# Owen1B/KAIR

Measured on AMD Instinct MI355X. Metric: train patches/sec + PSNR, SwinIR x4 48-px LQ, at 1/2/4/8 MI355X, higher is better.
Workload: dtype fp32x3

## Files before the change

include/kair_hip.h:

```cpp
#ifndef KAIR_HIP_H
#define KAIR_HIP_H

#ifdef __cplusplus
extern "C" {
#endif

#define KAIR_OK 0
#define KAIR_ERR_ARG (-1)
#define KAIR_ERR_HIP (-2)

typedef enum { KAIR_F32 = 0, KAIR_BF16 = 1, KAIR_F16 = 3 } kair_dtype;
#define KAIR_COMPUTE_X3 2
#define KAIR_X3_WEXP 12

typedef enum {
  KAIR_LD_ROWS = 0,
  KAIR_LD_IM2COL3 = 1,
  KAIR_LD_QKVBLK = 2,
  KAIR_LD_S2D = 3
} kair_load_mode;

typedef struct {
  const void* ptr;
  int dtype;
// ... 47 lines not shown
} kair_epilogue;

int kair_gemm_nt(const kair_operand* A, const kair_operand* B, const kair_epilogue* E,
                 long M, int N, int K, int compute, void* stream);

int kair_conv3x3_halo_geometry(int H, int W, int C, long M, int N);

int kair_wgrad_splits(long M, int N, int K);
int kair_gemm_tn(const kair_operand* A, const kair_operand* B, float* ws, int splits,
                 long M, int N, int K, int compute, void* stream);

typedef struct {
  int kind;
  int N, K;
  int nG, nGr, nGp;
  int kG, kGr, kGp;
  int n_perm;
} kair_wmap;

int kair_pack_weight(const float* src, void* dst, int dst_dtype, const kair_wmap* map, void* stream);
typedef struct kair_pack_job {
  const float* src;
  void* dst;
  int dst_dtype;
  int reserved;
  kair_wmap map;
  long total;
} kair_pack_job;
long kair_pack_table_bytes(int njobs);
long kair_pack_table_build(kair_pack_job* jobs, int njobs, void* table_dev);
int kair_pack_weights(const void* table_dev, int njobs, long nblocks, void* stream);
int kair_wgrad_finalize(const float* partial, int splits, const kair_wmap* map, float* grad_ref,
                        float* bias_grad, int ones_col, int accumulate, void* stream);
typedef struct {
  kair_operand A, B;
  int N, K;
  kair_wmap map;
  float* grad;
  float* bias_grad;
  int ones_col;
} kair_wgrad_job;
long kair_wgrad_grouped_ws(const kair_wgrad_job* jobs, int njobs, long M);
int kair_wgrad_grouped(const kair_wgrad_job* jobs, int njobs, long M, float* ws, void* stream);
int kair_wgrad_grouped_ex(const kair_wgrad_job* jobs, int njobs, long M, float* ws, int max_ctas, void* stream);
int kair_colsum(const kair_operand* G, long M, int Np, const kair_wmap* map, float* bias_grad,
                float* ws, int accumulate, void* stream);

int kair_layernorm_fwd(const float* x, long ldx, void* y, int y_dtype, long ldy, const float* gamma,
                       const float* beta, float* mean, float* rstd, long M, int C, float eps,
                       int win_H, int win_W, int win_ws, int win_shift, int one_col, void* stream);
int kair_layernorm_fwd_x3(const float* x, long ldx, void* y_hi, void* y_lo, long ldy, const float* gamma,
                          const float* beta, float* mean, float* rstd, long M, int C, float eps,
                          int win_H, int win_W, int win_ws, int win_shift, int one_col, int x3_exp, void* stream);
typedef struct {
  void* out;
  int dtype;
  long ld;
  const float* rowscale;
  int rows_per_scale;
  int win_H, win_W, win_ws, win_shift;
  void* out_lo;
  int x3_exp;
} kair_copy_desc;
int kair_row_copy(const float* src, long ld_src, long M, int C, const kair_copy_desc* copy, void* stream);

int kair_layernorm_bwd(const float* x, long ldx, const void* dy, int dy_dtype, long ldy,
                       const float* gamma, const float* mean, const float* rstd, float* dx_acc,
                       long ld_dx, int dx_accumulate, float* dgamma, float* dbeta, int dparam_accumulate,
                       float* ws, long M, int C, int win_H, int win_W, int win_ws, int win_shift,
                       const kair_copy_desc* copy, void* stream);

long kair_layernorm_bwd_blocks(long M);
typedef struct {
  const float* part; long nb; int C;
  float* dgamma; float* dbeta; int accumulate;
} kair_ln_param_job;
int kair_ln_param_reduce_grouped(const kair_ln_param_job* jobs, int njobs, void* stream);

int kair_window_attn_fwd(const void* qkv, int dtype, const float* table, void* O, long ldo, float* lse,
                         long nWin, int nh, int hd, float scale, int H, int W, int shift, int ones_col,
                         const float* mask, int mask_nw, void* stream);
long kair_window_attn_bwd_ws(long nWin, int nh);
int kair_window_attn_bwd(const void* qkv, const void* O, long ldo, const void* dO, long lddo, int dtype,
                         const float* table, const float* lse, void* dqkv, float* dtable, int dtable_accumulate,
                         float* ws, long nWin, int nh, int hd, float scale, int H, int W, int shift,
                         const float* mask, int mask_nw, void* stream);
int kair_window_attn_bwd_ex(const void* qkv, const void* O, long ldo, const void* dO, long lddo, int dtype,
                            const float* table, const float* lse, void* dqkv, int dqkv_rows, float* dtable,
                            int dtable_accumulate, float* ws, long nWin, int nh, int hd, float scale, int H, int W,
                            int shift, const float* mask, int mask_nw, int head_pad, void* stream);
int kair_window_attn_fwd_ex(const void* qkv, int dtype, const float* table, void* O, long ldo, float* lse,
                            long nWin, int nh, int hd, float scale, int H, int W, int shift, int ones_col,
                            const float* mask, int mask_nw, int head_pad, void* stream);
int kair_window_attn_fwd_w(const void* qkv, int dtype, const float* table, void* O, long ldo, float* lse,
                           long nWin, int nh, int hd, float scale, int H, int W, int shift, int ones_col,
                           const float* mask, int mask_nw, int head_pad, int ws, void* stream);
int kair_window_attn_bwd_w(const void* qkv, const void* O, long ldo, const void* dO, long lddo, int dtype,
                           const float* table, const float* lse, void* dqkv, int dqkv_rows, float* dtable,
                           int dtable_accumulate, float* ws, long nWin, int nh, int hd, float scale, int H, int W,
                           int shift, const float* mask, int mask_nw, int head_pad, int win_ws, void* stream);
long kair_window_attn_bwd_ws_w(long nWin, int nh, int win_ws);

int kair_window_attn_fwd_x3(const void* qkv, const void* qkv_lo, const float* table, void* O, void* O_lo, long ldo,
                            float* lse, long nWin, int nh, int hd, float scale, int H, int W, int shift, int ones_col,
                            int e_in, int e_out, void* stream);
int kair_window_attn_bwd_x3(const void* qkv, const void* qkv_lo, const void* O, const void* O_lo, long ldo,
                            const void* dO, const void* dO_lo, long lddo, const float* table, const float* lse,
                            void* dqkv, void* dqkv_lo, float* dtable, int dtable_accumulate, float* ws, long nWin,
                            int nh, int hd, float scale, int H, int W, int shift, int e_act, int e_grad, void* stream);
int kair_window_attn_fwd_x3_w(const void* qkv, const void* qkv_lo, const float* table, void* O, void* O_lo, long ldo,
                              float* lse, long nWin, int nh, int hd, float scale, int H, int W, int shift, int ones_col,
                              int e_in, int e_out, int ws, void* stream);
int kair_window_attn_bwd_x3_w(const void* qkv, const void* qkv_lo, const void* O, const void* O_lo, long ldo,
                              const void* dO, const void* dO_lo, long lddo, const float* table, const float* lse,
                              void* dqkv, void* dqkv_lo, float* dtable, int dtable_accumulate, float* ws, long nWin,
                              int nh, int hd, float scale, int H, int W, int shift, int e_act, int e_grad, int win_ws,
                              void* stream);

long kair_window_attn_bwd_groups(long nWin, int nh, int dtype);
typedef struct {
  const float* ws; long nWin; int nh; int dtype;
  float* dtable; int accumulate;
  int win_ws;
} kair_attn_dtable_job;
int kair_attn_dtable_grouped(const kair_attn_dtable_job* jobs, int njobs, void* stream);

int kair_swin_attn_fwd(const float* x, long ldx, const float* gamma, const float* beta, float eps, int C,
                       void* ln, long ldln, float* mean, float* rstd, const void* wqkv, const float* bqkv,
                       void* qkv, const float* table, float scale, void* O, long ldo, int o_ones_col,
                       float* lse, const void* wproj, const float* bproj, const float* rowscale,
                       int rows_per_scale, float* out, long ldout, long nWin, int nh, int H, int W, int shift,
                       int w_split, void* stream);
int kair_swin_mlp_fwd(const float* x, long ldx, const float* gamma, const float* beta, float eps, int C,
                      void* ln, long ldln, float* mean, float* rstd, const void* w1, const float* b1, void* u,
                      void* h, long ldh, int hd, const void* w2, const float* b2, const float* rowscale,
                      int rows_per_scale, float* out, long ldout, long M, int Cp, int Hp, int w_split,
                      void* stream);

long kair_swin_mlp_bwd_ws(void);
int kair_swin_mlp_bwd(const void* dc, long lddc, const void* gd, long ldg, const void* w2t, const void* w1t,
                      void* du, long lddu, const float* x, long ldx, const float* gamma, const float* mean,
                      const float* rstd, int C, float* D, long ldD, void* dco, long lddo, const float* rowscale,
                      int rows_per_scale, int H, int W, int shift, float* dgamma, float* dbeta, int dparam_acc,
                      float* ws, long M, int Cp, int Hp, void* stream);

int kair_conv3x3_wr_tile(int split, int B, int H, int W, int C, int N);
int kair_conv3x3_wr(const void* x, int x_dtype, long ldx, int split, int flip, const void* w, int n_blocks,
                    const float* bias, const float* resid, long ldr, void* out, int out_dtype, long ldo, void* acopy,
                    long ldac, int acones, int B, int H, int W, int C, int N, void* stream);
int kair_conv3x3_wr_ex(const void* x, int x_dtype, long ldx, int split, int flip, const void* w, int n_blocks,
                       const float* bias, const float* resid, long ldr, void* out, int out_dtype, long ldo, void* out_lo,
                       int ps_r, int act, float slope, const void* gate, long ldg, void* acopy, long ldac, int acones,
                       int B, int H, int W, int C, int N, void* stream);

int kair_conv3x3_narrow_fwd(const void* x, long ldx, int lo_off, const void* w, const float* bias, int NR,
                            const float* mean, float img_range, const float* resid, float* out, int B, int H, int W,
                            void* stream);
long kair_conv3x3_narrow_dgrad_ws(void);
int kair_conv3x3_narrow_dgrad(const void* dE, long lde, const float* w, int NR, void* ws, void* out, int out_dtype,
                              long ldo, int ps_r, int B, int H, int W, void* stream);
long kair_conv3x3_narrow_wgrad_ws(int NR);
int kair_conv3x3_narrow_wgrad(const void* dE, long lde, const void* x, long ldx, int NR, float* ws, float* grad_w,
                              float* grad_b, int accumulate, int B, int H, int W, void* stream);

long kair_conv3x3_narrow_x3_ws(void);
int kair_conv3x3_narrow_fwd_x3(const float* x, long ldx, int ex, const float* w, const float* bias, int NR, void* ws,
                               const float* mean, float img_range, const float* resid, float* out, int B, int H, int W,
                               void* stream);
int kair_conv3x3_narrow_dgrad_x3(const float* dE, long lde, int eg, const float* w, int NR, void* ws, float* out, long ldo,
                                 int ps_r, int B, int H, int W, void* stream);
int kair_conv3x3_narrow_wgrad_x3(const float* dE, long lde, int eg, const float* x, long ldx, int ex, int NR, float* ws,
                                 float* grad_w, float* grad_b, int accumulate, int B, int H, int W, void* stream);

int kair_image_to_nhwc(const float* img, void* out, int dtype, int ldc, const float* mean, float img_range,
                       int B, int C, int H, int W, void* stream);
int kair_image_to_nhwc_hilo(const float* img, void* out, int ldc, const float* mean, float img_range,
                            int B, int C, int H, int W, void* stream);
int kair_l1_loss(const float* E, const float* H, float* loss_out, void* dE, int dtype, int ldc, int ps_r, float weight,
                 int B, int C, int Hh, int Ww, float* ws, void* stream);
int kair_charbonnier_loss(const float* E, const float* H, float* loss_out, void* dE, int dtype, int ldc, int ps_r,
                          float weight, float eps, int B, int C, int Hh, int Ww, float* ws, void* stream);
int kair_axpy(float* y, const float* x, float a, long n, void* stream);
long kair_bn_ws(int C);
int kair_bn_fwd(const float* z, long ldz, void* out, int out_dtype, long ldo, long M, int C, const float* gamma,
                const float* beta, float* running_mean, float* running_var, float momentum, float eps, int training,
                float* mean, float* rstd, int act, float slope, float* ws, void* stream);
int kair_bn_bwd(const float* z, long ldz, const void* a, int a_dtype, long lda, const float* da, long ldda, void* dz,
                int dz_dtype, long lddz, long M, int C, const float* gamma, const float* mean, const float* rstd,
                int act, float slope, float* dgamma, float* dbeta, int accumulate, float* ws, void* stream);

int kair_axpby(float* y, const float* x, float a, float b, long n, void* stream);
int kair_axpby_rows(float* y, long ldy, const float* x, long ldx, long M, int C, float a, float b, void* stream);
int kair_act_grad_cast(const float* G, long ldg, const void* X, int x_dtype, long ldx, void* out, int out_dtype,
                       long ldo, long M, int C, int kind, float slope, float scale, void* stream);
int kair_sumpool2x(const float* src, long lds, float* dst, long ldd, int B, int H, int W, int C, int accumulate,
                   void* stream);
int kair_adam_ema(float* p, const float* g, float* m, float* v, float* ema, long n, const float* lr_t,
                  float beta1, float beta2, float eps, float weight_decay, float ema_decay, void* stream);
int kair_adam_ema_ex(float* p, const float* g, float* m, float* v, float* ema, long n, const float* lr_t,
                     float beta1, float beta2, float eps, float weight_decay, float ema_decay, const unsigned* skip,
                     void* stream);
int kair_range_check(const float* g, const float* p, long n, const float* loss, float p_limit, unsigned* flag,
                     void* stream);
long kair_gemm_nt_x3_lnbwd_parts(long M, int N);
int kair_gemm_nt_x3_lnbwd(const kair_operand* A, const kair_operand* B, long M, int N, int K, int win_H, int win_W,
                          int win_ws, int win_shift, const float* x, long ldx, const float* gamma, const float* mean,
                          const float* rstd, int C, float* D, long ldd, float* part, const kair_copy_desc* copy,
                          void* stream);

int kair_ktime_begin(int n);
int kair_ktime_count(void);
int kair_ktime_end(void);
int kair_ktime_read(int i, float* ms, const char** name);

int kair_gate_hold(int timeout_ms, void* stream);
int kair_gate_release(void);
int kair_gate_status(void);

#define KAIR_USR_SRC_NCHW 0
#define KAIR_USR_SRC_PSF 1
#define KAIR_USR_SRC_ZUP 2
#define KAIR_USR_SRC_NHWC 3
#define KAIR_USR_COL_FB 0
#define KAIR_USR_COL_FBFY 1
#define KAIR_USR_COL_DATA_FWD 2
#define KAIR_USR_COL_DATA_BWD 3
#define KAIR_USR_CHAN_CHUNKS 64
int kair_usr_fft_rows(const float* src, int src_mode, int C, long ld, int kh, int kw, int sf, void* T,
                      int planes, int H, int W, void* stream);
int kair_usr_fft_cols(int mode, const void* T, void* T_out, const void* FB, const void* FBFy, void* FR,
                      float* invW, const float* alpha, int alpha_stride, float* part, int planes, int C,
                      int H, int W, int sf, void* stream);
int kair_usr_ifft_rows(const void* T, void* dst, int nhwc, int dst_dtype, int C, long ld, float scale,
                       int planes, int H, int W, void* stream);
int kair_usr_seg_sum(const float* ws, int seglen, int nseg, float scale, float* out, int ostride,
                     int accumulate, void* stream);
int kair_usr_chan_sum(const float* x, long ld, int c, long HW, int B, float* ws, float* out, int ostride,
                      int accumulate, void* stream);
enum { KAIR_USR_PAD_REPLICATE = 0, KAIR_USR_PAD_ZERO = 1, KAIR_USR_PAD_FOLD = 2, KAIR_USR_CROP_NCHW = 3 };
int kair_usr_pad(const void* src, void* dst, int dtype, int mode, int ldc, int nb, int H, int W, int Hp, int Wp,
                 void* stream);
int kair_usr_upsample_nearest(const float* L, float* out, int planes, int h, int w, int sf, void* stream);
int kair_usr_pack_input(const float* x, const float* beta, int beta_stride, void* out, int dtype, int ld,
                        int B, int C, long HW, void* stream);
int kair_hypanet_fwd(const float* sigma, float sf, const float* W1, const float* b1, const float* W2,
                     const float* b2, const float* W3, const float* b3, int hc, int no, int B, float* ab,
                     void* stream);
int kair_hypanet_bwd(const float* sigma, float sf, const float* W1, const float* b1, const float* W2,
                     const float* b2, const float* W3, const float* b3, int hc, int no, int B, const float* gab,
                     float* gW1, float* gb1, float* gW2, float* gb2, float* gW3, float* gb3, int accumulate,
                     void* stream);

int kair_rowgemm_store(const void* A, long lda, long M, int K, const void* W, int N, void* out, long ldo,
                       void* stream);
int kair_rowgemm_gate(const void* A, long lda, long M, int K, const void* W, int N, const void* gate, long ldg,
                      void* out, long ldo, void* stream);
long kair_rowgemm_ln_blocks(long M, int K);
int kair_rowgemm_lnbwd(const void* A, long lda, long M, int K, const void* W, const float* x, long ldx,
                       const float* gamma, const float* mean, const float* rstd, int C, float* D, long ldD,
                       int win_H, int win_W, int win_ws, int win_shift, const kair_copy_desc* copy, float* part,
                       void* stream);

int kair_synth_sr(const float* pool, int C, int Hs, int Ws, const int* params, int B, int PS, int sf,
                  const float* wh, const int* ih, const float* ww, const int* iw, int P, float* outH,
                  float* outL, void* stream);
int kair_synth_dn(const float* pool, int C, int Hs, int Ws, const int* params, int B, int PS, float sigma,
                  unsigned long long seed, unsigned long long step, float* outH, float* outL, void* stream);

const char* kair_last_error(void);
int kair_device_arch(char* buf, int len);

int kair_debug_attn_stamps(unsigned long long* host, int n);
int kair_debug_fused_stamps(unsigned long long* host, int n);
int kair_debug_x3_stamps(unsigned long long* host, int n);

#ifdef __cplusplus
}
#endif
#endif
```

kair_amd/_hip.py:

```python
import ctypes
import os

import torch

LIB_PATH = os.path.join(os.path.dirname(os.path.abspath(__file__)), "lib",
                        {"debug": "libkair_hip_dbg.so", "base": "libkair_hip_base.so"}.get(os.environ.get("KAIR_LIB"),
                                                                                          "libkair_hip.so"))

F32, BF16, F16 = 0, 1, 3
X3 = 2
X3_WEXP = 12
LD_ROWS, LD_IM2COL3, LD_QKVBLK, LD_S2D = 0, 1, 2, 3
USR_SRC_NCHW, USR_SRC_PSF, USR_SRC_ZUP, USR_SRC_NHWC = 0, 1, 2, 3
USR_COL_FB, USR_COL_FBFY, USR_COL_DATA_FWD, USR_COL_DATA_BWD = 0, 1, 2, 3
USR_CHAN_CHUNKS = 64
USR_PAD_REPLICATE, USR_PAD_ZERO, USR_PAD_FOLD, USR_CROP_NCHW = 0, 1, 2, 3
OUT_ROWS, OUT_QKVBLK, OUT_PSHUF, OUT_PUNSHUF, OUT_NCHW, OUT_PSHUF_NCHW = 0, 1, 2, 3, 4, 5
OUT_PSHUF_SPM, OUT_PUNSHUF_SPM = 6, 7
ACT_NONE, ACT_GELU, ACT_LEAKY, ACT_RELU = 0, 1, 2, 3

c_long, c_int, c_float, c_vp = ctypes.c_long, ctypes.c_int, ctypes.c_float, ctypes.c_void_p


class Operand(ctypes.Structure):
    _fields_ = [("ptr", c_vp), ("dtype", c_int), ("mode", c_int), ("ld", c_long),
                ("win_H", c_int), ("win_W", c_int), ("win_ws", c_int), ("win_shift", c_int),
                ("im_H", c_int), ("im_W", c_int), ("im_C", c_int), ("im_flip", c_int),
                ("qkv_nh", c_int), ("qkv_hdp", c_int), ("qkv_tok", c_int),
                ("rowscale", c_vp), ("rows_per_scale", c_int), ("ones_col", c_int), ("ones_in_data", c_int),
                ("im_up", c_int), ("w_split", c_int), ("a_split", c_int), ("lo_ptr", c_vp), ("x3_exp", c_int)]


class CopyDesc(ctypes.Structure):
    _fields_ = [("out", c_vp), ("dtype", c_int), ("ld", c_long), ("rowscale", c_vp), ("rows_per_scale", c_int),
                ("win_H", c_int), ("win_W", c_int), ("win_ws", c_int), ("win_shift", c_int), ("out_lo", c_vp),
                ("x3_exp", c_int)]


def copy_desc(out, ld=None, rowscale=None, rows_per_scale=1, win=None, x3_exp=0):
    d = CopyDesc()
    d._keep = (out, rowscale)
    if out.dtype == torch.float16:
        d.out, d.out_lo, d.dtype, d.x3_exp = ptr(out[0]), ptr(out[1]), F16, int(x3_exp)
    else:
        d.out, d.dtype = ptr(out), dtype_code(out)
    d.ld = ld if ld is not None else out.shape[-1]
    d.rowscale, d.rows_per_scale = ptr(rowscale), rows_per_scale
    if win:
        d.win_H, d.win_W, d.win_ws, d.win_shift = win
    return d


class Epilogue(ctypes.Structure):
    _fields_ = [("out", c_vp), ("out_dtype", c_int), ("out_mode", c_int), ("ldo", c_long),
                ("win_H", c_int), ("win_W", c_int), ("win_ws", c_int), ("win_shift", c_int),
                ("bias", c_vp), ("act", c_int), ("slope", c_float),
                ("out_pre", c_vp), ("pre_dtype", c_int), ("ldp", c_long),
                ("resid", c_vp), ("ldr", c_long),
                ("rowscale", c_vp), ("rows_per_scale", c_int),
                ("gate", c_vp), ("gate_dtype", c_int), ("ldg", c_long), ("gate_kind", c_int),
                ("ps_r", c_int), ("ps_H", c_int), ("ps_W", c_int),
                ("qkv_nh", c_int), ("qkv_hdp", c_int), ("qkv_tok", c_int),
                ("img_mean", c_vp), ("img_range", c_float), ("img_C", c_int), ("img_H", c_int), ("img_W", c_int),
                ("out_ones_col_p1", c_int), ("resid2", c_vp), ("ldr2", c_long), ("pre_kind", c_int),
                ("a_copy", c_vp), ("ld_acopy", c_long), ("acopy_ones_col_p1", c_int), ("out_lo", c_vp),
                ("x3_out_exp", c_int)]


class WMap(ctypes.Structure):
    _fields_ = [("kind", c_int), ("N", c_int), ("K", c_int), ("nG", c_int), ("nGr", c_int), ("nGp", c_int),
                ("kG", c_int), ("kGr", c_int), ("kGp", c_int), ("n_perm", c_int)]


class WgradJob(ctypes.Structure):
    _fields_ = [("A", Operand), ("B", Operand), ("N", c_int), ("K", c_int), ("map", WMap), ("grad", c_vp),
                ("bias_grad", c_vp), ("ones_col", c_int)]


class LnParamJob(ctypes.Structure):
    _fields_ = [("part", c_vp), ("nb", c_long), ("C", c_int), ("dgamma", c_vp), ("dbeta", c_vp), ("accumulate", c_int)]


class DtabJob(ctypes.Structure):
    _fields_ = [("ws", c_vp), ("nWin", c_long), ("nh", c_int), ("dtype", c_int), ("dtable", c_vp), ("accumulate", c_int),
                ("win_ws", c_int)]


class PackJob(ctypes.Structure):
    _fields_ = [("src", c_vp), ("dst", c_vp), ("dst_dtype", c_int), ("reserved", c_int), ("map", WMap),
                ("total", c_long)]


_SIGS = {
    "kair_gemm_nt": [ctypes.POINTER(Operand), ctypes.POINTER(Operand), ctypes.POINTER(Epilogue), c_long, c_int, c_int,
                     c_int, c_vp],
    "kair_wgrad_splits": [c_long, c_int, c_int],
    "kair_conv3x3_halo_geometry": [c_int, c_int, c_int, c_long, c_int],
    "kair_gemm_tn": [ctypes.POINTER(Operand), ctypes.POINTER(Operand), c_vp, c_int, c_long, c_int, c_int, c_int, c_vp],
    "kair_wgrad_grouped_ws": [ctypes.POINTER(WgradJob), c_int, c_long],
    "kair_wgrad_grouped": [ctypes.POINTER(WgradJob), c_int, c_long, c_vp, c_vp],
    "kair_wgrad_grouped_ex": [ctypes.POINTER(WgradJob), c_int, c_long, c_vp, c_int, c_vp],
    "kair_layernorm_bwd_blocks": [c_long],
    "kair_ln_param_reduce_grouped": [ctypes.POINTER(LnParamJob), c_int, c_vp],
    "kair_window_attn_bwd_groups": [c_long, c_int, c_int],
    "kair_attn_dtable_grouped": [ctypes.POINTER(DtabJob), c_int, c_vp],
    "kair_pack_weight": [c_vp, c_vp, c_int, ctypes.POINTER(WMap), c_vp],
    "kair_pack_table_bytes": [c_int],
    "kair_pack_table_build": [ctypes.POINTER(PackJob), c_int, c_vp],
    "kair_pack_weights": [c_vp, c_int, c_long, c_vp],
    "kair_wgrad_finalize": [c_vp, c_int, ctypes.POINTER(WMap), c_vp, c_vp, c_int, c_int, c_vp],
    "kair_colsum": [ctypes.POINTER(Operand), c_long, c_int, ctypes.POINTER(WMap), c_vp, c_vp, c_int, c_vp],
    "kair_layernorm_fwd": [c_vp, c_long, c_vp, c_int, c_long, c_vp, c_vp, c_vp, c_vp, c_long, c_int, c_float, c_int,
                           c_int, c_int, c_int, c_int, c_vp],
    "kair_layernorm_fwd_x3": [c_vp, c_long, c_vp, c_vp, c_long, c_vp, c_vp, c_vp, c_vp, c_long, c_int, c_float, c_int,
                              c_int, c_int, c_int, c_int, c_int, c_vp],
    "kair_layernorm_bwd": [c_vp, c_long, c_vp, c_int, c_long, c_vp, c_vp, c_vp, c_vp, c_long, c_int, c_vp, c_vp, c_int,
                           c_vp, c_long, c_int, c_int, c_int, c_int, c_int, ctypes.POINTER(CopyDesc), c_vp],
    "kair_row_copy": [c_vp, c_long, c_long, c_int, ctypes.POINTER(CopyDesc), c_vp],
    "kair_gemm_nt_x3_lnbwd": [ctypes.POINTER(Operand), ctypes.POINTER(Operand), c_long, c_int, c_int, c_int, c_int, c_int,
                              c_int, c_vp, c_long, c_vp, c_vp, c_vp, c_int, c_vp, c_long, c_vp, ctypes.POINTER(CopyDesc),
                              c_vp],
    "kair_gemm_nt_x3_lnbwd_parts": [c_long, c_int],
    "kair_window_attn_fwd": [c_vp, c_int, c_vp, c_vp, c_long, c_vp, c_long, c_int, c_int, c_float, c_int, c_int, c_int,
                             c_int, c_vp, c_int, c_vp],
    "kair_window_attn_bwd_ws": [c_long, c_int],
    "kair_window_attn_bwd_ws_w": [c_long, c_int, c_int],
    "kair_window_attn_fwd_w": [c_vp, c_int, c_vp, c_vp, c_long, c_vp, c_long, c_int, c_int, c_float, c_int, c_int, c_int,
                               c_int, c_vp, c_int, c_int, c_int, c_vp],
    "kair_window_attn_bwd_w": [c_vp, c_vp, c_long, c_vp, c_long, c_int, c_vp, c_vp, c_vp, c_int, c_vp, c_int, c_vp, c_long,
                               c_int, c_int, c_float, c_int, c_int, c_int, c_vp, c_int, c_int, c_int, c_vp],
    "kair_window_attn_fwd_x3_w": [c_vp, c_vp, c_vp, c_vp, c_vp, c_long, c_vp, c_long, c_int, c_int, c_float, c_int, c_int,
                                  c_int, c_int, c_int, c_int, c_int, c_vp],
    "kair_window_attn_bwd_x3_w": [c_vp, c_vp, c_vp, c_vp, c_long, c_vp, c_vp, c_long, c_vp, c_vp, c_vp, c_vp, c_vp, c_int,
                                  c_vp, c_long, c_int, c_int, c_float, c_int, c_int, c_int, c_int, c_int, c_int, c_vp],
    "kair_window_attn_bwd": [c_vp, c_vp, c_long, c_vp, c_long, c_int, c_vp, c_vp, c_vp, c_vp, c_int, c_vp, c_long, c_int,
                             c_int, c_float, c_int, c_int, c_int, c_vp, c_int, c_vp],
    "kair_window_attn_bwd_ex": [c_vp, c_vp, c_long, c_vp, c_long, c_int, c_vp, c_vp, c_vp, c_int, c_vp, c_int, c_vp, c_long,
                                c_int, c_int, c_float, c_int, c_int, c_int, c_vp, c_int, c_int, c_vp],
    "kair_window_attn_fwd_ex": [c_vp, c_int, c_vp, c_vp, c_long, c_vp, c_long, c_int, c_int, c_float, c_int, c_int, c_int,
                                c_int, c_vp, c_int, c_int, c_vp],
    "kair_image_to_nhwc": [c_vp, c_vp, c_int, c_int, c_vp, c_float, c_int, c_int, c_int, c_int, c_vp],
    "kair_image_to_nhwc_hilo": [c_vp, c_vp, c_int, c_vp, c_float, c_int, c_int, c_int, c_int, c_vp],
    "kair_conv3x3_narrow_fwd": [c_vp, c_long, c_int, c_vp, c_vp, c_int, c_vp, c_float, c_vp, c_vp, c_int, c_int, c_int,
                                c_vp],
    "kair_conv3x3_wr_tile": [c_int, c_int, c_int, c_int, c_int, c_int],
    "kair_conv3x3_wr": [c_vp, c_int, c_long, c_int, c_int, c_vp, c_int, c_vp, c_vp, c_long, c_vp, c_int, c_long, c_vp,
                        c_long, c_int, c_int, c_int, c_int, c_int, c_int, c_vp],
    "kair_conv3x3_wr_ex": [c_vp, c_int, c_long, c_int, c_int, c_vp, c_int, c_vp, c_vp, c_long, c_vp, c_int, c_long, c_vp,
                           c_int, c_int, c_float, c_vp, c_long, c_vp, c_long, c_int, c_int, c_int, c_int, c_int, c_int,
                           c_vp],
    "kair_conv3x3_narrow_dgrad_ws": [],
    "kair_conv3x3_narrow_dgrad": [c_vp, c_long, c_vp, c_int, c_vp, c_vp, c_int, c_long, c_int, c_int, c_int, c_int, c_vp],
    "kair_conv3x3_narrow_wgrad_ws": [c_int],
    "kair_conv3x3_narrow_wgrad": [c_vp, c_long, c_vp, c_long, c_int, c_vp, c_vp, c_vp, c_int, c_int, c_int, c_int, c_vp],
    "kair_conv3x3_narrow_x3_ws": [],
    "kair_conv3x3_narrow_fwd_x3": [c_vp, c_long, c_int, c_vp, c_vp, c_int, c_vp, c_vp, c_float, c_vp, c_vp, c_int, c_int,
                                   c_int, c_vp],
    "kair_conv3x3_narrow_dgrad_x3": [c_vp, c_long, c_int, c_vp, c_int, c_vp, c_vp, c_long, c_int, c_int, c_int, c_int,
                                     c_vp],
    "kair_conv3x3_narrow_wgrad_x3": [c_vp, c_long, c_int, c_vp, c_long, c_int, c_int, c_vp, c_vp, c_vp, c_int, c_int,
                                     c_int, c_int, c_vp],
    "kair_l1_loss": [c_vp, c_vp, c_vp, c_vp, c_int, c_int, c_int, c_float, c_int, c_int, c_int, c_int, c_vp, c_vp],
    "kair_charbonnier_loss": [c_vp, c_vp, c_vp, c_vp, c_int, c_int, c_int, c_float, c_float, c_int, c_int, c_int, c_int,
                              c_vp, c_vp],
    "kair_axpy": [c_vp, c_vp, c_float, c_long, c_vp],
    "kair_axpby": [c_vp, c_vp, c_float, c_float, c_long, c_vp],
    "kair_bn_ws": [c_int],
    "kair_bn_fwd": [c_vp, c_long, c_vp, c_int, c_long, c_long, c_int, c_vp, c_vp, c_vp, c_vp, c_float, c_float, c_int,
                    c_vp, c_vp, c_int, c_float, c_vp, c_vp],
    "kair_bn_bwd": [c_vp, c_long, c_vp, c_int, c_long, c_vp, c_long, c_vp, c_int, c_long, c_long, c_int, c_vp, c_vp, c_vp,
                    c_int, c_float, c_vp, c_vp, c_int, c_vp, c_vp],
    "kair_axpby_rows": [c_vp, c_long, c_vp, c_long, c_long, c_int, c_float, c_float, c_vp],
    "kair_act_grad_cast": [c_vp, c_long, c_vp, c_int, c_long, c_vp, c_int, c_long, c_long, c_int, c_int, c_float, c_float,
                           c_vp],
    "kair_sumpool2x": [c_vp, c_long, c_vp, c_long, c_int, c_int, c_int, c_int, c_int, c_vp],
    "kair_adam_ema": [c_vp, c_vp, c_vp, c_vp, c_vp, c_long, c_vp, c_float, c_float, c_float, c_float, c_float, c_vp],
    "kair_adam_ema_ex": [c_vp, c_vp, c_vp, c_vp, c_vp, c_long, c_vp, c_float, c_float, c_float, c_float, c_float, c_vp,
                         c_vp],
    "kair_range_check": [c_vp, c_vp, c_long, c_vp, c_float, c_vp, c_vp],
    "kair_gate_hold": [c_int, c_vp],
    "kair_gate_release": [],
    "kair_gate_status": [],
    "kair_ktime_begin": [c_int],
    "kair_ktime_count": [],
    "kair_ktime_end": [],
    "kair_ktime_read": [c_int, ctypes.POINTER(ctypes.c_float), ctypes.POINTER(ctypes.c_char_p)],
    "kair_usr_fft_rows": [c_vp, c_int, c_int, c_long, c_int, c_int, c_int, c_vp, c_int, c_int, c_int, c_vp],
    "kair_usr_fft_cols": [c_int, c_vp, c_vp, c_vp, c_vp, c_vp, c_vp, c_vp, c_int, c_vp, c_int, c_int, c_int, c_int, c_int,
                          c_vp],
    "kair_usr_ifft_rows": [c_vp, c_vp, c_int, c_int, c_int, c_long, c_float, c_int, c_int, c_int, c_vp],
    "kair_usr_seg_sum": [c_vp, c_int, c_int, c_float, c_vp, c_int, c_int, c_vp],
    "kair_usr_chan_sum": [c_vp, c_long, c_int, c_long, c_int, c_vp, c_vp, c_int, c_int, c_vp],
    "kair_usr_upsample_nearest": [c_vp, c_vp, c_int, c_int, c_int, c_int, c_vp],
    "kair_usr_pack_input": [c_vp, c_vp, c_int, c_vp, c_int, c_int, c_int, c_int, c_long, c_vp],
    "kair_usr_pad": [c_vp, c_vp, c_int, c_int, c_int, c_int, c_int, c_int, c_int, c_int, c_vp],
    "kair_hypanet_fwd": [c_vp, c_float] + [c_vp] * 6 + [c_int, c_int, c_int, c_vp, c_vp],
    "kair_hypanet_bwd": [c_vp, c_float] + [c_vp] * 6 + [c_int, c_int, c_int, c_vp] + [c_vp] * 6 + [c_int, c_vp],
    "kair_synth_sr": [c_vp, c_int, c_int, c_int, c_vp, c_int, c_int, c_int, c_vp, c_vp, c_vp, c_vp, c_int, c_vp, c_vp,
                      c_vp],
    "kair_synth_dn": [c_vp, c_int, c_int, c_int, c_vp, c_int, c_int, c_float, ctypes.c_ulonglong, ctypes.c_ulonglong,
                      c_vp, c_vp, c_vp],
    "kair_swin_attn_fwd": [c_vp, c_long, c_vp, c_vp, c_float, c_int, c_vp, c_long, c_vp, c_vp, c_vp, c_vp, c_vp, c_vp,
                           c_float, c_vp, c_long, c_int, c_vp, c_vp, c_vp, c_vp, c_int, c_vp, c_long, c_long, c_int,
                           c_int, c_int, c_int, c_int, c_vp],
    "kair_swin_mlp_fwd": [c_vp, c_long, c_vp, c_vp, c_float, c_int, c_vp, c_long, c_vp, c_vp, c_vp, c_vp, c_vp, c_vp,
                          c_long, c_int, c_vp, c_vp, c_vp, c_int, c_vp, c_long, c_long, c_int, c_int, c_int, c_vp],
    "kair_debug_attn_stamps": [c_vp, c_int],
    "kair_debug_fused_stamps": [c_vp, c_int],
    "kair_debug_x3_stamps": [c_vp, c_int],
    "kair_swin_mlp_bwd_ws": [],
    "kair_swin_mlp_bwd": [c_vp, c_long, c_vp, c_long, c_vp, c_vp, c_vp, c_long, c_vp, c_long, c_vp, c_vp, c_vp, c_int,
                          c_vp, c_long, c_vp, c_long, c_vp, c_int, c_int, c_int, c_int, c_vp, c_vp, c_int, c_vp, c_long,
                          c_int, c_int, c_vp],
    "kair_rowgemm_store": [c_vp, c_long, c_long, c_int, c_vp, c_int, c_vp, c_long, c_vp],
    "kair_rowgemm_gate": [c_vp, c_long, c_long, c_int, c_vp, c_int, c_vp, c_long, c_vp, c_long, c_vp],
    "kair_rowgemm_ln_blocks": [c_long, c_int],
    "kair_rowgemm_lnbwd": [c_vp, c_long, c_long, c_int, c_vp, c_vp, c_long, c_vp, c_vp, c_vp, c_int, c_vp, c_long,
                           c_int, c_int, c_int, c_int, ctypes.POINTER(CopyDesc), c_vp, c_vp],
    "kair_window_attn_fwd_x3": [c_vp, c_vp, c_vp, c_vp, c_vp, c_long, c_vp, c_long, c_int, c_int, c_float, c_int, c_int,
                                c_int, c_int, c_int, c_int, c_vp],
    "kair_window_attn_bwd_x3": [c_vp, c_vp, c_vp, c_vp, c_long, c_vp, c_vp, c_long, c_vp, c_vp, c_vp, c_vp, c_vp, c_int,
                                c_vp, c_long, c_int, c_int, c_float, c_int, c_int, c_int, c_int, c_int, c_vp],
    "kair_last_error": [],
    "kair_device_arch": [ctypes.c_char_p, c_int],
}
_RESTYPE = {"kair_gemm_nt_x3_lnbwd_parts": c_long, "kair_layernorm_bwd_blocks": c_long, "kair_rowgemm_ln_blocks": c_long, "kair_window_attn_bwd_groups": c_long, "kair_wgrad_grouped_ws": c_long, "kair_swin_mlp_bwd_ws": c_long, "kair_bn_ws": c_long, "kair_last_error": ctypes.c_char_p, "kair_window_attn_bwd_ws": c_long, "kair_window_attn_bwd_ws_w": c_long, "kair_pack_table_bytes": c_long,
            "kair_pack_table_build": c_long, "kair_conv3x3_narrow_wgrad_ws": c_long,
            "kair_conv3x3_narrow_dgrad_ws": c_long, "kair_conv3x3_narrow_x3_ws": c_long}

_lib = None


def lib():
    global _lib
    if _lib is None:
        if not os.path.exists(LIB_PATH):
            raise RuntimeError(f"kair_amd: HIP kernel library not built ({LIB_PATH}); run `python -m kair_amd.build`")
        L = ctypes.CDLL(LIB_PATH)
        for name, args in _SIGS.items():
            if (name.startswith("kair_debug_") or os.environ.get("KAIR_LIB") == "base") and not hasattr(L, name):
                continue
            fn = getattr(L, name)
            fn.argtypes = args
            fn.restype = _RESTYPE.get(name, c_int)
        _lib = L
    return _lib


def exported_symbols():
    return list(_SIGS)


def check(rc, what=""):
    if rc != 0:
        msg = lib().kair_last_error().decode(errors="replace")
        raise RuntimeError(f"kair_hip {what} failed ({rc}): {msg}")


def ptr(t):
    if t is None:
        return None
    return t.data_ptr()


def stream_ptr():
    return torch.cuda.current_stream().cuda_stream


def dtype_code(t):
    if t.dtype == torch.float32:
        return F32
    if t.dtype == torch.bfloat16:
        return BF16
    if t.dtype == torch.float16:
        return F16
    raise TypeError(f"unsupported dtype {t.dtype}")


def require_device(*ts):
    for t in ts:
        if t is not None and not t.is_cuda:
            raise RuntimeError("kair_amd runs on the HIP device only (got a CPU tensor); there is no CPU fallback")


def rows(t, ld=None, win=None, rowscale=None, rows_per_scale=1, ones_col=-1, ones_in_data=False, w_split=False):
    o = Operand()
    o._keep = (t, rowscale)
    o.ptr = ptr(t)
    o.dtype = dtype_code(t)
    o.mode = LD_ROWS
    o.ld = ld if ld is not None else t.shape[-1]
    if win:
        o.win_H, o.win_W, o.win_ws, o.win_shift = win
    o.rowscale = ptr(rowscale)
    o.rows_per_scale = rows_per_scale
    o.ones_col = ones_col
    o.ones_in_data = int(ones_in_data)
    o.w_split = int(w_split)
    return o


def asplit(op, lo=None, pair=False):
    op.a_split = 2 if pair else 1
# ... 162 lines not shown
        arr = (PackJob * n)()
        for i, (src, dst, m) in enumerate(jobs):
            arr[i].src, arr[i].dst, arr[i].dst_dtype, arr[i].map = ptr(src), ptr(dst), dtype_code(dst), m
        self._keep = [(s, d) for s, d, _ in jobs]
        self.n = n
        self.table = torch.empty(lib().kair_pack_table_bytes(n), dtype=torch.uint8, device=jobs[0][1].device)
        nb = lib().kair_pack_table_build(arr, n, ptr(self.table))
        if nb <= 0:
            check(int(nb) or -1, "pack_table_build")
        self.nblocks = nb

    def run(self):
        check(lib().kair_pack_weights(ptr(self.table), self.n, self.nblocks, stream_ptr()), "pack_weights")


def wgrad_finalize(partial, splits, m, grad, bias_grad=None, ones_col=-1, accumulate=False):
    check(lib().kair_wgrad_finalize(ptr(partial), splits, ctypes.byref(m), ptr(grad), ptr(bias_grad), ones_col,
                                    int(accumulate), stream_ptr()), "wgrad_finalize")


def colsum(G, M, Np, m, bias_grad, ws, accumulate=False):
    check(lib().kair_colsum(ctypes.byref(G), M, Np, ctypes.byref(m), ptr(bias_grad), ptr(ws), int(accumulate),
                            stream_ptr()), "colsum")


def layernorm_fwd(x, ldx, y, ldy, gamma, beta, mean, rstd, M, C, eps=1e-5, win=(0, 0, 0, 0), one_col=-1):
    check(lib().kair_layernorm_fwd(ptr(x), ldx, ptr(y), dtype_code(y), ldy, ptr(gamma), ptr(beta), ptr(mean), ptr(rstd),
                                   M, C, eps, *win, one_col, stream_ptr()), "layernorm_fwd")


def layernorm_fwd_x3(x, ldx, y, ldy, gamma, beta, mean, rstd, M, C, eps=1e-5, win=(0, 0, 0, 0), one_col=-1, x3_exp=0):
    check(lib().kair_layernorm_fwd_x3(ptr(x), ldx, ptr(y[0]), ptr(y[1]), ldy, ptr(gamma), ptr(beta), ptr(mean), ptr(rstd),
                                      M, C, eps, *win, one_col, int(x3_exp), stream_ptr()), "layernorm_fwd_x3")


def layernorm_bwd(x, ldx, dy, ldy, gamma, mean, rstd, dx, ld_dx, dx_acc, dgamma, dbeta, dparam_acc, ws, M, C,
                  win=(0, 0, 0, 0), copy=None):
    check(lib().kair_layernorm_bwd(ptr(x), ldx, ptr(dy), dtype_code(dy), ldy, ptr(gamma), ptr(mean), ptr(rstd), ptr(dx),
                                   ld_dx, int(dx_acc), ptr(dgamma), ptr(dbeta), int(dparam_acc), ptr(ws), M, C, *win,
                                   ctypes.byref(copy) if copy is not None else None, stream_ptr()), "layernorm_bwd")


def gemm_nt_lnbwd(A, B, M, N, K, x, ldx, gamma, mean, rstd, C, D, ldd, part, win=(0, 0, 0, 0), copy=None):
    check(lib().kair_gemm_nt_x3_lnbwd(ctypes.byref(A), ctypes.byref(B), M, N, K, *win, ptr(x), ldx, ptr(gamma), ptr(mean),
                                      ptr(rstd), C, ptr(D), ldd, ptr(part),
                                      ctypes.byref(copy) if copy is not None else None, stream_ptr()), "gemm_nt_x3_lnbwd")


def gemm_nt_lnbwd_parts(M, N):
    return lib().kair_gemm_nt_x3_lnbwd_parts(M, N)


def row_copy(src, ld_src, M, C, copy):
    check(lib().kair_row_copy(ptr(src), ld_src, M, C, ctypes.byref(copy), stream_ptr()), "row_copy")


def window_attn_fwd(qkv, table, O, ldo, lse, nWin, nh, hd, scale, H, W, shift, ones_col=-1, mask=None, head_pad=32, ws=8):
    mnw = mask.shape[0] if mask is not None else 0
    check(lib().kair_window_attn_fwd_w(ptr(qkv), dtype_code(qkv), ptr(table), ptr(O), ldo, ptr(lse), nWin, nh, hd, scale,
                                       H, W, shift, ones_col, ptr(mask), mnw, head_pad, ws, stream_ptr()), "window_attn_fwd")


GROUP_MAX = 32


def layernorm_bwd_blocks(M):
    return lib().kair_layernorm_bwd_blocks(M)


def ln_param_reduce_grouped(jobs):
    arr = (LnParamJob * len(jobs))()
    for i, job in enumerate(jobs):
        part, M, C, dg, db, acc = job[:6]
        nb = job[6] if len(job) > 6 else layernorm_bwd_blocks(M)
        arr[i].part, arr[i].nb, arr[i].C = ptr(part), nb, C
        arr[i].dgamma, arr[i].dbeta, arr[i].accumulate = ptr(dg), ptr(db), int(acc)
    check(lib().kair_ln_param_reduce_grouped(arr, len(jobs), stream_ptr()), "ln_param_reduce_grouped")


def attn_dtable_grouped(jobs):
    arr = (DtabJob * len(jobs))()
    for i, job in enumerate(jobs):
        ws, nWin, nh, dt, dtable, acc = job[:6]
        arr[i].ws, arr[i].nWin, arr[i].nh, arr[i].dtype = ptr(ws), nWin, nh, dt
        arr[i].dtable, arr[i].accumulate = ptr(dtable), int(acc)
        arr[i].win_ws = job[6] if len(job) > 6 else 0
    check(lib().kair_attn_dtable_grouped(arr, len(jobs), stream_ptr()), "attn_dtable_grouped")


def window_attn_bwd_ws(nWin, nh, ws=8):
    if ws not in (7, 8):
        raise ValueError(f"window_attn_bwd_ws: window size {ws} (7 or 8)")
    return lib().kair_window_attn_bwd_ws_w(nWin, nh, ws)


def window_attn_bwd(qkv, O, ldo, dO, lddo, table, lse, dqkv, dtable, dtable_acc, ws, nWin, nh, hd, scale, H, W, shift,
                    mask=None, dqkv_rows=False, head_pad=32, win_ws=8):
    mnw = mask.shape[0] if mask is not None else 0
    check(lib().kair_window_attn_bwd_w(ptr(qkv), ptr(O), ldo, ptr(dO), lddo, dtype_code(qkv), ptr(table), ptr(lse),
                                       ptr(dqkv), int(dqkv_rows), ptr(dtable), int(dtable_acc), ptr(ws), nWin, nh, hd,
                                       scale, H, W, shift, ptr(mask), mnw, head_pad, win_ws, stream_ptr()), "window_attn_bwd")


def _planes(t):
    return (ptr(t), None) if t.dtype == torch.float32 else (ptr(t[0]), ptr(t[1]))


def window_attn_fwd_x3(qkv, table, O, ldo, lse, nWin, nh, hd, scale, H, W, shift, ones_col=-1, e_in=0, e_out=0, ws=8):
    o, ol = _planes(O)
    check(lib().kair_window_attn_fwd_x3_w(ptr(qkv[0]), ptr(qkv[1]), ptr(table), o, ol, ldo, ptr(lse), nWin,
                                          nh, hd, scale, H, W, shift, ones_col, e_in, e_out, ws, stream_ptr()),
          "window_attn_fwd_x3")


def window_attn_bwd_x3(qkv, O, ldo, dO, lddo, table, lse, dqkv, dtable, dtable_acc, ws, nWin, nh, hd, scale, H, W, shift,
                       e_act=0, e_grad=0, win_ws=8):
    o, ol = _planes(O)
    dq, dql = _planes(dqkv)
    check(lib().kair_window_attn_bwd_x3_w(ptr(qkv[0]), ptr(qkv[1]), o, ol, ldo, ptr(dO[0]), ptr(dO[1]), lddo,
                                          ptr(table), ptr(lse), dq, dql, ptr(dtable), int(dtable_acc),
                                          ptr(ws), nWin, nh, hd, scale, H, W, shift, e_act, e_grad, win_ws, stream_ptr()),
          "window_attn_bwd_x3")


def with_lo(op, lo):
    op.lo_ptr = ptr(lo)
    op._keep = (op._keep, lo)
    return op


def conv3x3_narrow_fwd(x, ldx, lo_off, w, bias, NR, mean, img_range, resid, out, B, H, W):
    check(lib().kair_conv3x3_narrow_fwd(ptr(x), ldx, lo_off, ptr(w), ptr(bias), NR, ptr(mean), img_range, ptr(resid),
                                        ptr(out), B, H, W, stream_ptr()), "conv3x3_narrow_fwd")


def conv3x3_wr_tile(split, B, H, W, C, N):
    return lib().kair_conv3x3_wr_tile(int(bool(split)), B, H, W, C, N)


def conv3x3_wr(x, ldx, flip, w, bias, resid, out, B, H, W, C, N, ldr=None, ldo=None, acopy=None, ldac=None, acones=-1,
               n_blocks=None, split=None, out_lo=None, ps_r=0, act=ACT_NONE, slope=0.0, gate=None, ldg=None):
    if split is None:
        split = x.dtype == torch.float32
    if n_blocks is None:
        n_blocks = 16 if N > 192 else 12 if N > 64 else 4
    check(lib().kair_conv3x3_wr_ex(ptr(x), dtype_code(x), ldx, int(bool(split)), int(flip), ptr(w), n_blocks, ptr(bias),
                                   ptr(resid), ldr if ldr is not None else (resid.shape[-1] if resid is not None else 0),
                                   ptr(out), dtype_code(out), ldo if ldo is not None else out.shape[-1], ptr(out_lo), ps_r,
                                   act, slope, ptr(gate), ldg if ldg is not None else (gate.shape[-1] if gate is not None else 0),
                                   ptr(acopy), ldac if ldac is not None else (acopy.shape[-1] if acopy is not None else 0),
                                   acones, B, H, W, C, N, stream_ptr()), "conv3x3_wr")


def conv3x3_narrow_dgrad_ws():
    return lib().kair_conv3x3_narrow_dgrad_ws()


def conv3x3_narrow_dgrad(dE, lde, w, NR, ws, out, ldo, ps_r, B, H, W):
    check(lib().kair_conv3x3_narrow_dgrad(ptr(dE), lde, ptr(w), NR, ptr(ws), ptr(out), dtype_code(out), ldo, ps_r, B, H, W,
                                          stream_ptr()), "conv3x3_narrow_dgrad")


def conv3x3_narrow_wgrad_ws(NR):
    return lib().kair_conv3x3_narrow_wgrad_ws(NR)


def conv3x3_narrow_wgrad(dE, lde, x, ldx, NR, ws, grad_w, grad_b, B, H, W, accumulate=False):
    check(lib().kair_conv3x3_narrow_wgrad(ptr(dE), lde, ptr(x), ldx, NR, ptr(ws), ptr(grad_w), ptr(grad_b),
                                          int(accumulate), B, H, W, stream_ptr()), "conv3x3_narrow_wgrad")


def conv3x3_narrow_x3_ws():
    return lib().kair_conv3x3_narrow_x3_ws()


def conv3x3_narrow_fwd_x3(x, ldx, ex, w, bias, NR, ws, mean, img_range, resid, out, B, H, W):
    check(lib().kair_conv3x3_narrow_fwd_x3(ptr(x), ldx, ex, ptr(w), ptr(bias), NR, ptr(ws), ptr(mean), img_range, ptr(resid),
                                           ptr(out), B, H, W, stream_ptr()), "conv3x3_narrow_fwd_x3")


def conv3x3_narrow_dgrad_x3(dE, lde, eg, w, NR, ws, out, ldo, ps_r, B, H, W):
    check(lib().kair_conv3x3_narrow_dgrad_x3(ptr(dE), lde, eg, ptr(w), NR, ptr(ws), ptr(out), ldo, ps_r, B, H, W,
                                             stream_ptr()), "conv3x3_narrow_dgrad_x3")


def conv3x3_narrow_wgrad_x3(dE, lde, eg, x, ldx, ex, NR, ws, grad_w, grad_b, B, H, W, accumulate=False):
    check(lib().kair_conv3x3_narrow_wgrad_x3(ptr(dE), lde, eg, ptr(x), ldx, ex, NR, ptr(ws), ptr(grad_w), ptr(grad_b),
                                             int(accumulate), B, H, W, stream_ptr()), "conv3x3_narrow_wgrad_x3")


def image_to_nhwc_hilo(img, out, ldc, mean, img_range, B, C, H, W):
    check(lib().kair_image_to_nhwc_hilo(ptr(img), ptr(out), ldc, ptr(mean), img_range, B, C, H, W, stream_ptr()),
          "image_to_nhwc_hilo")


def image_to_nhwc(img, out, ldc, mean, img_range, B, C, H, W):
    check(lib().kair_image_to_nhwc(ptr(img), ptr(out), dtype_code(out), ldc, ptr(mean), img_range, B, C, H, W,
                                   stream_ptr()), "image_to_nhwc")


def l1_loss(E, H, loss_out, dE, ldc, weight, B, C, Hh, Ww, ws, ps_r=1, charb_eps=None):
    if charb_eps is not None:
        check(lib().kair_charbonnier_loss(ptr(E), ptr(H), ptr(loss_out), ptr(dE), dtype_code(dE), ldc, ps_r, weight,
                                          float(charb_eps), B, C, Hh, Ww, ptr(ws), stream_ptr()), "charbonnier_loss")
        return
    check(lib().kair_l1_loss(ptr(E), ptr(H), ptr(loss_out), ptr(dE), dtype_code(dE), ldc, ps_r, weight, B, C, Hh, Ww,
                             ptr(ws), stream_ptr()), "l1_loss")


def axpy(y, x, a, n=None):
    check(lib().kair_axpy(ptr(y), ptr(x), a, n if n is not None else y.numel(), stream_ptr()), "axpy")


def adam_ema(p, g, m, v, ema, n, lr_t, beta1, beta2, eps, wd, decay, skip=None):
    if skip is not None:
        check(lib().kair_adam_ema_ex(ptr(p), ptr(g), ptr(m), ptr(v), ptr(ema), n, ptr(lr_t), beta1, beta2, eps, wd, decay,
                                     ptr(skip), stream_ptr()), "adam_ema_ex")
        return
    check(lib().kair_adam_ema(ptr(p), ptr(g), ptr(m), ptr(v), ptr(ema), n, ptr(lr_t), beta1, beta2, eps, wd, decay,
                              stream_ptr()), "adam_ema")


def ktime_begin(n=4096):
    check(lib().kair_ktime_begin(n), "ktime_begin")


def ktime_count():
    return lib().kair_ktime_count()


def ktime_end():
    return lib().kair_ktime_end()


def gate_hold(timeout_ms=5000):
    check(lib().kair_gate_hold(timeout_ms, stream_ptr()), "gate_hold")


def gate_release():
    check(lib().kair_gate_release(), "gate_release")


def gate_status():
    return lib().kair_gate_status()


def ktime_read(i):
    ms, name = ctypes.c_float(), ctypes.c_char_p()
    check(lib().kair_ktime_read(i, ctypes.byref(ms), ctypes.byref(name)), "ktime_read")
    return ms.value, (name.value or b"").decode(errors="replace")


def range_check(g, p, loss, p_limit, flag):
    check(lib().kair_range_check(ptr(g), ptr(p), g.numel(), ptr(loss), float(p_limit), ptr(flag), stream_ptr()),
          "range_check")


def axpby(y, x, a, b, n=None):
    check(lib().kair_axpby(ptr(y), ptr(x), a, b, n if n is not None else y.numel(), stream_ptr()), "axpby")


def act_grad_cast(G, ldg, X, ldx, out, ldo, M, C, kind, slope=0.0, scale=1.0):
    check(lib().kair_act_grad_cast(ptr(G), ldg, ptr(X), dtype_code(X) if X is not None else F32, ldx, ptr(out),
                                   dtype_code(out), ldo, M, C, kind, slope, scale, stream_ptr()), "act_grad_cast")


def sumpool2x(src, lds, dst, ldd, B, H, W, C, accumulate=False):
    check(lib().kair_sumpool2x(ptr(src), lds, ptr(dst), ldd, B, H, W, C, int(accumulate), stream_ptr()), "sumpool2x")


def axpby_rows(y, ldy, x, ldx, M, C, a, b):
    check(lib().kair_axpby_rows(ptr(y), ldy, ptr(x), ldx, M, C, a, b, stream_ptr()), "axpby_rows")


def usr_fft_rows(src, mode, C, ld, kh, kw, sf, T, planes, Hh, Ww):
    check(lib().kair_usr_fft_rows(ptr(src), mode, C, ld, kh, kw, sf, ptr(T), planes, Hh, Ww, stream_ptr()), "usr_fft_rows")


def usr_fft_cols(mode, T, Tout, FB, FBFy, FR, invW, alpha, alpha_stride, part, planes, C, Hh, Ww, sf):
    check(lib().kair_usr_fft_cols(mode, ptr(T), ptr(Tout), ptr(FB), ptr(FBFy), ptr(FR), ptr(invW), ptr(alpha),
                                  alpha_stride, ptr(part), planes, C, Hh, Ww, sf, stream_ptr()), "usr_fft_cols")


def usr_ifft_rows(T, dst, nhwc, C, ld, scale, planes, Hh, Ww):
    check(lib().kair_usr_ifft_rows(ptr(T), ptr(dst), int(nhwc), dtype_code(dst), C, ld, scale, planes, Hh, Ww,
                                   stream_ptr()), "usr_ifft_rows")


def usr_seg_sum(ws, seglen, nseg, scale, out, ostride, accumulate=False):
    check(lib().kair_usr_seg_sum(ptr(ws), seglen, nseg, scale, ptr(out), ostride, int(accumulate), stream_ptr()),
          "usr_seg_sum")


def usr_chan_sum(x, ld, c, HW, B, ws, out, ostride, accumulate=False):
    check(lib().kair_usr_chan_sum(ptr(x), ld, c, HW, B, ptr(ws), ptr(out), ostride, int(accumulate), stream_ptr()),
          "usr_chan_sum")


def usr_upsample_nearest(L, out, planes, h, w, sf):
    check(lib().kair_usr_upsample_nearest(ptr(L), ptr(out), planes, h, w, sf, stream_ptr()), "usr_upsample_nearest")


def usr_pad(src, dst, mode, ldc, nb, H, W, Hp, Wp):
    if src.dtype != dst.dtype:
        raise ValueError("usr_pad: src and dst dtypes differ")
    check(lib().kair_usr_pad(ptr(src), ptr(dst), dtype_code(dst), mode, ldc, nb, H, W, Hp, Wp, stream_ptr()), "usr_pad")
# ... 130 lines not shown
```

kair_amd/csrc/conv_wr.hip:

```cpp
#include "common.h"

namespace {

constexpr int WR_WAVES = 4;
constexpr int WR_NT = 64 * WR_WAVES;
template <int RN, bool SPLIT> struct WrPD {
  static constexpr int PD = RN != 1 ? 3 : SPLIT ? 6 : 9, UNR = RN == 1 && !SPLIT ? 18 : 6;
};

struct ConvWrArgs {
  const void* x; long ldx;
  const bf16* w;
  const float* bias;
  const float* resid; long ldr;
  void* out; int odt; long ldo;
  bf16* acopy; long ldac; int acones;
  bf16* out_lo;
  int ps_r;
  int act; float slope;
  const bf16* gate; long ldg;
  int psH, psW;
  int B, H, W, C, N, flip;
  long tilesM;
  FDiv fc8, fhwd;
};

template <bool SPLIT> struct WrGeom {
  static constexpr int HALO = SPLIT ? 40000 : 80000;
};

template <typename TX, bool SPLIT, int BM, bool RESID, int RN, int EM>
__global__ __launch_bounds__(WR_NT, 1) void conv3x3_wr_kernel(const ConvWrArgs a) {
  constexpr bool PAIR = SPLIT && sizeof(TX) == 2;
  constexpr int RM = BM / 16;
  constexpr int HALO = WrGeom<SPLIT>::HALO;
  constexpr int NB = SPLIT ? 2 : 1;
  __shared__ __attribute__((aligned(16))) bf16 sH[SPLIT ? 2 * HALO : HALO];
  bf16* const sLo = sH + (SPLIT ? HALO : 0);
  const int tid = threadIdx.x, lane = tid & 63, wave = __builtin_amdgcn_readfirstlane(tid >> 6);
  const int fr = lane & 15, fq = lane >> 4;
  const int H = a.H, W = a.W, C = a.C;
  constexpr int CGP = BM == 192 ? 2 : 1;
  static_assert(CGP == 1 || (!SPLIT && !RESID), "channel-half passes: plain image, no residual");
  const int CH = C / CGP;
  const int XW = W < BM ? W : BM, RPT = BM / XW, HWD = XW + 2, HR = RPT + 2, PS = CH + 8;
  const int c8n = CH / 8, halo_pieces = HR * HWD * c8n;
  const int cps = C / 32, cpsP = CH / 32, KSP = 9 * cpsP, KS = 9 * cps;
  int pass = 0;
  auto wstep = [&](int sl) { const int tap = sl / cpsP; return tap * cps + pass * cpsP + (sl - tap * cpsP); };
  int hb[RM];
#pragma unroll
  for (int i = 0; i < RM; ++i) {
    const int p = i * 16 + fr;
    const int ry = p / XW, rx = p - (p / XW) * XW;
    hb[i] = ((ry + 1) * HWD + rx + 1) * PS + fq * 8;
  }
  const bf16* wb = a.w + ((long)(RN * wave) * KS * NB) * 512 + lane * 8;
  auto wfrag = [&](int rn, int s, int half) {
    return *(const bf16x8*)(wb + (((long)rn * KS + s) * NB + half) * 512);
  };
  float4 bias4[RN];
#pragma unroll
  for (int rn = 0; rn < RN; ++rn) {
    const int n = 16 * RN * wave + 16 * rn + 4 * fq;
    bias4[rn] = a.bias && n < a.N ? *(const float4*)(a.bias + n) : make_float4(0.f, 0.f, 0.f, 0.f);
  }

  constexpr int PD = WrPD<RN, SPLIT>::PD, UNR = WrPD<RN, SPLIT>::UNR;
  bf16x8 rb[PD][RN][NB];
  auto issue_w = [&](int slot, int s) {
#pragma unroll
    for (int rn = 0; rn < RN; ++rn)
#pragma unroll
      for (int h = 0; h < NB; ++h) rb[slot][rn][h] = wfrag(rn, s, h);
  };
  bf16x8 ra[2][RM][NB];
  auto read_a = [&](int buf, int s) {
    const int tap = s / cpsP, c0 = (s - tap * cpsP) * 32;
    int dy = tap / 3 - 1, dx = tap - (tap / 3) * 3 - 1;
    if (a.flip) { dy = -dy; dx = -dx; }
    const int off = (dy * HWD + dx) * PS + c0;
#pragma unroll
    for (int i = 0; i < RM; ++i) {
      ra[buf][i][0] = *(const bf16x8*)(sH + hb[i] + off);
      if constexpr (SPLIT) ra[buf][i][1] = *(const bf16x8*)(sLo + hb[i] + off);
    }
  };

  const long tiles = a.tilesM;
  for (long t = blockIdx.x; t < tiles; t += gridDim.x) {
    const long p0 = t * BM;
    const int b = (int)(p0 / ((long)H * W));
    const int rem = (int)(p0 - (long)b * H * W);
    const int y0 = rem / W, x0 = rem - (rem / W) * W;
    f32x4 acc[RM][RN];
#pragma unroll
    for (int i = 0; i < RM; ++i)
#pragma unroll
      for (int rn = 0; rn < RN; ++rn) acc[i][rn] = f32x4{0.f, 0.f, 0.f, 0.f};
    float4 ex[RESID ? RM : 1][RN];
    auto load_resid = [&]() {
      if constexpr (RESID) {
#pragma unroll
        for (int i = 0; i < RM; ++i)
#pragma unroll
          for (int rn = 0; rn < RN; ++rn) {
            const long m = p0 + i * 16 + fr;
            const int n = 16 * RN * wave + 16 * rn + 4 * fq;
            ex[i][rn] = *(const float4*)(a.resid + m * a.ldr + (n < a.N ? n : 0));
          }
      }
    };
    for (pass = 0; pass < CGP; ++pass) {
#pragma unroll
    for (int u = 0; u < PD; ++u) issue_w(u, wstep(u));
    __syncthreads();
    {
      constexpr int HP = PAIR ? 5 : SPLIT ? 10 : (sizeof(TX) == 4 ? 12 : 16);
      const int per = (halo_pieces + WR_NT - 1) / WR_NT;
      for (int h0 = 0; h0 < per; h0 += HP) {
        uint4 v0[HP], v1[HP];
        bool okv[HP];
#pragma unroll
        for (int i = 0; i < HP; ++i) {
          const int idx = tid + WR_NT * (h0 + i);
          const int pix = fdiv(idx, a.fc8), c8 = idx - pix * c8n;
          const int hr = fdiv(pix, a.fhwd), hc = pix - hr * HWD;
          const int y = y0 - 1 + hr, x = x0 - 1 + hc;
          okv[i] = idx < halo_pieces && y >= 0 && y < H && x >= 0 && x < W;
          const long src = okv[i] ? ((long)(b * H + y) * W + x) * a.ldx + pass * CH + c8 * 8 : 0;
          if constexpr (sizeof(TX) == 4) {
            v0[i] = *(const uint4*)((const float*)a.x + src);
            v1[i] = *(const uint4*)((const float*)a.x + src + 4);
          } else {
            v0[i] = *(const uint4*)((const bf16*)a.x + src);
            if constexpr (PAIR) v1[i] = *(const uint4*)((const bf16*)a.x + src + C);
          }
        }
#pragma unroll
        for (int i = 0; i < HP; ++i) {
          const int idx = tid + WR_NT * (h0 + i);
          if (idx >= halo_pieces) continue;
          const int pix = fdiv(idx, a.fc8), c8 = idx - pix * c8n;
          uint4 qh, ql = make_uint4(0, 0, 0, 0);
          if constexpr (sizeof(TX) == 4) {
            const float4 u = __builtin_bit_cast(float4, v0[i]), v = __builtin_bit_cast(float4, v1[i]);
            const float f[8] = {u.x, u.y, u.z, u.w, v.x, v.y, v.z, v.w};
            bf16x8 hh, ll;
#pragma unroll
            for (int e = 0; e < 8; ++e) {
              hh[e] = (bf16)f[e];
              if constexpr (SPLIT) ll[e] = (bf16)(f[e] - (float)hh[e]);
            }
            qh = __builtin_bit_cast(uint4, hh);
            if constexpr (SPLIT) ql = __builtin_bit_cast(uint4, ll);
          } else {
            qh = v0[i];
            if constexpr (PAIR) ql = v1[i];
          }
          if (!okv[i]) qh = ql = make_uint4(0, 0, 0, 0);
          *(uint4*)(sH + pix * PS + c8 * 8) = qh;
          if constexpr (SPLIT) *(uint4*)(sLo + pix * PS + c8 * 8) = ql;
          if (a.acopy) {
            const int hr = fdiv(pix, a.fhwd), hc = pix - hr * HWD;
            if (hr >= 1 && hr <= RPT && hc >= 1 && hc <= XW) {
              uint4 qc = qh;
              const int oc = a.acones - c8 * 8;
              if ((unsigned)oc < 8u) {
                bf16x8 v8 = __builtin_bit_cast(bf16x8, qc);
                v8[oc] = (bf16)1.f;
                qc = __builtin_bit_cast(uint4, v8);
              }
              const long px = (long)(b * H + y0 + hr - 1) * W + x0 + hc - 1;
              *(uint4*)(a.acopy + px * a.ldac + c8 * 8) = qc;
            }
          }
        }
      }
    }
    __syncthreads();

    read_a(0, 0);
    auto step = [&](int u, int s, bool tail) {
      const int ab = u & 1, ws = u % PD;
      read_a(ab ^ 1, s + 1 < KSP ? s + 1 : KSP - 1);
      if (RESID && tail && u == UNR - 3) load_resid();
#pragma unroll
      for (int i = 0; i < RM; ++i)
#pragma unroll
        for (int rn = 0; rn < RN; ++rn) {
          acc[i][rn] = __builtin_amdgcn_mfma_f32_16x16x32_bf16(rb[ws][rn][0], ra[ab][i][0], acc[i][rn], 0, 0, 0);
          if constexpr (SPLIT) {
            acc[i][rn] = __builtin_amdgcn_mfma_f32_16x16x32_bf16(rb[ws][rn][1], ra[ab][i][0], acc[i][rn], 0, 0, 0);
            acc[i][rn] = __builtin_amdgcn_mfma_f32_16x16x32_bf16(rb[ws][rn][0], ra[ab][i][1], acc[i][rn], 0, 0, 0);
          }
        }
      issue_w(ws, wstep(s + PD < KSP ? s + PD : KSP - 1));
    };
    for (int s0 = 0; s0 < KSP - UNR; s0 += UNR) {
#pragma unroll
      for (int u = 0; u < UNR; ++u) step(u, s0 + u, false);
    }
#pragma unroll
    for (int u = 0; u < UNR; ++u) step(u, KSP - UNR + u, CGP == 1 || pass == CGP - 1);
    }
#pragma unroll
    for (int i = 0; i < RM; ++i)
#pragma unroll
      for (int rn = 0; rn < RN; ++rn) {
        const long m = p0 + i * 16 + fr;
        const int n = 16 * RN * wave + 16 * rn + 4 * fq;
        if (n >= a.N) continue;
        const float4 bb = bias4[rn];
        float v[4] = {acc[i][rn][0] + bb.x, acc[i][rn][1] + bb.y, acc[i][rn][2] + bb.z, acc[i][rn][3] + bb.w};
        if constexpr (RESID) {
          v[0] += ex[i][rn].x; v[1] += ex[i][rn].y; v[2] += ex[i][rn].z; v[3] += ex[i][rn].w;
        }
        if (a.act == KAIR_ACT_LEAKY) {
#pragma unroll
          for (int q = 0; q < 4; ++q) v[q] = v[q] > 0.f ? v[q] : v[q] * a.slope;
        }
        if (a.gate) {
          const bf16x4 gv = *(const bf16x4*)(a.gate + m * a.ldg + n);
#pragma unroll
          for (int q = 0; q < 4; ++q) v[q] *= (float)gv[q] > 0.f ? 1.f : a.slope;
        }
        long o = m * a.ldo + n;
        if constexpr (EM == 1) {
          const int r = a.ps_r, nf = a.N / (r * r);
          const int bi = (int)(m / ((long)H * W)), pp = (int)(m - (long)bi * H * W), yy = pp / W, xx = pp - yy * W;
          const int sp = n / nf, cc = n - sp * nf, ii = sp / r, jj = sp - ii * r;
          o = (((long)bi * H * r + (long)yy * r + ii) * ((long)W * r) + (long)xx * r + jj) * a.ldo + cc;
        } else if constexpr (EM == 2) {
          const int r = a.ps_r;
          const int bi = (int)(m / ((long)H * W)), pp = (int)(m - (long)bi * H * W), yy = pp / W, xx = pp - yy * W;
          const int yl = yy / r, xl = xx / r;
          o = (((long)bi * a.psH + yl) * a.psW + xl) * a.ldo + ((yy - yl * r) * r + (xx - xl * r)) * a.N + n;
        }
        if (a.odt == KAIR_BF16) {
          const bf16x4 hv = {(bf16)v[0], (bf16)v[1], (bf16)v[2], (bf16)v[3]};
          *(bf16x4*)((bf16*)a.out + o) = hv;
          if (a.out_lo)
            *(bf16x4*)(a.out_lo + o) = bf16x4{(bf16)(v[0] - (float)hv[0]), (bf16)(v[1] - (float)hv[1]),
                                              (bf16)(v[2] - (float)hv[2]), (bf16)(v[3] - (float)hv[3])};
        } else {
          *(float4*)((float*)a.out + o) = make_float4(v[0], v[1], v[2], v[3]);
        }
      }
  }
}

int wr_num_cus() {
  static int n = 0;
  if (n == 0) {
    int dev = 0;
    if (hipGetDevice(&dev) != hipSuccess || hipDeviceGetAttribute(&n, hipDeviceAttributeMultiprocessorCount, dev) != hipSuccess ||
        n <= 0)
      n = 256;
  }
  return n;
}

bool wr_geometry(int BM, int halo, long M, int H, int W, int C) {
  if (W <= 0 || H <= 0 || M <= 0) return false;
  if (W <= BM) {
    if (BM % W != 0 || H % (BM / W) != 0) return false;
  } else if (W % BM != 0) {
    return false;
  }
  const int XW = W < BM ? W : BM, RPT = BM / XW;
  return (long)(RPT + 2) * (XW + 2) * (C + 8) <= halo && M % BM == 0 && M % ((long)H * W) == 0;
}

}

extern "C" int kair_conv3x3_wr_tile(int split, int B, int H, int W, int C, int N) {
  const long M = (long)B * H * W;
  if (C <= 0 || C > 256 || C % 64 != 0 || N <= 0 || N > 256 || N % 4 != 0) return 0;
  if (split && C > 192) return 0;
  if (!split && N > 192) return 0;
  static const int cand_split[] = {96, 48}, cand_plain[] = {144, 96, 48}, cand_256[] = {192, 96, 48};
  const int* cand = split ? cand_split : C == 256 ? cand_256 : cand_plain;
  const int nc = split ? 2 : 3;
  const long want = 3L * wr_num_cus() / 4;
  int best = 0;
  for (int i = 0; i < nc; ++i) {
    const int bm = cand[i];
    if (!(split ? wr_geometry(bm, WrGeom<true>::HALO, M, H, W, C)
                : wr_geometry(bm, WrGeom<false>::HALO, M, H, W, bm == 192 ? C / 2 : C)))
      continue;
    if (bm == 192 && (N > 64 || W < 96)) continue;
    best = bm;
    if (M / bm >= want) return bm;
  }
  return best;
}

#define KAIR_WR(TXV, SPV, BMV, RV, RNV, EMV) \
  KAIR_LAUNCH((conv3x3_wr_kernel<TXV, SPV, BMV, RV, RNV, EMV>), dim3(grid), dim3(WR_NT), 0, s, a)

extern "C" int kair_conv3x3_wr_ex(const void* x, int x_dtype, long ldx, int split, int flip, const void* w, int n_blocks,
                                  const float* bias, const float* resid, long ldr, void* out, int out_dtype, long ldo,
                                  void* out_lo, int ps_r, int act, float slope, const void* gate, long ldg, void* acopy,
                                  long ldac, int acones, int B, int H, int W, int C, int N, void* stream) {
  KAIR_CHECK_ARG(x && w && out && B > 0, "conv3x3_wr: null operand");
  KAIR_CHECK_ARG(x_dtype == KAIR_F32 || x_dtype == KAIR_BF16, "conv3x3_wr: image dtype");
  KAIR_CHECK_ARG(out_dtype == KAIR_F32 || out_dtype == KAIR_BF16, "conv3x3_wr: output dtype");
  const bool pair = split && x_dtype == KAIR_BF16;
  int BM = kair_conv3x3_wr_tile(split, B, H, W, C, N);
  KAIR_CHECK_ARG(BM > 0, "conv3x3_wr: unsupported geometry (B %d, H %d, W %d, C %d, N %d)", B, H, W, C, N);
  if (BM == 144 && resid) {
    const long Mg = (long)B * H * W;
    BM = wr_geometry(96, WrGeom<false>::HALO, Mg, H, W, C) ? 96 : wr_geometry(48, WrGeom<false>::HALO, Mg, H, W, C) ? 48 : 0;
    KAIR_CHECK_ARG(BM > 0, "conv3x3_wr: no tile for a plain conv with a residual at this geometry");
  }
  const int RN = N > 192 ? 4 : N > 64 ? 3 : 1;
  KAIR_CHECK_ARG(n_blocks == 4 * RN, "conv3x3_wr: the packed weight needs %d output rows (%d blocks of 16), got %d blocks",
                 64 * RN, 4 * RN, n_blocks);
  KAIR_CHECK_ARG(ldx >= (pair ? 2 * C : C) && ldx % (x_dtype == KAIR_F32 ? 4 : 8) == 0 && ((uintptr_t)x & 15) == 0 &&
                     ((uintptr_t)w & 15) == 0,
                 "conv3x3_wr: image rows 16-byte aligned, ldx >= C (2 C for a [hi | lo] pair)");
  const int pr = ps_r < 0 ? -ps_r : ps_r;
  KAIR_CHECK_ARG(ps_r <= 0 || (N % (pr * pr) == 0 && (N / (pr * pr)) % 4 == 0 && !resid),
                 "conv3x3_wr: PixelShuffle output needs N %% r^2 == 0, N / r^2 %% 4 == 0 and no residual");
  KAIR_CHECK_ARG(ps_r >= 0 || (H % pr == 0 && W % pr == 0 && !resid && ldo >= (long)N * pr * pr),
                 "conv3x3_wr: PixelUnshuffle output needs H, W multiples of r, ldo >= N r^2, no residual");
  KAIR_CHECK_ARG(ldo >= (ps_r > 0 ? N / (pr * pr) : N) && ldo % 4 == 0 && ((uintptr_t)out & 15) == 0, "conv3x3_wr: output rows");
  KAIR_CHECK_ARG(!gate || (ps_r == 0 && !resid && ldg >= N && ldg % 4 == 0 && ((uintptr_t)gate & 7) == 0),
                 "conv3x3_wr: a gate needs a row output, no residual, 8-byte aligned bf16 rows");
  KAIR_CHECK_ARG(!out_lo || (out_dtype == KAIR_BF16 && ((uintptr_t)out_lo & 7) == 0), "conv3x3_wr: out_lo needs a bf16 output");
  KAIR_CHECK_ARG(!resid || (ldr >= N && ldr % 4 == 0 && ((uintptr_t)resid & 15) == 0), "conv3x3_wr: residual rows");
  KAIR_CHECK_ARG(!bias || ((uintptr_t)bias & 15) == 0, "conv3x3_wr: bias alignment");
  KAIR_CHECK_ARG(!acopy || (!pair && ldac >= C && ldac % 8 == 0 && ((uintptr_t)acopy & 15) == 0), "conv3x3_wr: a_copy rows");
  const long M = (long)B * H * W;
  KAIR_CHECK_ARG(M * (ldx > ldo ? ldx : ldo) * (ps_r ? ps_r * ps_r : 1) < (1L << 31), "conv3x3_wr: operands past 2^31 elements");
  ConvWrArgs a;
  a.x = x; a.ldx = ldx; a.w = (const bf16*)w; a.bias = bias; a.resid = resid; a.ldr = ldr;
  a.out = out; a.odt = out_dtype; a.ldo = ldo; a.acopy = (bf16*)acopy; a.ldac = ldac; a.acones = acopy ? acones : -1;
  a.out_lo = (bf16*)out_lo; a.ps_r = pr;
  a.gate = (const bf16*)gate; a.ldg = ldg;
  a.psH = pr ? H / pr : 0; a.psW = pr ? W / pr : 0;
  KAIR_CHECK_ARG(act == KAIR_ACT_NONE || (act == KAIR_ACT_LEAKY && !resid && !gate),
                 "conv3x3_wr: act none, or LeakyReLU without residual / gate");
  a.act = act; a.slope = slope;
  a.B = B; a.H = H; a.W = W; a.C = C; a.N = N; a.flip = flip;
  a.tilesM = M / BM;
  a.fc8 = make_fdiv(C / (BM == 192 ? 2 : 1) / 8);
  a.fhwd = make_fdiv((W < BM ? W : BM) + 2);
  const int ncu = wr_num_cus();
  const int grid = (int)(a.tilesM < ncu ? a.tilesM : ncu);
  hipStream_t s = (hipStream_t)stream;
  const bool rs = resid != nullptr;
#define KAIR_WR3(TXV, SPV, RV, RNV, EMV)                                                   \
  do {                                                                                     \
    if (BM == 48) KAIR_WR(TXV, SPV, 48, RV, RNV, EMV);                                     \
    else if (BM == 96) KAIR_WR(TXV, SPV, 96, RV, RNV, EMV);                                \
    else if constexpr (!SPV && !RV) KAIR_WR(TXV, SPV, 144, RV, RNV, EMV);                  \
  } while (0)
  if (pair) {
    KAIR_CHECK_ARG(RN == 4 && ps_r > 0 && !rs, "conv3x3_wr: the pair form is built for N in (192, 256] with a PixelShuffle store");
    KAIR_WR3(bf16, true, false, 4, 1);
  } else if (RN == 1 && !split) {
    KAIR_CHECK_ARG(x_dtype == KAIR_BF16 && ps_r <= 0 && !rs, "conv3x3_wr: the plain N <= 64 form takes a bf16 image");
    if (BM == 192) {
      KAIR_CHECK_ARG(!acopy, "conv3x3_wr: no a_copy with the two-pass tile");
      if (ps_r < 0) KAIR_WR(bf16, false, 192, false, 1, 2); else KAIR_WR(bf16, false, 192, false, 1, 0);
    } else if (ps_r < 0) KAIR_WR3(bf16, false, false, 1, 2); else KAIR_WR3(bf16, false, false, 1, 0);
  } else if (RN == 1) {
    KAIR_CHECK_ARG(split && x_dtype == KAIR_F32 && ps_r == 0, "conv3x3_wr: the N <= 64 form takes an fp32 image, split, rows");
    if (rs) KAIR_WR3(float, true, true, 1, 0); else KAIR_WR3(float, true, false, 1, 0);
  } else {
    KAIR_CHECK_ARG(RN == 3 && ps_r == 0, "conv3x3_wr: N <= 192 row outputs for this form");
    if (split) {
      if (rs) KAIR_WR3(float, true, true, 3, 0); else KAIR_WR3(float, true, false, 3, 0);
    } else if (x_dtype == KAIR_F32) {
      if (rs) KAIR_WR3(float, false, true, 3, 0); else KAIR_WR3(float, false, false, 3, 0);
    } else {
      if (rs) KAIR_WR3(bf16, false, true, 3, 0); else KAIR_WR3(bf16, false, false, 3, 0);
    }
  }
#undef KAIR_WR3
#undef KAIR_WR
  KAIR_CHECK_LAUNCH();
  return 0;
}

extern "C" int kair_conv3x3_wr(const void* x, int x_dtype, long ldx, int split, int flip, const void* w, int n_blocks,
                               const float* bias, const float* resid, long ldr, void* out, int out_dtype, long ldo, void* acopy,
                               long ldac, int acones, int B, int H, int W, int C, int N, void* stream) {
  return kair_conv3x3_wr_ex(x, x_dtype, ldx, split, flip, w, n_blocks, bias, resid, ldr, out, out_dtype, ldo, nullptr, 0,
                            KAIR_ACT_NONE, 0.f, nullptr, 0, acopy, ldac, acones, B, H, W, C, N, stream);
}
```

kair_amd/csrc/elementwise.hip:

```cpp
#include <stdlib.h>
#include <string.h>

#include <vector>

#include "common.h"

namespace {

KAIR_DEV int unpad(int ip, int G, int Gr, int Gp) {
  const int g = ip / Gp, i = ip - g * Gp;
  return (g < G && i < Gr) ? g * Gr + i : -1;
}

KAIR_DEV int nperm_fwd(const kair_wmap& mp, int n) {
  if (mp.n_perm <= 1 || n < 0) return n;
  const int nf = mp.N / mp.n_perm;
  return (n % nf) * mp.n_perm + n / nf;
}
KAIR_DEV int nperm_inv(const kair_wmap& mp, int co) {
  if (mp.n_perm <= 1) return co;
  const int nf = mp.N / mp.n_perm;
  return (co % mp.n_perm) * nf + co / mp.n_perm;
}

// ... 52 lines not shown
  } else if (mp.kind == 1) {
    const int np = (int)(t / (9 * Kp));
    const int kk = (int)(t - (long)np * 9 * Kp);
    const int tap = kk / Kp, cip = kk - tap * Kp;
    const int n = nperm_fwd(mp, unpad(np, mp.nG, mp.nGr, mp.nGp)), ci = unpad(cip, mp.kG, mp.kGr, mp.kGp);
    if (n >= 0 && ci >= 0) v = src[((long)n * mp.K + ci % mp.K) * 9 + tap];
  } else if (mp.kind == 2) {
    const int cip = (int)(t / (9 * Np));
    const int kk = (int)(t - (long)cip * 9 * Np);
    const int tap = kk / Np, cop = kk - tap * Np;
    const int n = nperm_fwd(mp, unpad(cop, mp.nG, mp.nGr, mp.nGp)), ci = unpad(cip, mp.kG, mp.kGr, mp.kGp);
    if (n >= 0 && ci >= 0) v = src[((long)n * mp.K + ci) * 9 + tap];
  } else if (mp.kind == 7) {
    const int np = (int)(t / (4 * Kp));
    const int kk = (int)(t - (long)np * 4 * Kp);
    const int tap = kk / Kp, kp = kk - tap * Kp;
    const int n = nperm_fwd(mp, unpad(np, mp.nG, mp.nGr, mp.nGp)), k = unpad(kp, mp.kG, mp.kGr, mp.kGp);
    if (n >= 0 && k >= 0) v = src[((long)n * mp.K + k) * 4 + tap];
  } else if (mp.kind == 9) {
    const int Kc = 9 * Kp, KS = 2 * ((Kc + 63) / 64) * 64;
    const int np = (int)(t / KS);
    const int kk = (int)(t - (long)np * KS);
    const int half = (kk >> 6) & 1, k = ((kk >> 7) << 6) + (kk & 63);
    if (k < Kc) {
      const int tap = k / Kp, cip = k - tap * Kp;
      const int n = nperm_fwd(mp, unpad(np, mp.nG, mp.nGr, mp.nGp)), ci = unpad(cip, mp.kG, mp.kGr, mp.kGp);
      if (n >= 0 && ci >= 0) v = src[((long)n * mp.K + ci % mp.K) * 9 + tap];
    }
    if (dt == KAIR_F16) {
      const float w = ldexpf(v, KAIR_X3_WEXP);
      const f16 hf = (f16)w;
      ((f16*)dst)[t] = half ? (f16)(w - (float)hf) : hf;
      return;
    }
    const bf16 hi = (bf16)v;
    ((bf16*)dst)[t] = half ? (bf16)(v - (float)hi) : hi;
    return;
  } else if (mp.kind == 10) {
    const int KB = Kp / 16;
    const int j = (int)(t & 7), ln = (int)((t >> 3) & 63);
    const long blk = t >> 9;
    const int kb = (int)(blk % KB), nb = (int)(blk / KB);
    const int np = nb * 32 + (ln & 31), kp = kb * 16 + 8 * (ln >> 5) + j;
    const int n = nperm_fwd(mp, unpad(np, mp.nG, mp.nGr, mp.nGp)), k = unpad(kp, mp.kG, mp.kGr, mp.kGp);
    if (n >= 0 && k >= 0) v = src[(long)n * mp.K + k];
  } else if (mp.kind == 13) {
    const int KB = Np / 16;
    const int j = (int)(t & 7), ln = (int)((t >> 3) & 63);
    const long blk = t >> 9;
    const int kb = (int)(blk % KB), ob = (int)(blk / KB);
    const int kp = ob * 32 + (ln & 31), np = kb * 16 + 8 * (ln >> 5) + j;
    const int n = nperm_fwd(mp, unpad(np, mp.nG, mp.nGr, mp.nGp)), k = unpad(kp, mp.kG, mp.kGr, mp.kGp);
    if (n >= 0 && k >= 0) v = src[(long)n * mp.K + k];
  } else if (mp.kind == 14) {
    const int KB = Kp / 32;
    const int j = (int)(t & 7), ln = (int)((t >> 3) & 63);
    const long blk = t >> 9;
    const int kb = (int)(blk % KB), nb = (int)(blk / KB);
    const int np = nb * 16 + (ln & 15), kp = kb * 32 + 8 * (ln >> 4) + j;
    const int n = nperm_fwd(mp, unpad(np, mp.nG, mp.nGr, mp.nGp)), k = unpad(kp, mp.kG, mp.kGr, mp.kGp);
    if (n >= 0 && k >= 0) v = src[(long)n * mp.K + k];
  } else if (mp.kind == 12) {
    const int KB = Kp / 16;
    const int j = (int)(t & 7), ln = (int)((t >> 3) & 63), half = (int)((t >> 9) & 1);
    const long blk = t >> 10;
    const int kb = (int)(blk % KB), nb = (int)(blk / KB);
    const int np = nb * 32 + (ln & 31), kp = kb * 16 + 8 * (ln >> 5) + j;
    const int n = nperm_fwd(mp, unpad(np, mp.nG, mp.nGr, mp.nGp)), k = unpad(kp, mp.kG, mp.kGr, mp.kGp);
    if (n >= 0 && k >= 0) v = src[(long)n * mp.K + k];
    const bf16 hi = (bf16)v;
    ((bf16*)dst)[t] = half ? (bf16)(v - (float)hi) : hi;
    return;
  } else if (mp.kind == 15) {
    const int KB = 9 * Kp / 32;
    const int j = (int)(t & 7), ln = (int)((t >> 3) & 63), half = (int)((t >> 9) & 1);
    const long blk = t >> 10;
    const int kb = (int)(blk % KB), nb = (int)(blk / KB);
    const int np = nb * 16 + (ln & 15), kk = kb * 32 + 8 * (ln >> 4) + j;
    const int tap = kk / Kp, cip = kk - tap * Kp;
    const int n = nperm_fwd(mp, unpad(np, mp.nG, mp.nGr, mp.nGp)), ci = unpad(cip, mp.kG, mp.kGr, mp.kGp);
    if (n >= 0 && ci >= 0) v = src[((long)n * mp.K + ci % mp.K) * 9 + tap];
    const bf16 hi = (bf16)v;
    ((bf16*)dst)[t] = half ? (bf16)(v - (float)hi) : hi;
    return;
  } else if (mp.kind == 16) {
    const int KB = 9 * Np / 32;
    const int j = (int)(t & 7), ln = (int)((t >> 3) & 63);
    const long blk = t >> 9;
    const int kb = (int)(blk % KB), cb = (int)(blk / KB);
    const int cip = cb * 16 + (ln & 15), kk = kb * 32 + 8 * (ln >> 4) + j;
    const int tap = kk / Np, cop = kk - tap * Np;
    const int n = nperm_fwd(mp, unpad(cop, mp.nG, mp.nGr, mp.nGp)), ci = unpad(cip, mp.kG, mp.kGr, mp.kGp);
    if (n >= 0 && ci >= 0) v = src[((long)n * mp.K + ci) * 9 + tap];
  } else if (mp.kind == 8) {
    const int row = (int)(t / Np), np = (int)(t - (long)row * Np);
    const int kp = row >> 2, tap = row & 3;
    const int n = nperm_fwd(mp, unpad(np, mp.nG, mp.nGr, mp.nGp)), k = unpad(kp, mp.kG, mp.kGr, mp.kGp);
    if (n >= 0 && k >= 0) v = src[((long)n * mp.K + k) * 4 + tap];
  } else {
    const int n = nperm_fwd(mp, unpad((int)t, mp.nG, mp.nGr, mp.nGp));
    if (n >= 0) v = src[n];
  }
  if (dt == KAIR_BF16) ((bf16*)dst)[t] = (bf16)v;
  else ((float*)dst)[t] = v;
}

__global__ void pack_kernel(const float* __restrict__ src, void* __restrict__ dst, int dt, kair_wmap mp, long total) {
  const long t = (long)blockIdx.x * blockDim.x + threadIdx.x;
  if (t < total) pack_element(src, dst, dt, mp, t);
}

__host__ __device__ inline bool pack_vec(const kair_wmap& mp, int dt) {
  if (dt != KAIR_BF16) return false;
  if (mp.kind == 0 || mp.kind == 10 || mp.kind == 14) return mp.kGp % 8 == 0 && (mp.kG * mp.kGp) % 8 == 0;
  if (mp.kind == 13) return mp.nGp % 8 == 0 && (mp.nG * mp.nGp) % 8 == 0;
  return false;
}

KAIR_DEV void pack_chunk(const float* __restrict__ src, bf16* __restrict__ dst, const kair_wmap& mp, long u) {
  const int Np = mp.nG * mp.nGp, Kp = mp.kG * mp.kGp;
  float v[8];
  long t0;
  if (mp.kind == 13) {
    const int kp = (int)(u % Kp), np0 = (int)(u / Kp) * 8;
    const int k = unpad(kp, mp.kG, mp.kGr, mp.kGp);
#pragma unroll
    for (int j = 0; j < 8; ++j) {
      const int n = nperm_fwd(mp, unpad(np0 + j, mp.nG, mp.nGr, mp.nGp));
      v[j] = (n >= 0 && k >= 0) ? src[(long)n * mp.K + k] : 0.f;
    }
    t0 = (((long)(kp >> 5) * (Np / 16) + (np0 >> 4)) * 64 + (kp & 31) + 32 * ((np0 & 15) >> 3)) * 8;
  } else {
    const int kc = Kp / 8;
    const int np = (int)(u / kc), kp0 = (int)(u % kc) * 8;
    const int n = nperm_fwd(mp, unpad(np, mp.nG, mp.nGr, mp.nGp));
#pragma unroll
    for (int j = 0; j < 8; ++j) {
      const int k = unpad(kp0 + j, mp.kG, mp.kGr, mp.kGp);
      v[j] = (n >= 0 && k >= 0) ? src[(long)n * mp.K + k] : 0.f;
    }
    if (mp.kind == 0) t0 = (long)np * Kp + kp0;
    else if (mp.kind == 10) t0 = (((long)(np >> 5) * (Kp / 16) + (kp0 >> 4)) * 64 + (np & 31) + 32 * ((kp0 & 15) >> 3)) * 8;
    else t0 = (((long)(np >> 4) * (Kp / 32) + (kp0 >> 5)) * 64 + (np & 15) + 16 * ((kp0 & 31) >> 3)) * 8;
  }
  bf16x8 o;
#pragma unroll
  for (int j = 0; j < 8; ++j) o[j] = (bf16)v[j];
  *(bf16x8*)(dst + t0) = o;
}

__host__ __device__ inline bool pack_pair_vec(const kair_wmap& mp, int dt) {
  if (dt != KAIR_F16 && dt != KAIR_BF16) return false;
  const int Np = mp.nG * mp.nGp, Kp = mp.kG * mp.kGp;
  if (mp.kind == 9 || mp.kind == 17 || mp.kind == 20) return Kp % 8 == 0;
  if (mp.kind == 18 || mp.kind == 19 || mp.kind == 21) return Np % 8 == 0;
  return false;
}

KAIR_DEV void pack_pair_chunk(const float* __restrict__ src, void* __restrict__ dst, int dt, const kair_wmap& mp, int u) {
  const int Np = mp.nG * mp.nGp, Kp = mp.kG * mp.kGp;
  const bool rows_n = mp.kind == 9 || mp.kind == 17 || mp.kind == 20;
  const int rowlen = mp.kind == 9 ? 9 * Kp : mp.kind == 17 ? Kp : mp.kind == 18 ? 9 * Np : mp.kind == 20 ? 4 * Kp : Np;
  const int rl64 = (rowlen + 63) / 64 * 64, cpr = rl64 / 8;
  const int row = u / cpr, k0 = (u - row * cpr) * 8;
  float v[8];
#pragma unroll
  for (int j = 0; j < 8; ++j) v[j] = 0.f;
  if (k0 < rowlen) {
    const int rr = rows_n ? nperm_fwd(mp, unpad(row, mp.nG, mp.nGr, mp.nGp))
                          : unpad(mp.kind == 21 ? row >> 2 : row, mp.kG, mp.kGr, mp.kGp);
    const int seg = (mp.kind == 9 || mp.kind == 20) ? Kp : (mp.kind == 18) ? Np : rowlen;
    const int tap = mp.kind == 21 ? (row & 3) : k0 / seg, c0 = mp.kind == 21 ? k0 : k0 - (k0 / seg) * seg;
#pragma unroll
    for (int j = 0; j < 8; ++j) {
      const int c = c0 + j;
      int n, k;
      if (rows_n) { n = rr; k = unpad(c, mp.kG, mp.kGr, mp.kGp); }
      else { n = nperm_fwd(mp, unpad(c, mp.nG, mp.nGr, mp.nGp)); k = rr; }
      if (n < 0 || k < 0) continue;
      if (mp.kind == 9) v[j] = src[((long)n * mp.K + k % mp.K) * 9 + tap];
      else if (mp.kind == 18) v[j] = src[((long)n * mp.K + k) * 9 + tap];
      else if (mp.kind == 20 || mp.kind == 21) v[j] = src[((long)n * mp.K + k) * 4 + tap];
      else v[j] = src[(long)n * mp.K + k];
    }
  }
  const long o = (long)row * 2 * rl64 + ((k0 >> 6) << 7) + (k0 & 63);
  if (dt == KAIR_F16) {
    f16x8 hi, lo;
#pragma unroll
    for (int j = 0; j < 8; ++j) {
      const float w = ldexpf(v[j], KAIR_X3_WEXP);
      hi[j] = (f16)w;
      lo[j] = (f16)(w - (float)hi[j]);
    }
    *(f16x8*)((f16*)dst + o) = hi;
    *(f16x8*)((f16*)dst + o + 64) = lo;
  } else {
    bf16x8 hi, lo;
#pragma unroll
    for (int j = 0; j < 8; ++j) {
      hi[j] = (bf16)v[j];
      lo[j] = (bf16)(v[j] - (float)hi[j]);
    }
    *(bf16x8*)((bf16*)dst + o) = hi;
    *(bf16x8*)((bf16*)dst + o + 64) = lo;
  }
}

__global__ __launch_bounds__(256) void pack_pair_kernel(const float* __restrict__ src, void* __restrict__ dst, int dt,
                                                        kair_wmap mp, long chunks) {
  const long u = (long)blockIdx.x * blockDim.x + threadIdx.x;
  if (u < chunks) pack_pair_chunk(src, dst, dt, mp, (int)u);
}

__global__ __launch_bounds__(256) void pack_batched_kernel(const kair_pack_job* __restrict__ jobs, int njobs,
                                                           const long* __restrict__ first) {
  const long bid = blockIdx.x;
  int lo = 0, hi = njobs - 1;
  while (lo < hi) {
    const int mid = (lo + hi + 1) >> 1;
    if (first[mid] <= bid) lo = mid;
    else hi = mid - 1;
  }
  const kair_pack_job& j = jobs[lo];
  const long t = (bid - first[lo]) * 256 + threadIdx.x;
  if (pack_vec(j.map, j.dst_dtype)) {
    if (t < j.total / 8) pack_chunk(j.src, (bf16*)j.dst, j.map, t);
  } else if (pack_pair_vec(j.map, j.dst_dtype)) {
    if (t < j.total / 16) pack_pair_chunk(j.src, j.dst, j.dst_dtype, j.map, (int)t);
  } else if (t < j.total) {
    pack_element(j.src, j.dst, j.dst_dtype, j.map, t);
  }
}

__global__ __launch_bounds__(1024) void wgrad_finalize_kernel(const float* __restrict__ part, int splits, kair_wmap mp,
                                                              float* grad, float* bias_grad, int ones_col, int acc,
                                                              long nw, long Kt, long plane, int taps) {
  const long t = (long)blockIdx.x * 64 + (threadIdx.x & 63);
  const long nb = bias_grad ? mp.N : 0;
  const bool valid = t < nw + nb;
  long off = 0;
  if (valid) {
    if (t < nw) {
      if (mp.kind == 0) {
        const int n = (int)(t / mp.K), k = (int)(t - (long)n * mp.K);
        const int np = (n / mp.nGr) * mp.nGp + n % mp.nGr, kp = (k / mp.kGr) * mp.kGp + k % mp.kGr;
        off = (long)np * Kt + kp;
      } else {
        const int co = (int)(t / ((long)mp.K * taps));
        const int rem = (int)(t - (long)co * mp.K * taps);
        const int ci = rem / taps, tap = rem - (rem / taps) * taps;
        const int cq = nperm_inv(mp, co);
        const int np = (cq / mp.nGr) * mp.nGp + cq % mp.nGr;
        const int cip = (ci / mp.kGr) * mp.kGp + ci % mp.kGr;
        const int Cip = mp.kG * mp.kGp;
        off = (long)np * Kt + (long)tap * Cip + cip;
      }
    } else {
      const int n = nperm_inv(mp, (int)(t - nw));
      const int np = (n / mp.nGr) * mp.nGp + n % mp.nGr;
      off = (long)np * Kt + ones_col;
    }
  }
  const float s = split_sum16(part, splits, plane, off, valid);
  if (valid && threadIdx.x < 64) {
    float* o = t < nw ? grad + t : bias_grad + (t - nw);
    *o = acc ? *o + s : s;
  }
}

KAIR_DEV void finalize4_body(const float* __restrict__ part, int splits, const kair_wmap& mp, float* grad,
                             float* bias_grad, int ones_col, int acc, long Kt, long plane, int taps, long blk) {
  __shared__ float4 red[4][64];
  const int q = threadIdx.x & 63, ph = threadIdx.x >> 6;
  const long e4 = blk * 64 + q;
  const bool valid = e4 * 4 < plane;
  float4 s = make_float4(0.f, 0.f, 0.f, 0.f);
  if (valid) {
    const float4* p = (const float4*)part + e4;
    const long st = plane / 4;
    for (int sp = ph; sp < splits; sp += 32) {
      float4 v[8];
#pragma unroll
      for (int u = 0; u < 8; ++u) {
        const int spu = sp + 4 * u < splits ? sp + 4 * u : splits - 1;
        v[u] = p[(long)spu * st];
      }
#pragma unroll
      for (int u = 0; u < 8; ++u)
        if (sp + 4 * u < splits) { s.x += v[u].x; s.y += v[u].y; s.z += v[u].z; s.w += v[u].w; }
    }
  }
  red[ph][q] = s;
  __syncthreads();
  if (ph != 0 || !valid) return;
  const float4 a = red[0][q], b = red[1][q], c = red[2][q], d = red[3][q];
  const float t4[4] = {((a.x + b.x) + c.x) + d.x, ((a.y + b.y) + c.y) + d.y, ((a.z + b.z) + c.z) + d.z,
                       ((a.w + b.w) + c.w) + d.w};
  const int Cip = mp.kG * mp.kGp;
#pragma unroll
  for (int j = 0; j < 4; ++j) {
    const long pe = e4 * 4 + j;
    const int np = (int)(pe / Kt);
    const int kk = (int)(pe - (long)np * Kt);
    const int n = nperm_fwd(mp, unpad(np, mp.nG, mp.nGr, mp.nGp));
    if (n < 0) continue;
    float* o = nullptr;
    if (bias_grad && kk == ones_col) {
      o = bias_grad + n;
    } else {
      const int tap = taps == 1 ? 0 : kk / Cip;
      const int k = unpad(taps == 1 ? kk : kk - tap * Cip, mp.kG, mp.kGr, mp.kGp);
      if (k < 0) continue;
      o = grad + ((long)n * mp.K + k) * taps + tap;
    }
    *o = acc ? *o + t4[j] : t4[j];
  }
}

__global__ __launch_bounds__(256) void wgrad_finalize4_kernel(const float* __restrict__ part, int splits, kair_wmap mp,
                                                              float* grad, float* bias_grad, int ones_col, int acc,
                                                              long Kt, long plane, int taps) {
  finalize4_body(part, splits, mp, grad, bias_grad, ones_col, acc, Kt, plane, taps, blockIdx.x);
}

__global__ __launch_bounds__(256) void wgrad_finalize_grouped_kernel(const FinGroup g) {
  const long b = blockIdx.x;
  int ji = 0;
  for (int i = 1; i < g.njobs; ++i)
    if (g.j[i].blk0 <= b) ji = i;
  ji = __builtin_amdgcn_readfirstlane(ji);
  const FinJob& jb = g.j[ji];
  finalize4_body(jb.part, g.splits, jb.mp, jb.grad, jb.bias, jb.ones_col, 0, jb.Kt, jb.plane, 1, b - jb.blk0);
}

template <typename T>
__global__ void row_copy_kernel(const float* __restrict__ src, long lds, T* __restrict__ dst, long ldd,
                                const float* __restrict__ scale, int rps, WinMap wm, long M, int C4) {
  const long i = (long)blockIdx.x * blockDim.x + threadIdx.x;
  if (i >= M * C4) return;
  const long t = i / C4;
  const int c = (int)(i - t * C4) * 4;
  const float4 v = *(const float4*)(src + t * lds + c);
  const float sc = scale ? scale[t / rps] : 1.f;
  T* o = dst + token_to_win(t, wm) * ldd + c;
  if constexpr (sizeof(T) == 2) {
    bf16x4 q = {(bf16)(sc * v.x), (bf16)(sc * v.y), (bf16)(sc * v.z), (bf16)(sc * v.w)};
    *(bf16x4*)o = q;
  } else {
    *(float4*)o = make_float4(sc * v.x, sc * v.y, sc * v.z, sc * v.w);
  }
}

__global__ void row_copy_pair_kernel(const float* __restrict__ src, long lds, f16* __restrict__ hi, f16* __restrict__ lo,
                                     long ldd, const float* __restrict__ scale, int rps, WinMap wm, long M, int C4, float es) {
  const long i = (long)blockIdx.x * blockDim.x + threadIdx.x;
  if (i >= M * C4) return;
  const long t = i / C4;
// ... 213 lines not shown
      const long i = ((long)b * C + c) * HW + pp;
      const float d = E[i] - H[i];
      if constexpr (CH) {
        const float q = sqrtf(d * d + eps);
        s += q;
        g4[c] = q > 0.f ? gscale * d / q : 0.f;
      } else {
        s += fabsf(d);
        g4[c] = d > 0.f ? gscale : (d < 0.f ? -gscale : 0.f);
      }
    }
    *(float4*)(dE + (long)pix * 4) = make_float4(g4[0], g4[1], g4[2], g4[3]);
  }
  red[threadIdx.x] = s;
  __syncthreads();
  for (int o = 128; o > 0; o >>= 1) {
    if (threadIdx.x < o) red[threadIdx.x] += red[threadIdx.x + o];
    __syncthreads();
  }
  if (threadIdx.x == 0) ws[blockIdx.x] = red[0];
}

__global__ void l1_final(const float* __restrict__ ws, int nb, float scale, float* out) {
  __shared__ float red[256];
  float s = 0.f;
  for (int i = threadIdx.x; i < nb; i += 256) s += ws[i];
  red[threadIdx.x] = s;
  __syncthreads();
  for (int o = 128; o > 0; o >>= 1) {
    if (threadIdx.x < o) red[threadIdx.x] += red[threadIdx.x + o];
    __syncthreads();
  }
  if (threadIdx.x == 0) out[0] = red[0] * scale;
}

__global__ void range_check_kernel(const float* __restrict__ g, const float* __restrict__ p, long n,
                                   const float* __restrict__ loss, float p_limit, unsigned* __restrict__ flag) {
  unsigned bits = 0;
  const long n4 = n / 4;
  for (long i = (long)blockIdx.x * blockDim.x + threadIdx.x; i < n4; i += (long)gridDim.x * blockDim.x) {
    const float4 gv = ((const float4*)g)[i];
    const float4 pv = ((const float4*)p)[i];
    const float gs = (gv.x - gv.x) + (gv.y - gv.y) + (gv.z - gv.z) + (gv.w - gv.w);
    if (gs != 0.f) bits |= 1u;
    const float pm = fmaxf(fmaxf(fabsf(pv.x), fabsf(pv.y)), fmaxf(fabsf(pv.z), fabsf(pv.w)));
    if (!(pm < p_limit)) bits |= 4u;
  }
  for (long i = n4 * 4 + (long)blockIdx.x * blockDim.x + threadIdx.x; i < n; i += (long)gridDim.x * blockDim.x) {
    if (g[i] - g[i] != 0.f) bits |= 1u;
    if (!(fabsf(p[i]) < p_limit)) bits |= 4u;
  }
  if (blockIdx.x == 0 && threadIdx.x == 0 && loss && loss[0] - loss[0] != 0.f) bits |= 2u;
  __shared__ unsigned red;
  if (threadIdx.x == 0) red = 0;
  __syncthreads();
  if (bits) atomicOr(&red, bits);
  __syncthreads();
  if (threadIdx.x == 0 && red) atomicOr(flag, red);
}

__global__ void adam_ema_kernel(float* __restrict__ p, const float* __restrict__ g, float* __restrict__ m,
                                float* __restrict__ v, float* __restrict__ ema, long n, const float* __restrict__ lr_t,
                                float b1, float b2, float eps, float wd, float decay, const unsigned* __restrict__ skip) {
  if (skip && *skip) return;
  const float step = lr_t[0], bc2s = lr_t[1];
  for (long i = (long)blockIdx.x * blockDim.x + threadIdx.x; i < n; i += (long)gridDim.x * blockDim.x) {
    float gi = g[i];
    float pi = p[i];
    if (wd != 0.f) gi = gi + wd * pi;
    float mi = m[i];
    mi = mi + (1.f - b1) * (gi - mi);
    float vi = v[i] * b2;
    vi = vi + (1.f - b2) * (gi * gi);
    const float denom = sqrtf(vi) / bc2s + eps;
    pi = pi + (-step) * (mi / denom);
    m[i] = mi;
    v[i] = vi;
    p[i] = pi;
    if (ema) ema[i] = ema[i] * decay + (1.f - decay) * pi;
  }
}

__global__ void axpy_kernel(float* __restrict__ y, const float* __restrict__ x, float a, long n) {
  const long n4 = n / 4;
  for (long i = (long)blockIdx.x * blockDim.x + threadIdx.x; i < n4; i += (long)gridDim.x * blockDim.x) {
    float4 yv = ((float4*)y)[i];
    const float4 xv = ((const float4*)x)[i];
    yv.x += a * xv.x; yv.y += a * xv.y; yv.z += a * xv.z; yv.w += a * xv.w;
    ((float4*)y)[i] = yv;
  }
  for (long i = n4 * 4 + (long)blockIdx.x * blockDim.x + threadIdx.x; i < n; i += (long)gridDim.x * blockDim.x)
    y[i] += a * x[i];
}

__global__ void axpby_kernel(float* __restrict__ y, const float* __restrict__ x, float a, float b, long n) {
  for (long i = (long)blockIdx.x * blockDim.x + threadIdx.x; i < n; i += (long)gridDim.x * blockDim.x)
    y[i] = a * x[i] + b * y[i];
}

__global__ void axpby_rows_kernel(float* __restrict__ y, long ldy, const float* __restrict__ x, long ldx, long M, int C,
                                  float a, float b) {
  const long i = (long)blockIdx.x * blockDim.x + threadIdx.x;
  if (i >= M * C) return;
  const long m = i / C;
  const int c = (int)(i - m * C);
  float* o = y + m * ldy + c;
  *o = a * x[m * ldx + c] + b * *o;
}

template <typename TX, typename TO>
__global__ void act_grad_cast_kernel(const float* __restrict__ G, long ldg, const TX* __restrict__ X, long ldx,
                                     TO* __restrict__ out, long ldo, long M, int C, int kind, float slope, float scale) {
  const long i = (long)blockIdx.x * blockDim.x + threadIdx.x;
  if (i >= M * C) return;
  const long m = i / C;
  const int c = (int)(i - m * C);
  float g = G[m * ldg + c] * scale;
  if (kind == 3) {
    g *= gelu_erf_grad((float)X[m * ldx + c]);
  } else if (kind) {
    const float xv = (float)X[m * ldx + c];
    g = xv > 0.f ? g : (kind == 2 ? g * slope : 0.f);
  }
  out[m * ldo + c] = (TO)g;
}

__global__ void sumpool2x_kernel(const float* __restrict__ src, long lds, float* __restrict__ dst, long ldd, int B, int H,
                                 int W, int C, int acc) {
  const long i = (long)blockIdx.x * blockDim.x + threadIdx.x;
  const long total = (long)B * H * W * C;
  if (i >= total) return;
  const int c = (int)(i % C);
  const long pix = i / C;
  const int x = (int)(pix % W);
  const long by = pix / W;
  const int y = (int)(by % H);
  const long b = by / H;
  const long r0 = (b * 2 * H + 2 * y) * (2L * W) + 2 * x;
  const float s = src[r0 * lds + c] + src[(r0 + 1) * lds + c] + src[(r0 + 2L * W) * lds + c] +
                  src[(r0 + 2L * W + 1) * lds + c];
  float* o = dst + pix * ldd + c;
  *o = acc ? *o + s : s;
}

inline unsigned nblk(long n, int bs) { return (unsigned)((n + bs - 1) / bs); }

}

static int pack_total(const kair_wmap& mp, int dst_dtype, long* total) {
  KAIR_CHECK_ARG((mp.kind != 12 && mp.kind != 15) || dst_dtype == KAIR_BF16,
                 "pack_weight: the hi/lo split forms 12 / 15 are bf16 only");
  KAIR_CHECK_ARG(mp.kind != 9 || dst_dtype == KAIR_BF16 || dst_dtype == KAIR_F16,
                 "pack_weight: kind 9 is a bf16 or (x3) fp16 pair form");
  KAIR_CHECK_ARG(dst_dtype == KAIR_F32 || dst_dtype == KAIR_BF16 || ((mp.kind == 9 || (mp.kind >= 17 && mp.kind <= 21)) &&
                                                                     dst_dtype == KAIR_F16),
                 "pack_weight: fp16 destinations are the x3 pair forms (kinds 9, 17, 18, 19, 20, 21)");
  KAIR_CHECK_ARG(mp.nG > 0 && mp.nGr > 0 && mp.nGp >= mp.nGr && mp.nG * mp.nGr == mp.N, "pack_weight: bad N map");
  KAIR_CHECK_ARG(mp.kind == 4 ||
                     (mp.kG > 0 && mp.kGr > 0 && mp.kGp >= mp.kGr &&
                      (mp.kG * mp.kGr == mp.K ||
                       ((mp.kind == 1 || mp.kind == 9 || mp.kind == 15) && mp.K > 0 && (mp.kG * mp.kGr) % mp.K == 0))),
                 "pack_weight: bad K map");
  KAIR_CHECK_ARG(mp.n_perm <= 1 || (mp.nG == 1 && mp.N % mp.n_perm == 0), "pack_weight: n_perm needs nG == 1, N %% n_perm == 0");
  const long Np = (long)mp.nG * mp.nGp, Kp = (long)mp.kG * mp.kGp;
  KAIR_CHECK_ARG((mp.kind != 10 && mp.kind != 12) || (Np % 32 == 0 && Kp % 16 == 0),
                 "pack_weight: fragment order needs Np %% 32 == 0, Kp %% 16 == 0");
  KAIR_CHECK_ARG(mp.kind != 13 || (Kp % 32 == 0 && Np % 16 == 0), "pack_weight: transposed fragment order needs Kp %% 32 == 0, Np %% 16 == 0");
  KAIR_CHECK_ARG(mp.kind != 14 || (Np % 16 == 0 && Kp % 32 == 0), "pack_weight: 16x16x32 fragment order needs Np %% 16 == 0, Kp %% 32 == 0");
  KAIR_CHECK_ARG(mp.kind != 15 || (Np % 16 == 0 && (9 * Kp) % 32 == 0), "pack_weight: kind 15 needs Np %% 16 == 0, 9 Kp %% 32 == 0");
  KAIR_CHECK_ARG(mp.kind != 16 || (Kp % 16 == 0 && (9 * Np) % 32 == 0), "pack_weight: kind 16 needs Kp %% 16 == 0, 9 Np %% 32 == 0");
  if (mp.kind >= 17 && mp.kind <= 19) {
    KAIR_CHECK_ARG(dst_dtype == KAIR_BF16 || dst_dtype == KAIR_F16, "pack_weight: kinds 17-19 are bf16 / fp16 pairs");
    int base;
    long rowlen, rows;
    split_rows(mp, &base, &rowlen, &rows);
    *total = rows * 2 * ((rowlen + 63) / 64) * 64;
    return 0;
  }
  if (mp.kind == 20 || mp.kind == 21) {
    KAIR_CHECK_ARG(dst_dtype == KAIR_BF16 || dst_dtype == KAIR_F16, "pack_weight: kinds 20 / 21 are bf16 / fp16 pairs");
    KAIR_CHECK_ARG(pack_pair_vec(mp, dst_dtype), "pack_weight: kind 20 needs Kp %% 8 == 0, kind 21 Np %% 8 == 0");
    const long rows = mp.kind == 20 ? Np : 4 * Kp, rowlen = mp.kind == 20 ? 4 * Kp : Np;
    KAIR_CHECK_ARG(rows * ((rowlen + 63) / 64 * 8) < (1L << 31), "pack_weight: kind %d pack too large", mp.kind);
    *total = rows * 2 * ((rowlen + 63) / 64) * 64;
    return 0;
  }
  if (mp.kind == 0 || mp.kind == 3 || mp.kind == 10 || mp.kind == 13 || mp.kind == 14) *total = Np * Kp;
  else if (mp.kind == 12) *total = 2 * Np * Kp;
  else if (mp.kind == 1 || mp.kind == 2 || mp.kind == 16) *total = Np * 9 * Kp;
  else if (mp.kind == 7 || mp.kind == 8) *total = Np * 4 * Kp;
  else if (mp.kind == 9) *total = Np * 2 * ((9L * Kp + 63) / 64) * 64;
  else if (mp.kind == 15) *total = 2 * Np * 9 * Kp;
  else if (mp.kind == 4) *total = Np;
  else return kair_set_error(KAIR_ERR_ARG, "pack_weight: bad kind %d", mp.kind);
  return 0;
}

extern "C" int kair_pack_weight(const float* src, void* dst, int dst_dtype, const kair_wmap* map, void* stream) {
  KAIR_CHECK_ARG(src && dst && map, "pack_weight: null pointer");
  long total;
  if (int rc = pack_total(*map, dst_dtype, &total)) return rc;
  if (map->kind == 20 || map->kind == 21) {
    KAIR_LAUNCH(pack_pair_kernel, dim3(nblk(total / 16, 256)), dim3(256), 0, (hipStream_t)stream, src, dst, dst_dtype,
                       *map, total / 16);
    KAIR_CHECK_LAUNCH();
    return 0;
  }
  KAIR_LAUNCH(pack_kernel, dim3(nblk(total, 256)), dim3(256), 0, (hipStream_t)stream, src, dst, dst_dtype, *map,
                     total);
  KAIR_CHECK_LAUNCH();
  return 0;
}

extern "C" long kair_pack_table_bytes(int njobs) {
  return (long)njobs * (long)sizeof(kair_pack_job) + (long)(njobs + 1) * (long)sizeof(long);
}

extern "C" long kair_pack_table_build(kair_pack_job* jobs, int njobs, void* table_dev) {
  KAIR_CHECK_ARG(jobs && table_dev && njobs > 0, "pack_table_build: bad args");
  const size_t jb = (size_t)njobs * sizeof(kair_pack_job);
  char* host = (char*)malloc(jb + (size_t)(njobs + 1) * sizeof(long));
  if (!host) return kair_set_error(KAIR_ERR_ARG, "pack_table_build: out of host memory");
  long* first = (long*)(host + jb);
  long nb = 0;
  for (int i = 0; i < njobs; ++i) {
    long total;
    int rc = jobs[i].src && jobs[i].dst ? pack_total(jobs[i].map, jobs[i].dst_dtype, &total)
                                        : kair_set_error(KAIR_ERR_ARG, "pack_table_build: job %d null pointer", i);
    if (rc) { free(host); return rc; }
    jobs[i].total = total;
    first[i] = nb;
    const long items = pack_vec(jobs[i].map, jobs[i].dst_dtype) ? total / 8
                       : pack_pair_vec(jobs[i].map, jobs[i].dst_dtype) ? total / 16 : total;
    if (items >= (1L << 31)) { free(host); return kair_set_error(KAIR_ERR_ARG, "pack_table_build: job %d too large", i); }
    nb += (items + 255) / 256;
  }
  first[njobs] = nb;
  memcpy(host, jobs, jb);
  const hipError_t e = hipMemcpy(table_dev, host, jb + (size_t)(njobs + 1) * sizeof(long), hipMemcpyHostToDevice);
  free(host);
  if (e != hipSuccess) return kair_set_error(KAIR_ERR_HIP, "pack_table_build: %s", hipGetErrorString(e));
  return nb;
}

extern "C" int kair_pack_weights(const void* table_dev, int njobs, long nblocks, void* stream) {
  KAIR_CHECK_ARG(table_dev && njobs > 0 && nblocks > 0, "pack_weights: bad args");
  const kair_pack_job* jobs = (const kair_pack_job*)table_dev;
  const long* first = (const long*)((const char*)table_dev + (size_t)njobs * sizeof(kair_pack_job));
  KAIR_LAUNCH(pack_batched_kernel, dim3((unsigned)nblocks), dim3(256), 0, (hipStream_t)stream, jobs, njobs, first);
  KAIR_CHECK_LAUNCH();
  return 0;
}

int kair_launch_finalize_grouped(const FinGroup& g, hipStream_t s) {
  KAIR_LAUNCH(wgrad_finalize_grouped_kernel, dim3((unsigned)g.nblocks), dim3(256), 0, s, g);
  KAIR_CHECK_LAUNCH();
  return 0;
}

extern "C" int kair_wgrad_finalize(const float* partial, int splits, const kair_wmap* map, float* grad_ref,
                                   float* bias_grad, int ones_col, int accumulate, void* stream) {
  KAIR_CHECK_ARG(partial && map && grad_ref && splits > 0, "wgrad_finalize: null pointer");
  const kair_wmap& mp = *map;
  KAIR_CHECK_ARG(mp.kind == 0 || mp.kind == 1 || mp.kind == 7,
                 "wgrad_finalize: kind must be 0 (linear), 1 (conv3x3) or 7 (conv2x2)");
  KAIR_CHECK_ARG(!bias_grad || ones_col >= 0, "wgrad_finalize: bias needs ones_col");
  KAIR_CHECK_ARG(mp.n_perm <= 1 || (mp.nG == 1 && mp.N % mp.n_perm == 0), "wgrad_finalize: n_perm needs nG == 1");
  const int taps = mp.kind == 0 ? 1 : (mp.kind == 1 ? 9 : 4);
  const long Np = (long)mp.nG * mp.nGp;
  const long Kt = (long)taps * mp.kG * mp.kGp;
  const long nw = (long)mp.N * mp.K * taps;
  const long tot = nw + (bias_grad ? mp.N : 0);
  if ((Np * Kt) % 4 == 0 && ((uintptr_t)partial % 16) == 0) {
    KAIR_LAUNCH(wgrad_finalize4_kernel, dim3(nblk(Np * Kt / 4, 64)), dim3(256), 0, (hipStream_t)stream, partial,
                       splits, mp, grad_ref, bias_grad, ones_col, accumulate, Kt, Np * Kt, taps);
  } else {
    KAIR_LAUNCH(wgrad_finalize_kernel, dim3(nblk(tot, 64)), dim3(1024), 0, (hipStream_t)stream, partial, splits, mp,
                       grad_ref, bias_grad, ones_col, accumulate, nw, Kt, Np * Kt, taps);
  }
  KAIR_CHECK_LAUNCH();
  return 0;
}

extern "C" int kair_row_copy(const float* src, long lds, long M, int C, const kair_copy_desc* copy, void* stream) {
  KAIR_CHECK_ARG(src && copy && copy->out && M > 0 && C > 0, "row_copy: bad args");
  KAIR_CHECK_ARG(C % 4 == 0 && lds % 4 == 0 && copy->ld % 4 == 0, "row_copy: widths must be multiples of 4");
  KAIR_CHECK_ARG(M < KAIR_MAX_MAPPED_ROWS, "row_copy: M must be < 2^24");
  KAIR_CHECK_ARG(copy->win_ws == 0 || (copy->win_H % copy->win_ws == 0 && copy->win_W % copy->win_ws == 0),
                 "row_copy: window geometry");
  const WinMap wm = make_winmap(copy->win_H, copy->win_W, copy->win_ws, copy->win_shift);
  const int rps = copy->rows_per_scale > 0 ? copy->rows_per_scale : 1;
  const long n = M * (C / 4);
  hipStream_t s = (hipStream_t)stream;
  if (copy->dtype == KAIR_F16) {
    KAIR_CHECK_ARG(copy->out_lo && ((uintptr_t)copy->out % 8) == 0 && ((uintptr_t)copy->out_lo % 8) == 0,
                   "row_copy: an fp16 pair copy needs its 8-byte aligned lo plane (out_lo)");
    KAIR_LAUNCH(row_copy_pair_kernel, dim3(nblk(n, 256)), dim3(256), 0, s, src, lds, (f16*)copy->out,
                       (f16*)copy->out_lo, copy->ld, copy->rowscale, rps, wm, M, C / 4, ldexpf(1.f, copy->x3_exp));
  } else if (copy->dtype == KAIR_BF16)
    KAIR_LAUNCH(row_copy_kernel<bf16>, dim3(nblk(n, 256)), dim3(256), 0, s, src, lds, (bf16*)copy->out, copy->ld,
                       copy->rowscale, rps, wm, M, C / 4);
  else
    KAIR_LAUNCH(row_copy_kernel<float>, dim3(nblk(n, 256)), dim3(256), 0, s, src, lds, (float*)copy->out, copy->ld,
                       copy->rowscale, rps, wm, M, C / 4);
  KAIR_CHECK_LAUNCH();
  return 0;
}

extern "C" int kair_colsum(const kair_operand* G, long M, int Np, const kair_wmap* map, float* bias_grad, float* ws,
                           int accumulate, void* stream) {
  KAIR_CHECK_ARG(G && G->ptr && map && bias_grad && ws, "colsum: null pointer");
  KAIR_CHECK_ARG(G->mode == KAIR_LD_ROWS && G->win_ws == 0, "colsum: plain row operands only");
  const int nb = 512;
  const long rows_per = (M + nb - 1) / nb;
  dim3 grid(nb, (Np + 255) / 256);
  hipStream_t s = (hipStream_t)stream;
  const bool vec = Np % 8 == 0 && Np <= 256 && G->ld % 8 == 0 && ((uintptr_t)G->ptr & 15) == 0;
  if (vec && G->dtype == KAIR_BF16)
    KAIR_LAUNCH(colsum_partial_v<bf16>, dim3(nb), dim3(256), 0, s, (const bf16*)G->ptr, G->ld, M, Np, ws, rows_per);
  else if (vec)
    KAIR_LAUNCH(colsum_partial_v<float>, dim3(nb), dim3(256), 0, s, (const float*)G->ptr, G->ld, M, Np, ws, rows_per);
  else if (G->dtype == KAIR_BF16)
    KAIR_LAUNCH(colsum_partial<bf16>, grid, dim3(256), 0, s, (const bf16*)G->ptr, G->ld, M, Np, ws, rows_per);
  else
    KAIR_LAUNCH(colsum_partial<float>, grid, dim3(256), 0, s, (const float*)G->ptr, G->ld, M, Np, ws, rows_per);
  KAIR_CHECK_LAUNCH();
  KAIR_LAUNCH(colsum_final, dim3(nblk(map->N, 8)), dim3(256), 0, s, ws, nb, Np, *map, bias_grad, accumulate);
  KAIR_CHECK_LAUNCH();
  return 0;
}

extern "C" int kair_image_to_nhwc(const float* img, void* out, int dtype, int ldc, const float* mean, float img_range,
                                  int B, int C, int H, int W, void* stream) {
  KAIR_CHECK_ARG(img && out && ldc >= C, "image_to_nhwc: bad args");
  const long total = (long)B * H * W * ldc;
  hipStream_t s = (hipStream_t)stream;
  if (dtype == KAIR_BF16)
    KAIR_LAUNCH(image_to_nhwc_kernel<bf16>, dim3(nblk(total, 256)), dim3(256), 0, s, img, (bf16*)out, ldc, mean,
                       img_range, C, (long)H * W, total);
  else
    KAIR_LAUNCH(image_to_nhwc_kernel<float>, dim3(nblk(total, 256)), dim3(256), 0, s, img, (float*)out, ldc, mean,
                       img_range, C, (long)H * W, total);
  KAIR_CHECK_LAUNCH();
  return 0;
}

extern "C" int kair_image_to_nhwc_hilo(const float* img, void* out, int ldc, const float* mean, float img_range, int B,
                                       int C, int H, int W, void* stream) {
  KAIR_CHECK_ARG(img && out && ldc % 2 == 0 && 2 * C <= ldc, "image_to_nhwc_hilo: needs 2 * C <= ldc (even)");
  const long total = (long)B * H * W * ldc;
  KAIR_LAUNCH(image_to_nhwc_hilo_kernel, dim3(nblk(total, 256)), dim3(256), 0, (hipStream_t)stream, img, (bf16*)out,
                     ldc, mean, img_range, C, (long)H * W, total);
  KAIR_CHECK_LAUNCH();
  return 0;
}
// ... 245 lines not shown
```

kair_amd/engine/swinir_engine.py:

```python
import contextlib
import math
import os
import weakref

import torch

from .. import _hip as H
from .plans import Lease, PlanPool, autograd_mode, plan_mode

WINDOW_SIZES = (7, 8)


def _rup(x, m):
    return (x + m - 1) // m * m


def swinir_flops(net, Hh, Ww):
    C = net.embed_dim
    HW = Hh * Ww
    f = 2 * HW * 9 * net.conv_first.in_channels * C
    def resi(m):
        if isinstance(m, torch.nn.Sequential):
            q = m[0].out_channels
            return 2 * HW * (9 * C * q + q * q + 9 * q * C)
        return 2 * HW * 9 * C * C

    for layer in net.layers:
        for blk in layer.residual_group.blocks:
            Hd = blk.mlp.fc1.out_features
            f += 2 * HW * C * 3 * C + 2 * HW * C * C
            f += 2 * 2 * HW * (blk.window_size ** 2) * C
            f += 2 * 2 * HW * C * Hd
        f += resi(layer.conv)
    f += resi(net.conv_after_body)
    first_dgrad = 2 * HW * 9 * net.conv_first.in_channels * C
    if net.upsampler == "nearest+conv":
        nf = 64
        f += 2 * HW * 9 * C * nf + 2 * (4 * HW + 16 * HW + 16 * HW) * 9 * nf * nf + 2 * 16 * HW * 9 * nf * net.conv_last.out_channels
    elif net.upsampler in (None, ""):
        f += 2 * HW * 9 * C * net.conv_last.out_channels
    elif net.upsampler == "pixelshuffle":
        nf = 64
        f += 2 * HW * 9 * C * nf
        hw = HW
        for m in net.upsample:
            if isinstance(m, torch.nn.Conv2d):
                f += 2 * hw * 9 * nf * m.out_channels
                hw *= m.out_channels // nf
        f += 2 * hw * 9 * nf * net.conv_last.out_channels
    else:
        conv = net.upsample[0]
        f += 2 * HW * 9 * C * conv.out_channels
    return {"fwd": f, "train": 3 * f - first_dgrad}


class _Lin:

    def __init__(self, eng, mod, n_grp, k_grp, frag=False, split=False, frag_t=False, rows=True, frag16=False):
        self.w, self.b = mod.weight, mod.bias
        N, K = self.w.shape[:2]
        self.N, self.K = N, K
        self.map = H.wmap(0, N, K, n_grp, k_grp)
        self.mapT = H.wmap(3, N, K, n_grp, k_grp)
        self.mapb = H.wmap(4, N, 0, n_grp, (1, 1, 1))
        self.Np = n_grp[0] * n_grp[2]
        self.Kp = k_grp[0] * k_grp[2]
        dev = self.w.device
        self.x3 = getattr(eng, "x3", False)
        if self.x3:
            self.pmap, self.pmapT = H.wmap(17, N, K, n_grp, k_grp), H.wmap(19, N, K, n_grp, k_grp)
            self.Wp = torch.empty(self.Np, 2 * _rup(self.Kp, 64), device=dev, dtype=torch.float16) if rows else None
            self.Wt = torch.empty(self.Kp, 2 * _rup(self.Np, 64), device=dev, dtype=torch.float16) if not frag_t else None
        else:
            self.pmap, self.pmapT = self.map, self.mapT
            self.Wp = torch.empty(self.Np, self.Kp, device=dev, dtype=eng.tdt) if rows else None
            self.Wt = torch.empty(self.Kp, self.Np, device=dev, dtype=eng.tdt) if not frag_t else None
        self.bp = torch.empty(self.Np, device=dev)
        self.split = bool(frag and split)
        self.mapg = H.wmap(12 if self.split else (14 if frag16 else 10), N, K, n_grp, k_grp) if frag else None
        self.Wg = (torch.empty((2 if self.split else 1) * self.Np, self.Kp, device=dev, dtype=eng.tdt)
                   if frag else None)
        self.mapgt = H.wmap(13, N, K, n_grp, k_grp) if frag_t else None
        self.Wgt = torch.empty(self.Kp, self.Np, device=dev, dtype=eng.tdt) if frag_t else None

    def pack_jobs(self):
        w, b = self.w.detach(), self.b.detach()
        jobs = [(b, self.bp, self.mapb)]
        if self.Wp is not None:
            jobs.append((w, self.Wp, self.pmap))
        if self.Wt is not None:
            jobs.append((w, self.Wt, self.pmapT))
        if self.Wg is not None:
            jobs.append((w, self.Wg, self.mapg))
        if self.Wgt is not None:
            jobs.append((w, self.Wgt, self.mapgt))
        return jobs


class _Conv:

    def __init__(self, eng, mod, Cop, Cip, need_dgrad=True, split=None, n_perm=0, tied_in=False, fwd_cip=None,
                 narrow=False, wr=False):
        self.w, self.b = mod.weight, mod.bias
        Co, Ci = self.w.shape[:2]
        self.Co, self.Ci, self.Cop, self.Cip = Co, Ci, Cop, Cip
        if split is None:
            split = getattr(eng, "split_conv", False)
        x3 = getattr(eng, "x3", False)
        self.split = (bool(split) and eng.tdt == torch.bfloat16) or x3
        self.x3 = x3
        self.n_perm = n_perm
        self.map = H.wmap(1, Co, Ci, (1, Co, Cop), (1, Ci, Cip), n_perm=n_perm)
        fcip = fwd_cip or Cip
        self.fcip = fcip
        kf_grp = (2, Ci, fcip // 2) if tied_in else (1, Ci, Cip)
        self.mapf = H.wmap(9 if self.split else 1, Co, Ci, (1, Co, Cop), kf_grp, n_perm=n_perm)
        self.mapd = H.wmap(2, Co, Ci, (1, Co, Cop), (1, Ci, Cip), n_perm=n_perm)
        self.mapb = H.wmap(4, Co, 0, (1, Co, Cop), (1, 1, 1), n_perm=n_perm)
        dev = self.w.device
        kf = 2 * _rup(9 * fcip, 64) if self.split else 9 * fcip
        self.Wf = torch.empty(Cop, kf, device=dev, dtype=torch.float16 if self.x3 else
                              (torch.bfloat16 if self.split else eng.tdt))
        self.narrow = bool(narrow)
        if self.narrow:
            self.mapn = H.wmap(15, Co, Ci, (1, Co, 16), (1, Ci, Cip))
            self.Wn = torch.empty(16, 2 * 9 * Cip, device=dev, dtype=torch.bfloat16)
        if self.x3:
            self.mapd = H.wmap(18, Co, Ci, (1, Co, Cop), (1, Ci, Cip), n_perm=n_perm)
            self.Wd = torch.empty(Cip, 2 * _rup(9 * Cop, 64), device=dev, dtype=torch.float16) if need_dgrad else None
        else:
            self.Wd = torch.empty(Cip, 9 * Cop, device=dev, dtype=eng.tdt) if need_dgrad else None
        self.bp = torch.empty(Cop, device=dev)
        self.wr = bool(wr) and Cop == 192 and Cip == 192 and self.split
        self.wr_pair = bool(wr) and not self.wr and tied_in and Cip == 64 and fcip == 128 and Cop == 256 and self.split
        if self.wr_pair:
            self.mapp = H.wmap(15, Co, Ci, (1, Co, Cop), (1, Ci, Cip), n_perm=n_perm)
            self.Wp15 = torch.empty(Cop * 2 * 9 * Cip, device=dev, dtype=torch.bfloat16)
            self.mapp16 = H.wmap(16, Co, Ci, (1, Co, Cop), (1, Ci, Cip), n_perm=n_perm)
            self.Wp16 = torch.empty(Cip * 9 * Cop, device=dev, dtype=torch.bfloat16)
        self.wr_n64 = bool(wr) and not self.wr and not self.wr_pair and Cop == 64 and Cip == 192 and self.split and not tied_in
        if self.wr_n64:
            self.mapc = H.wmap(15, Co, Ci, (1, Co, Cop), (1, Ci, Cip))
            self.Wc15 = torch.empty(Cop * 2 * 9 * Cip, device=dev, dtype=torch.bfloat16)
            self.mapc16 = H.wmap(16, Co, Ci, (1, Co, Cop), (1, Ci, Cip))
            self.Wc16 = torch.empty(Cip * 9 * Cop, device=dev, dtype=torch.bfloat16)
        if self.wr:
            self.map15 = H.wmap(15, Co, Ci, (1, Co, Cop), (1, Ci, Cip))
            self.Wf15 = torch.empty(Cop * 2 * 9 * Cip, device=dev, dtype=torch.bfloat16)
            self.map16 = H.wmap(16, Co, Ci, (1, Co, Cop), (1, Ci, Cip))
            self.Wd16 = torch.empty(Cip * 9 * Cop, device=dev, dtype=torch.bfloat16)

    def fwd(self):
        return H.rows(self.Wf, w_split=self.split)

    def pack_jobs(self):
        w, b = self.w.detach(), self.b.detach()
        jobs = [(w, self.Wf, self.mapf), (b, self.bp, self.mapb)]
        if self.Wd is not None:
            jobs.append((w, self.Wd, self.mapd))
        if self.narrow:
            jobs.append((w, self.Wn, self.mapn))
        if self.wr:
            jobs += [(w, self.Wf15, self.map15), (w, self.Wd16, self.map16)]
        if self.wr_pair:
            jobs += [(w, self.Wp15, self.mapp), (w, self.Wp16, self.mapp16)]
        if self.wr_n64:
            jobs += [(w, self.Wc15, self.mapc), (w, self.Wc16, self.mapc16)]
        return jobs


class _Resi3:

    def __init__(self, eng, seq):
        C = seq[0].in_channels
        q = seq[0].out_channels
        self.q, self.Cq = q, _rup(q, 8)
        self.c1 = _Conv(eng, seq[0], self.Cq, eng.Cp)
        self.c2 = _Lin(eng, seq[2], (1, q, self.Cq), (1, q, self.Cq))
        self.c3 = _Conv(eng, seq[4], eng.Cp, self.Cq)
        assert C == eng.C and seq[4].out_channels == C

    def pack_jobs(self):
        return self.c1.pack_jobs() + self.c2.pack_jobs() + self.c3.pack_jobs()


def _resi(eng, m):
    if isinstance(m, torch.nn.Sequential):
        return _Resi3(eng, m)
    return _Conv(eng, m, eng.Cp, eng.Cp, wr=getattr(eng, "conv_wr", False))


class _Blk:
    def __init__(self, eng, blk):
        C, Cp, nh = eng.C, eng.Cp, eng.nh
        hd = C // nh
        self.mod = blk
        self.shift = blk.shift_size
        self.dp = blk.drop_path_rate
        self.n1, self.n2 = blk.norm1, blk.norm2
        self.table = blk.attn.relative_position_bias_table
        self.scale = blk.attn.scale
        Hd = blk.mlp.fc1.out_features
        sp = eng.split_linear
        fa, fm, fb, rg = eng.fused_attn, eng.fused_mlp, eng.fused_mlp_bwd, eng.rowgemm
        hp = eng.hp
        self.qkv = _Lin(eng, blk.attn.qkv, (3 * nh, hd, hp), (1, C, Cp), frag=fa, split=sp, rows=not fa, frag_t=rg)
        self.proj = _Lin(eng, blk.attn.proj, (1, C, Cp), (nh, hd, hp), frag=fa, split=sp, rows=not fa, frag_t=rg)
        self.fc1 = _Lin(eng, blk.mlp.fc1, (1, Hd, eng.Hdp), (1, C, Cp), frag=fm, split=sp, frag_t=fb or rg, rows=not fm)
        self.fc2 = _Lin(eng, blk.mlp.fc2, (1, C, Cp), (1, Hd, eng.Hdp), frag=fm, split=sp, frag_t=fb or rg, rows=not fm,
                        frag16=True)

    def linears(self):
        return (self.qkv, self.proj, self.fc1, self.fc2)


class SwinIREngine:
    def __init__(self, net, compute_dtype="bf16", split_conv=True, fused_blocks=True, fused_mlp=None,
                 split_linear=None, fused_mlp_bwd=False, side_stream=True, side_ctas=None, side_priority=0,
                 split_act=True, conv_wr=True, head_pad=None, grouped_wgrad=None):
        self.net_ref = weakref.ref(net)
        if compute_dtype not in ("bf16", "fp32", "fp32x3"):
            raise ValueError(compute_dtype)
        self.x3 = compute_dtype == "fp32x3"
        self._ax = 0
        self.X3_AEXP = 4
        self.x3_gexp_off = 4
        self.x3_backoffs = 0
        self.cd = H.BF16 if compute_dtype in ("bf16", "fp32x3") else H.F32
        self.tn_cd = H.X3 if self.x3 else self.cd
        self.tdt = torch.bfloat16 if compute_dtype == "bf16" else torch.float32
        self.split_conv = bool(split_conv) and compute_dtype == "bf16"
        self.split_act = bool(split_act) and self.split_conv
        self.C = net.embed_dim
        heads = {l.residual_group.blocks[0].num_heads for l in net.layers}
        if len(heads) != 1:
            raise NotImplementedError("kair_amd SwinIR: per-stage head counts must match")
        self.nh = heads.pop()
        hd = self.C // self.nh
        if hd >= 32 or self.C % self.nh:
            raise NotImplementedError("kair_amd SwinIR: head_dim must be < 32")
        self.ws = net.window_size
        if self.ws not in WINDOW_SIZES:
            raise NotImplementedError(f"kair_amd SwinIR: window_size {self.ws}: the attention kernels are built for "
                                      f"window sizes 7 and 8")
        self.T = self.ws * self.ws
        ws8 = self.ws == 8
        self.Cp = _rup(self.C + 1, 32)
        self.fused_attn = (bool(fused_blocks) and compute_dtype == "bf16" and self.nh == 6 and self.Cp == 32 * self.nh
                           and ws8)
        Hd = net.layers[0].residual_group.blocks[0].mlp.fc1.out_features
        self.Hdp = _rup(Hd + 1, 32)
        if fused_mlp is None:
            fused_mlp = fused_blocks
        self.fused_mlp = bool(fused_mlp) and compute_dtype == "bf16" and self.Cp == 192 and self.Hdp == 384 and ws8
        hp16 = (compute_dtype == "bf16" and hd < 16 and not self.fused_attn and not (self.Cp == 192 and self.Hdp == 384)
                and ws8)
        self.hp = 16 if hp16 and head_pad in (None, 16) else 32
        if head_pad not in (None, 16, 32) or (head_pad == 16 and self.hp != 16):
            raise ValueError(f"head_pad {head_pad}: 32, or 16 for bf16 head dims below 16 on the unfused path")
        self.fused_mlp_bwd = (bool(fused_blocks) and compute_dtype == "bf16" and self.Cp == 192 and self.Hdp == 384
                              and bool(fused_mlp_bwd) and ws8)
        self.split_linear = bool(split_linear) and compute_dtype == "bf16"
        self.rowgemm = (compute_dtype == "bf16" and self.Cp == 192 and self.Hdp == 384 and self.nh * self.hp == self.Cp
                        and ws8)
        self.upsampler, self.scale = net.upsampler, net.upscale
        self.in_ch = net.conv_first.in_channels
        self.img_range = float(net.img_range)
        self.Cin_p = 8
        self.xin_hilo = self.split_act and 2 * self.in_ch <= self.Cin_p
        self.conv_wr = bool(conv_wr) and self.split_act and self.Cp == 192 and self.C % 4 == 0
        self.device = net.conv_first.weight.device
        dev = self.device
        self.mean = net.mean.view(-1).to(dev, torch.float32).contiguous()
        self.conv_first = _Conv(self, net.conv_first, self.Cp, self.Cin_p, need_dgrad=False, tied_in=self.xin_hilo)
        self.pe_norm = net.patch_embed.norm
        self.rstb = []
        for layer in net.layers:
            blks = [_Blk(self, b) for b in layer.residual_group.blocks]
            self.rstb.append((blks, _resi(self, layer.conv)))
        self.norm = net.norm
        self.cab = _resi(self, net.conv_after_body)
        nf = 64
        self.last_narrow_x3 = False
        if self.upsampler == "pixelshuffle":
            self.cbu = _Conv(self, net.conv_before_upsample[0], nf, self.Cp, wr=self.conv_wr)
            self.ups = []
            for m in net.upsample:
                if isinstance(m, torch.nn.Conv2d):
                    self.ups.append(_Conv(self, m, m.out_channels, nf, n_perm=m.out_channels // nf,
                                          tied_in=self.split_act, fwd_cip=2 * nf if self.split_act else None,
                                          wr=self.conv_wr))
            self.ups_r = [int(math.isqrt(c.Co // nf)) for c in self.ups]
            self.last_narrow = self.tdt == torch.bfloat16 and self.split_conv and self.in_ch <= 4
            self.last = _Conv(self, net.conv_last, 16, nf, narrow=self.last_narrow)
            self.last_narrow_x3 = self.x3 and self.in_ch <= 4
        elif self.upsampler == "pixelshuffledirect":
            conv = net.upsample[0]
            self.ups_r = [self.scale]
            self.up1 = _Conv(self, conv, _rup(conv.out_channels, 16), self.Cp)
        elif self.upsampler == "nearest+conv":
            self.cbu = _Conv(self, net.conv_before_upsample[0], nf, self.Cp)
            self.nup = [_Conv(self, net.conv_up1, nf, nf), _Conv(self, net.conv_up2, nf, nf)]
            self.hrc = _Conv(self, net.conv_hr, nf, nf)
            self.last = _Conv(self, net.conv_last, 16, nf)
        elif self.upsampler in (None, ""):
            self.last = _Conv(self, net.conv_last, 16, self.Cp)
        else:
            raise NotImplementedError(self.upsampler)
        self.blocks = [b for blks, _ in self.rstb for b in blks]
        self.plans = PlanPool(self._build_plan)
        self.plan_mode = "primary"
        self._packed_version = None
        self._pack_table = None
        self.seg_hook = None
        self.grouped_wgrad = (grouped_wgrad is not False and self.tdt == torch.bfloat16 and self.Hdp <= 576 and
                              3 * self.nh * self.hp <= 576 and
                              max(len(l.residual_group.blocks) for l in net.layers) <= H.WgradGroup.WG_MAX // 4)
        self._wg_pending = []
        self._lnp_pending = []
        self._dtab_pending = []
        self._conv_pending = []
        self._side = None
        self.x3_side = self.x3 and self.Hdp <= 576
        self.side_stream = (self.grouped_wgrad or self.x3_side) and torch.cuda.is_available() and bool(side_stream)
        self.side_priority = side_priority
        self.side_ctas_auto = side_ctas is None and self.x3
        if side_ctas is None:
            side_ctas = 192 if self.x3 else 0
        self.x3_grouped = self.x3_side and os.environ.get("KAIR_X3_GROUPED", "1") != "0"
        self.x3_lnfuse = (self.x3 and self.Cp == 192 and self.C % 4 == 0 and not self.rowgemm and not fused_mlp_bwd and
                          os.environ.get("KAIR_X3_LNFUSE", "0") == "1")
        self.side_ctas = int(side_ctas)
        self.conv_tap = self.tdt == torch.bfloat16 and self.Cp == 192 and self.C % 4 == 0
        self.conv_wr_min_tiles = 64

    def grad_segments(self):
        net = self.net_ref()
        tail = list(net.norm.parameters()) + list(net.conv_after_body.parameters())
        if self.upsampler == "pixelshuffle":
            tail += (list(net.conv_before_upsample.parameters()) + list(net.upsample.parameters()) +
                     list(net.conv_last.parameters()))
        elif self.upsampler == "nearest+conv":
            tail += [p for m in (net.conv_before_upsample, net.conv_up1, net.conv_up2, net.conv_hr, net.conv_last)
                     for p in m.parameters()]
        elif self.upsampler in (None, ""):
            tail += list(net.conv_last.parameters())
        else:
            tail += list(net.upsample.parameters())
        segs = [tail]
        for gi in range(len(net.layers) - 1, 0, -1):
            segs.append(list(net.layers[gi].parameters()))
        segs.append(list(net.conv_first.parameters()) + list(net.patch_embed.parameters()) +
                    list(net.layers[0].parameters()))
        return segs

    def _segment_done(self):
        if self.seg_hook is not None:
            self.seg_hook()

    def convs(self):
        cs = [self.conv_first] + [c for _, c in self.rstb] + [self.cab]
        if self.upsampler == "pixelshuffle":
            cs += [self.cbu] + self.ups + [self.last]
        elif self.upsampler == "nearest+conv":
            cs += [self.cbu] + self.nup + [self.hrc, self.last]
        elif self.upsampler in (None, ""):
            cs += [self.last]
        else:
            cs += [self.up1]
        return cs

    def pack(self, force=False):
        net = self.net_ref()
        force = force or getattr(self, "repack_always", False)
        ver = None if force else tuple(p._version for p in net.parameters())
        if ver is not None and ver == self._packed_version:
            return
        ptrs = tuple(p.data_ptr() for p in net.parameters())
        if self._pack_table is None or self._pack_table[0] != ptrs:
            jobs = [j for c in self.convs() for j in c.pack_jobs()]
            jobs += [j for b in self.blocks for l in b.linears() for j in l.pack_jobs()]
            self._pack_table = (ptrs, H.PackTable(jobs))
        self._pack_table[1].run()
        self._packed_version = ver

    def plan(self, B, Hh, Ww):
        return self.plans.get((B, Hh, Ww), self.plan_mode)

    def _build_plan(self, key, infer):
        B, Hh, Ww = key
        dev, T, f32 = self.device, self.tdt, torch.float32
        M = B * Hh * Ww
        Cp, Hdp, nh, hp = self.Cp, self.Hdp, self.nh, self.hp
        if Hh % self.ws or Ww % self.ws:
            raise ValueError(f"kair_amd SwinIR: the {Hh}x{Ww} token grid is no multiple of window_size {self.ws}")
        nWin = M // self.T
        e = lambda *s, dt=f32: torch.empty(*s, device=dev, dtype=dt)
        hf = torch.float16
        P = {"B": B, "H": Hh, "W": Ww, "M": M, "nWin": nWin}
        P["e_g"] = self._x3_grad_exp(B * self.in_ch * Hh * self.scale * Ww * self.scale)
        P["xin"] = e(M, self.Cin_p, dt=T)
        P["f0"] = e(M, Cp)
        P["pe_mean"], P["pe_rstd"] = e(M), e(M)
        P["s0"] = e(M, Cp)
        blocks = []
        for bi in range(len(self.blocks)):
            if infer and bi >= 2:
                blocks.append(blocks[bi % 2])
                continue
            pr = (lambda *sh: e(2, *sh, dt=hf)) if self.x3 else (lambda *sh: e(*sh, dt=T))
            blocks.append({
                "mid": e(M, Cp), "out": e(M, Cp), "ln1": pr(M, Cp), "m1": e(M), "r1": e(M),
                "qkv": e(2, 3 * M * nh * hp, dt=hf) if self.x3 else e(3 * M * nh * hp, dt=T),
                "O": pr(M, nh * hp), "lse": e(nWin * nh * self.T),
                "ln2": pr(M, Cp), "m2": e(M), "r2": e(M), "u": e(M, Hdp, dt=T), "h": pr(M, Hdp)})
        P["blocks"] = blocks
        P["rstb_out"] = [e(M, Cp) for _ in range(min(2, len(self.rstb)) if infer else len(self.rstb))]
        if infer:
            P["rstb_out"] = [P["rstb_out"][i % len(P["rstb_out"])] for i in range(len(self.rstb))]
        P["nf"], P["n_mean"], P["n_rstd"] = e(M, Cp), e(M), e(M)
        P["fb"] = e(M, Cp)
        if self.upsampler == "pixelshuffle":
            nf = 64
            tl = P["tail_ld"] = 2 * nf if self.split_act else nf
            P["a0"] = e(M, tl, dt=T)
            acts, hw = [], M
            for r in self.ups_r:
                hw *= r * r
                acts.append(e(hw, tl, dt=T))
            P["ups_act"] = acts
            P["M_hr"] = hw
            if self.last_narrow_x3:
                P["narrow_fws"] = e(H.conv3x3_narrow_x3_ws())
        elif self.upsampler == "nearest+conv":
            nf = 64
            P["a0"] = e(M, nf, dt=T)
            P["nup_act"] = [e(4 * M, nf, dt=T), e(16 * M, nf, dt=T)]
            P["nhr"] = e(16 * M, nf, dt=T)
            P["M_hr"] = 16 * M
        P["r3"] = {id(r): (e(M, r.Cq, dt=T), e(M, r.Cq, dt=T)) for r in [c for _, c in self.rstb] + [self.cab]
                   if isinstance(r, _Resi3)}
        P["E"] = e(B, self.in_ch, Hh * self.scale, Ww * self.scale)
        P["infer"] = infer
        if infer:
            return P
        z32 = lambda *s: torch.zeros(*s, device=dev, dtype=f32)
        P["D"], P["G"] = z32(M, Cp), z32(M, Cp)
        P["dxn"] = e(M, Cp, dt=T)
        if self.fused_mlp_bwd:
            P["mlp_ws"] = e(H.swin_mlp_bwd_ws())
        depth = max(len(blks) for blks, _ in self.rstb)
        z = lambda *s: torch.zeros(*s, device=dev, dtype=T)
        zp = (lambda *sh: torch.zeros(2, *sh, device=dev, dtype=hf)) if self.x3 else z
        ep = (lambda *sh: e(2, *sh, dt=hf)) if self.x3 else (lambda *sh: e(*sh, dt=T))
        lnp = max(2 * 2048 * Cp, 2 * self.C * H.gemm_nt_lnbwd_parts(M, Cp) if self.x3_lnfuse else 0)
        P["gw"] = [[{"Dm": zp(M, Cp), "Da": zp(M, Cp), "dU": ep(M, Hdp),
                     "dqkv": ep(M, 3 * nh * hp) if self.x3 else e(3 * M * nh * hp, dt=T),
                     "ln1p": e(lnp), "ln2p": e(lnp), "attn_ws": e(H.window_attn_bwd_ws(nWin, nh, self.ws))}
                    for _ in range(depth)] for _ in range(2)]
        P["G3"] = z32(M, Cp)
        if self.rowgemm:
            P["rg_nb"] = {k: H.rowgemm_ln_blocks(M, k) for k in (Hdp, 3 * nh * hp)}
            assert max(P["rg_nb"].values()) <= 2048, P["rg_nb"]
        P["dO"] = e(2, M, nh * hp, dt=hf) if self.x3 else e(M, nh * hp, dt=T)
        P["ln_ws"] = e(2 * 2048 * Cp)
        P["attn_ws"] = e(H.window_attn_bwd_ws(nWin, nh, self.ws))
        P["loss"] = e(1)
        P["loss_ws"] = e(1024)
        P["colsum_ws"] = e(1024 * 256)
        if self.upsampler == "pixelshuffle":
            P["dE_ld"] = 4 if self.last_narrow_x3 and (Ww * self.scale) % 64 == 0 else 16
            P["dE"] = e(P["M_hr"], P["dE_ld"], dt=T)
            if self.last.narrow or self.last_narrow_x3:
                P["narrow_ws"] = e(H.conv3x3_narrow_wgrad_ws(self.in_ch))
                P["narrow_dws"] = e(H.conv3x3_narrow_x3_ws() if self.x3 else H.conv3x3_narrow_dgrad_ws())
            dpre, hw = [], M
            for c in self.ups:
                dpre.append(e(hw, c.Co, dt=T))
                hw *= c.Co // 64
            P["dpre"] = dpre
            P["da0"] = e(M, 64, dt=T)
        elif self.upsampler == "nearest+conv":
            nf = 64
            P["dE"] = e(16 * M, 16, dt=T)
            P["dz_hr"], P["dz_u"] = e(16 * M, nf, dt=T), e(16 * M, nf, dt=T)
            P["G_hi"], P["G_lo"] = e(16 * M, nf), e(4 * M, nf)
            P["da0"] = e(M, nf, dt=T)
        elif self.upsampler in (None, ""):
            P["dE"] = e(M, 16, dt=T)
        else:
            P["dE"] = e(M, self.up1.Cop, dt=T)
        if P["r3"]:
            q = max(r.Cq for r in [c for _, c in self.rstb] + [self.cab] if isinstance(r, _Resi3))
            P["r3_dz"] = (e(M, q, dt=T), e(M, q, dt=T))
        P["dfb"] = e(M, Cp)
        if self.conv_tap:
            P["conv_halo"] = H.conv_halo_geometry(Hh, Ww, Cp, M, Cp)
            P["conv_wr"] = bool(self.conv_wr and H.conv3x3_wr_tile(1, B, Hh, Ww, Cp, Cp) > 0 and
                                H.conv3x3_wr_tile(0, B, Hh, Ww, Cp, Cp) > 0 and M // 96 >= self.conv_wr_min_tiles)
            if P["conv_wr"]:
                P["conv_halo"] = True
            P["conv_bf"] = {}
            for r in [c for _, c in self.rstb] + [self.cab]:
                if not isinstance(r, _Resi3):
                    P["conv_bf"][id(r)] = (torch.zeros(M, Cp, device=dev, dtype=T), torch.zeros(M, Cp, device=dev, dtype=T))
                    P["conv_bf"][id(r)][1][:, self.C] = 1.0
        P["wg_ws"] = e(self._max_wgrad_ws(M, P))
        P["wg_ws2"] = (e(P["wg_ws"].numel() * max(1, -self.side_ctas)) if self.grouped_wgrad or self.side_stream
                       else None)
        return P

    def _wgrad_shapes(self, M, P):
        Cp, Hdp, nh = self.Cp, self.Hdp, self.nh
        out = [(M, Cp, 9 * self.Cin_p)]

        def resi(r):
            if isinstance(r, _Resi3):
                return [(M, r.Cq, 9 * Cp), (M, r.Cq, r.Cq), (M, Cp, 9 * r.Cq)]
            return [(M, Cp, 9 * Cp)]

        for blks, conv in self.rstb:
            for _ in blks:
                out += [(M, Cp, Hdp), (M, Hdp, Cp), (M, Cp, nh * self.hp), (M, 3 * nh * self.hp, Cp)]
            out += resi(conv)
        out += resi(self.cab)
        if self.upsampler == "nearest+conv":
            out += [(M, 64, 9 * Cp), (4 * M, 64, 9 * 64), (16 * M, 64, 9 * 64), (16 * M, 64, 9 * 64),
                    (16 * M, 16, 9 * 64)]
        elif self.upsampler in (None, ""):
            out.append((M, 16, 9 * Cp))
        elif self.upsampler == "pixelshuffle":
            out.append((M, 64, 9 * Cp))
            hw = M
            for c in self.ups:
                out.append((hw, c.Co, 9 * 64))
                hw *= c.Co // 64
            out.append((hw, 16, 9 * 64))
        else:
            out.append((M, self.up1.Cop, 9 * Cp))
        return out

    def _max_wgrad_ws(self, M, P):
        ws = max(H.wgrad_splits(m, n, k) * n * k for m, n, k in self._wgrad_shapes(M, P))
        if self.grouped_wgrad or self.x3_grouped:
            Cp, Hdp, nh = self.Cp, self.Hdp, self.nh
            depth = max(len(blks) for blks, _ in self.rstb)
            shapes = [(Cp, Hdp), (Hdp, Cp), (Cp, nh * self.hp), (3 * nh * self.hp, Cp)] * depth
            for i in range(0, len(shapes), H.WgradGroup.WG_MAX):
                ws = max(ws, H.wgrad_grouped_ws(shapes[i:i + H.WgradGroup.WG_MAX], M, x3=self.x3))
        return ws

    def forward(self, x, drop_scales=None):
        B, _, Hh, Ww = x.shape
        P = self.plan(B, Hh, Ww)
        self.pack()
        cd, T = self.cd, self.tdt
        M, Cp, nh = P["M"], self.Cp, self.nh
        HW = Hh * Ww
        x = x.contiguous()
        self.cur = P
        self._ax = self.X3_AEXP
        P["x"] = x
        P["drop"] = drop_scales
        if self.xin_hilo:
            H.image_to_nhwc_hilo(x, P["xin"], self.Cin_p, self.mean, self.img_range, B, self.in_ch, Hh, Ww)
        else:
            H.image_to_nhwc(x, P["xin"], self.Cin_p, self.mean, self.img_range, B, self.in_ch, Hh, Ww)
        c = self.conv_first
        self._nt(H.im2col(P["xin"], Hh, Ww, self.Cin_p), c.fwd(), H.epilogue(P["f0"], bias=c.bp), M, Cp,
                  9 * self.Cin_p, cd)
        n = self.pe_norm
        H.layernorm_fwd(P["f0"], Cp, P["s0"], Cp, n.weight, n.bias, P["pe_mean"], P["pe_rstd"], M, self.C, n.eps)
        cur = P["s0"]
        bi = 0
        for gi, (blks, conv) in enumerate(self.rstb):
            g_in = cur
            for blk in blks:
                cur = self._block_fwd(blk, P, P["blocks"][bi], cur, bi)
                bi += 1
            out = P["rstb_out"][gi]
            self._resi_fwd(conv, P, cur, out, g_in)
            cur = out
        n = self.norm
        H.layernorm_fwd(cur, Cp, P["nf"], Cp, n.weight, n.bias, P["n_mean"], P["n_rstd"], M, self.C, n.eps)
        self._resi_fwd(self.cab, P, P["nf"], P["fb"], P["f0"])
        return self._forward_tail(P)

    def _resi_fwd(self, r, P, src, out, resid):
        cd, Cp, M, Hh, Ww = self.cd, self.Cp, P["M"], P["H"], P["W"]
        if not isinstance(r, _Resi3):
            ac = (P["conv_bf"][id(r)][1], self.C) if P.get("conv_halo") else None
            if P.get("conv_wr") and r.wr:
                assert src.dtype == torch.float32 and resid.dtype == torch.float32
                H.conv3x3_wr(src, Cp, 0, r.Wf15, r.bp, resid, out, P["B"], Hh, Ww, Cp, Cp, acopy=ac[0], acones=ac[1],
                             split=True)
                return
            self._nt(self._ain(H.im2col(src, Hh, Ww, Cp)), r.fwd(), H.epilogue(out, bias=r.bp, resid=resid, acopy=ac), M,
                      Cp, 9 * Cp, cd)
            return
        t1, t2 = P["r3"][id(r)]
        lk = dict(act=H.ACT_LEAKY, slope=0.2)
        self._nt(H.im2col(src, Hh, Ww, Cp), r.c1.fwd(), H.epilogue(t1, bias=r.c1.bp, **lk), M, r.Cq, 9 * Cp, cd)
        self._nt(H.rows(t1), H.rows(r.c2.Wp), H.epilogue(t2, bias=r.c2.bp, **lk), M, r.Cq, r.Cq, cd)
        self._nt(H.im2col(t2, Hh, Ww, r.Cq), r.c3.fwd(), H.epilogue(out, bias=r.c3.bp, resid=resid), M, Cp, 9 * r.Cq, cd)

    def _resi_bwd(self, r, P, G, src, D, grads):
        cd, Cp, M, Hh, Ww = self.cd, self.Cp, P["M"], P["H"], P["W"]
        g = lambda p: grads[p]
        if not isinstance(r, _Resi3):
            ac = (P["conv_bf"][id(r)][0], -1) if P.get("conv_halo") else None
            if P.get("conv_wr") and r.wr:
                H.conv3x3_wr(G, Cp, 1, r.Wd16, None, None, D, P["B"], Hh, Ww, Cp, Cp, acopy=ac[0], split=False)
            else:
                self._nt(H.im2col(G, Hh, Ww, Cp, flip=True), H.rows(r.Wd), H.epilogue(D, acopy=ac), M, Cp, 9 * Cp, cd)
            if self.conv_tap:
                return ("tap", G, src, r, g(r.w), g(r.b))
            return (H.rows(G), H.im2col(src, Hh, Ww, Cp, ones_col=self.C), M, Cp, 9 * Cp, r.map, g(r.w), g(r.b), self.C)
        t1, t2 = P["r3"][id(r)]
        q = r.Cq
        lk = dict(gate_kind=2, slope=0.2)
        dz2 = P["r3_dz"][0].view(-1)[:M * q].view(M, q)
        dz1 = P["r3_dz"][1].view(-1)[:M * q].view(M, q)
        self._nt(H.im2col(G, Hh, Ww, Cp, flip=True), H.rows(r.c3.Wd), H.epilogue(dz2, gate=t2, **lk), M, q, 9 * Cp, cd)
        self._wgrad(P, H.rows(G), H.im2col(t2, Hh, Ww, q), M, Cp, 9 * q, r.c3.map, g(r.c3.w))
        self._bias_colsum(P, H.rows(G), M, Cp, r.c3.mapb, g(r.c3.b))
        self._nt(H.rows(dz2), H.rows(r.c2.Wt), H.epilogue(dz1, gate=t1, **lk), M, q, q, cd)
        self._wgrad(P, H.rows(dz2), H.rows(t1), M, q, q, r.c2.map, g(r.c2.w))
        self._bias_colsum(P, H.rows(dz2), M, q, r.c2.mapb, g(r.c2.b))
        self._nt(H.im2col(dz1, Hh, Ww, q, flip=True), H.rows(r.c1.Wd), H.epilogue(D), M, Cp, 9 * q, cd)
        self._wgrad(P, H.rows(dz1), H.im2col(src, Hh, Ww, Cp), M, q, 9 * Cp, r.c1.map, g(r.c1.w))
        self._bias_colsum(P, H.rows(dz1), M, q, r.c1.mapb, g(r.c1.b))
        return None

    @staticmethod
    def _op(t, **kw):
        if t.dtype == torch.float16 and t.dim() == 3 and t.shape[0] == 2:
            return H.with_lo(H.rows(t[0], **kw), t[1])
        return H.rows(t, **kw)

    def _ain(self, op, lo=None):
        return H.asplit(op, lo) if self.split_act else op

    def _nt_lnbwd(self, A, B, M, K, x, gamma, mean, rstd, D, part, win=(0, 0, 0, 0), copy=None):
        A.x3_exp, B.x3_exp = self._ax, H.X3_WEXP
        H.gemm_nt_lnbwd(A, B, M, self.Cp, K, x, self.Cp, gamma, mean, rstd, self.C, D, self.Cp, part, win=win, copy=copy)

    def _nt(self, A, B, E, M, N, K, cd):
        if self.x3:
            if A.dtype == H.F16 and not A.lo_ptr:
                raise RuntimeError("fp32x3: an fp16 GEMM operand needs its lo plane")
            A.x3_exp, B.x3_exp = self._ax, H.X3_WEXP
            if A.ones_col >= 0:
                raise RuntimeError("fp32x3: no injected ones column on a GEMM A operand")
            if E.out_dtype == H.F16:
                E.x3_out_exp = self._ax
            H.gemm_nt(A, B, E, M, N, K, H.X3)
            return
        H.gemm_nt(A, B, E, M, N, K, cd)

    X3_AEXP = 4
    X3_BACKOFF_STEP = 6
    X3_BACKOFF_MAX = 4

    def _x3_grad_exp(self, numel, weight=1.0):
        return int(round(math.log2(max(numel, 1) / max(abs(weight), 1e-30)))) + self.x3_gexp_off

    def x3_backoff(self, step=None, act=True, grad=True):
        if not self.x3:
            raise RuntimeError("x3_backoff: not an fp32x3 engine")
        if self.x3_backoffs >= self.X3_BACKOFF_MAX:
            raise RuntimeError(f"fp32x3 range guard: the step is still non-finite after {self.x3_backoffs} exponent "
                               f"back-offs (activation 2^{self.X3_AEXP}, gradient offset 2^{self.x3_gexp_off}): the data "
                               f"is not finite, or a weight left its pack window |w| < 2^{16 - H.X3_WEXP}")
        step = self.X3_BACKOFF_STEP if step is None else int(step)
        if act:
            self.X3_AEXP -= step
        if grad:
            self.x3_gexp_off -= step
        self.x3_backoffs += 1
        return self.X3_AEXP, self.x3_gexp_off

    def _forward_tail(self, P):
        cd, Cp, M, B, Hh, Ww = self.cd, self.Cp, P["M"], P["B"], P["H"], P["W"]
        sa = self.split_act
        if self.upsampler == "pixelshuffle":
            tl = P["tail_ld"]
            lo = (lambda t: t[:, 64:]) if sa else (lambda t: None)
            c = self.cbu
            if (c.wr_n64 and self.conv_wr and H.conv3x3_wr_tile(1, B, Hh, Ww, Cp, 64) > 0 and
                    M // 96 >= self.conv_wr_min_tiles):
                H.conv3x3_wr(P["fb"], Cp, 0, c.Wc15, c.bp, None, P["a0"], B, Hh, Ww, Cp, 64, ldo=tl, split=True,
                             out_lo=lo(P["a0"]), act=H.ACT_LEAKY, slope=0.01)
            else:
                self._nt(self._ain(H.im2col(P["fb"], Hh, Ww, Cp)), c.fwd(),
                          H.epilogue(P["a0"], ldo=tl, bias=c.bp, act=H.ACT_LEAKY, slope=0.01, out_lo=lo(P["a0"])), M, 64,
                          9 * Cp, cd)
            src, h, w = P["a0"], Hh, Ww
            for c, r, dst in zip(self.ups, self.ups_r, P["ups_act"]):
                if (c.wr_pair and self.conv_wr and H.conv3x3_wr_tile(1, B, h, w, 64, c.Co) > 0 and
                        B * h * w // 96 >= self.conv_wr_min_tiles):
                    H.conv3x3_wr(src, tl, 0, c.Wp15, c.bp, None, dst, B, h, w, 64, c.Co, ldo=tl, split=True,
                                 out_lo=lo(dst), ps_r=r)
                    src, h, w = dst, h * r, w * r
                    continue
                A = H.asplit(H.im2col(src, h, w, c.fcip), pair=True) if sa else H.im2col(src, h, w, 64)
                self._nt(A, c.fwd(), H.epilogue(dst, mode=H.OUT_PSHUF_SPM, ldo=tl, bias=c.bp, ps=(r, h, w), out_lo=lo(dst)),
                          B * h * w, c.Co, 9 * c.fcip, cd)
                src, h, w = dst, h * r, w * r
            c = self.last
            if self.last_narrow_x3 and w % 64 == 0:
                H.conv3x3_narrow_fwd_x3(src, tl, self.X3_AEXP, c.w.detach(), c.bp, self.in_ch, P["narrow_fws"], self.mean,
                                        self.img_range, None, P["E"], B, h, w)
                return P["E"]
            if c.narrow and w % 64 == 0:
                H.conv3x3_narrow_fwd(src, tl, 64 if sa else 0, c.Wn, c.bp, self.in_ch, self.mean, self.img_range, None,
                                     P["E"], B, h, w)
                return P["E"]
            self._nt(self._ain(H.im2col(src, h, w, 64, ld=tl), lo(src)), c.fwd(),
                      H.epilogue(P["E"], mode=H.OUT_NCHW, ldo=0, bias=c.bp, img=(self.mean, self.img_range, self.in_ch, h, w)),
                      B * h * w, c.Cop, 9 * 64, cd)
        elif self.upsampler == "nearest+conv":
            c = self.cbu
            self._nt(H.im2col(P["fb"], Hh, Ww, Cp), c.fwd(),
                      H.epilogue(P["a0"], bias=c.bp, act=H.ACT_LEAKY, slope=0.01), M, 64, 9 * Cp, cd)
            src, h, w = P["a0"], Hh, Ww
            for c, dst in zip(self.nup, P["nup_act"]):
                h, w = 2 * h, 2 * w
                self._nt(H.im2col(src, h, w, 64, up=2), c.fwd(), H.epilogue(dst, bias=c.bp, act=H.ACT_LEAKY, slope=0.2),
                          B * h * w, 64, 9 * 64, cd)
                src = dst
            c = self.hrc
            self._nt(H.im2col(src, h, w, 64), c.fwd(), H.epilogue(P["nhr"], bias=c.bp, act=H.ACT_LEAKY, slope=0.2),
                      B * h * w, 64, 9 * 64, cd)
            c = self.last
            self._nt(H.im2col(P["nhr"], h, w, 64), c.fwd(),
                      H.epilogue(P["E"], mode=H.OUT_NCHW, ldo=0, bias=c.bp, img=(self.mean, self.img_range, self.in_ch, h, w)),
                      B * h * w, c.Cop, 9 * 64, cd)
        elif self.upsampler in (None, ""):
            c = self.last
            self._nt(self._ain(H.im2col(P["fb"], Hh, Ww, Cp)), c.fwd(),
                      H.epilogue(P["E"], mode=H.OUT_NCHW, ldo=0, bias=c.bp, resid=P["x"],
                                 img=(None, self.img_range, self.in_ch, Hh, Ww)), M, c.Cop, 9 * Cp, cd)
        else:
            c = self.up1
            self._nt(self._ain(H.im2col(P["fb"], Hh, Ww, Cp)), c.fwd(),
                      H.epilogue(P["E"], mode=H.OUT_PSHUF_NCHW, ldo=0, bias=c.bp, ps=(self.scale, Hh, Ww),
                                 img=(self.mean, self.img_range, self.in_ch, Hh, Ww)), M, c.Cop, 9 * Cp, cd)
        return P["E"]

    def _block_fwd(self, blk, P, S, x, bi):
        cd = self.cd
        M, Cp, nh, hp, Hh, Ww = P["M"], self.Cp, self.nh, self.hp, P["H"], P["W"]
        HW = Hh * Ww
        win = (Hh, Ww, self.ws, blk.shift)
        drop = P["drop"]
        s_attn = drop[bi, 0] if drop is not None else None
        s_mlp = drop[bi, 1] if drop is not None else None
        if self.fused_attn:
            H.swin_attn_fwd(x, Cp, blk.n1.weight, blk.n1.bias, blk.n1.eps, self.C, S["ln1"], Cp, S["m1"], S["r1"],
                            blk.qkv.Wg, blk.qkv.bp, S["qkv"], blk.table, blk.scale, S["O"], nh * 32, self.C // nh,
                            S["lse"], blk.proj.Wg, blk.proj.bp, s_attn, HW, S["mid"], Cp, P["nWin"], nh, Hh, Ww,
                            blk.shift, w_split=blk.qkv.split)
        else:
            if self.x3:
# ... 478 lines not shown
```

Before: 653.7.

## Add fp16-pair x3 path to the fused halo conv3x3 kernel

Extends the shared-memory halo 3x3 conv kernel with an fp16 hi/lo split mode (x3) that scales activations by a power of two, runs three fp16 MFMAs per step, and rescales the output. Adds new weight pack kinds 22/23 that lay the fp16 pairs out in MFMA fragment order. The SwinIR engine now routes forward and data-gradient RSTB convs through this kernel when running in x3 mode, instead of the im2col GEMM path. This is meant to avoid im2col traffic and GEMM overhead in fp32x3 training, but it depends on fp16 exponent scaling staying accurate and only applies to C=192 geometries.

```diff
diff --git a/include/kair_hip.h b/include/kair_hip.h
--- a/include/kair_hip.h
+++ b/include/kair_hip.h
@@ -223,6 +223,11 @@
                        const float* bias, const float* resid, long ldr, void* out, int out_dtype, long ldo, void* out_lo,
                        int ps_r, int act, float slope, const void* gate, long ldg, void* acopy, long ldac, int acones,
                        int B, int H, int W, int C, int N, void* stream);
+
+int kair_conv3x3_wr_x3_tile(int B, int H, int W, int C, int N);
+int kair_conv3x3_wr_x3(const float* x, long ldx, int ea, int flip, const void* w, int n_blocks, const float* bias,
+                       const float* resid, long ldr, float* out, long ldo, int B, int H, int W, int C, int N,
+                       void* stream);
 
 int kair_conv3x3_narrow_fwd(const void* x, long ldx, int lo_off, const void* w, const float* bias, int NR,
                             const float* mean, float img_range, const float* resid, float* out, int B, int H, int W,
diff --git a/kair_amd/_hip.py b/kair_amd/_hip.py
--- a/kair_amd/_hip.py
+++ b/kair_amd/_hip.py
@@ -149,6 +149,9 @@
     "kair_conv3x3_wr_ex": [c_vp, c_int, c_long, c_int, c_int, c_vp, c_int, c_vp, c_vp, c_long, c_vp, c_int, c_long, c_vp,
                            c_int, c_int, c_float, c_vp, c_long, c_vp, c_long, c_int, c_int, c_int, c_int, c_int, c_int,
                            c_vp],
+    "kair_conv3x3_wr_x3_tile": [c_int, c_int, c_int, c_int, c_int],
+    "kair_conv3x3_wr_x3": [c_vp, c_long, c_int, c_int, c_vp, c_int, c_vp, c_vp, c_long, c_vp, c_long, c_int, c_int, c_int,
+                           c_int, c_int, c_vp],
     "kair_conv3x3_narrow_dgrad_ws": [],
     "kair_conv3x3_narrow_dgrad": [c_vp, c_long, c_vp, c_int, c_vp, c_vp, c_int, c_long, c_int, c_int, c_int, c_int, c_vp],
     "kair_conv3x3_narrow_wgrad_ws": [c_int],
@@ -617,6 +620,18 @@
                                    acones, B, H, W, C, N, stream_ptr()), "conv3x3_wr")
 
 
+def conv3x3_wr_x3_tile(B, H, W, C, N):
+    return lib().kair_conv3x3_wr_x3_tile(B, H, W, C, N)
+
+
+def conv3x3_wr_x3(x, ldx, x3_exp, flip, w, bias, resid, out, B, H, W, C, N, ldr=None, ldo=None):
+    if x.dtype != torch.float32 or out.dtype != torch.float32 or w.dtype != torch.float16:
+        raise TypeError("conv3x3_wr_x3: fp32 rows in and out, fp16 packed weights")
+    check(lib().kair_conv3x3_wr_x3(ptr(x), ldx, int(x3_exp), int(flip), ptr(w), 12, ptr(bias), ptr(resid),
+                                   ldr if ldr is not None else (resid.shape[-1] if resid is not None else 0), ptr(out),
+                                   ldo if ldo is not None else out.shape[-1], B, H, W, C, N, stream_ptr()), "conv3x3_wr_x3")
+
+
 def conv3x3_narrow_dgrad_ws():
     return lib().kair_conv3x3_narrow_dgrad_ws()
 
diff --git a/kair_amd/csrc/conv_wr.hip b/kair_amd/csrc/conv_wr.hip
--- a/kair_amd/csrc/conv_wr.hip
+++ b/kair_amd/csrc/conv_wr.hip
@@ -20,6 +20,7 @@
   int act; float slope;
   const bf16* gate; long ldg;
   int psH, psW;
+  float ascale, oscale;
   int B, H, W, C, N, flip;
   long tilesM;
   FDiv fc8, fhwd;
@@ -29,14 +30,24 @@
   static constexpr int HALO = SPLIT ? 40000 : 80000;
 };
 
-template <typename TX, bool SPLIT, int BM, bool RESID, int RN, int EM>
+KAIR_DEV f32x4 wr_mfma(const bf16x8& w, const bf16x8& x, f32x4 c) {
+  return __builtin_amdgcn_mfma_f32_16x16x32_bf16(w, x, c, 0, 0, 0);
+}
+KAIR_DEV f32x4 wr_mfma(const f16x8& w, const f16x8& x, f32x4 c) {
+  return __builtin_amdgcn_mfma_f32_16x16x32_f16(w, x, c, 0, 0, 0);
+}
+
+template <typename TX, bool SPLIT, int BM, bool RESID, int RN, int EM, typename TH = bf16>
 __global__ __launch_bounds__(WR_NT, 1) void conv3x3_wr_kernel(const ConvWrArgs a) {
   constexpr bool PAIR = SPLIT && sizeof(TX) == 2;
+  constexpr bool X3 = sizeof(TH) == 2 && !__is_same(TH, bf16);
+  static_assert(!X3 || (SPLIT && sizeof(TX) == 4 && EM == 0), "fp16-pair form: fp32 image, split, row output");
+  typedef typename V8<TH>::t th8;
   constexpr int RM = BM / 16;
   constexpr int HALO = WrGeom<SPLIT>::HALO;
   constexpr int NB = SPLIT ? 2 : 1;
-  __shared__ __attribute__((aligned(16))) bf16 sH[SPLIT ? 2 * HALO : HALO];
-  bf16* const sLo = sH + (SPLIT ? HALO : 0);
+  __shared__ __attribute__((aligned(16))) TH sH[SPLIT ? 2 * HALO : HALO];
+  TH* const sLo = sH + (SPLIT ? HALO : 0);
   const int tid = threadIdx.x, lane = tid & 63, wave = __builtin_amdgcn_readfirstlane(tid >> 6);
   const int fr = lane & 15, fq = lane >> 4;
   const int H = a.H, W = a.W, C = a.C;
@@ -55,9 +66,9 @@
     const int ry = p / XW, rx = p - (p / XW) * XW;
     hb[i] = ((ry + 1) * HWD + rx + 1) * PS + fq * 8;
   }
-  const bf16* wb = a.w + ((long)(RN * wave) * KS * NB) * 512 + lane * 8;
+  const TH* wb = (const TH*)a.w + ((long)(RN * wave) * KS * NB) * 512 + lane * 8;
   auto wfrag = [&](int rn, int s, int half) {
-    return *(const bf16x8*)(wb + (((long)rn * KS + s) * NB + half) * 512);
+    return *(const th8*)(wb + (((long)rn * KS + s) * NB + half) * 512);
   };
   float4 bias4[RN];
 #pragma unroll
@@ -67,14 +78,14 @@
   }
 
   constexpr int PD = WrPD<RN, SPLIT>::PD, UNR = WrPD<RN, SPLIT>::UNR;
-  bf16x8 rb[PD][RN][NB];
+  th8 rb[PD][RN][NB];
   auto issue_w = [&](int slot, int s) {
 #pragma unroll
     for (int rn = 0; rn < RN; ++rn)
 #pragma unroll
       for (int h = 0; h < NB; ++h) rb[slot][rn][h] = wfrag(rn, s, h);
   };
-  bf16x8 ra[2][RM][NB];
+  th8 ra[2][RM][NB];
   auto read_a = [&](int buf, int s) {
     const int tap = s / cpsP, c0 = (s - tap * cpsP) * 32;
     int dy = tap / 3 - 1, dx = tap - (tap / 3) * 3 - 1;
@@ -82,8 +93,8 @@
     const int off = (dy * HWD + dx) * PS + c0;
 #pragma unroll
     for (int i = 0; i < RM; ++i) {
-      ra[buf][i][0] = *(const bf16x8*)(sH + hb[i] + off);
-      if constexpr (SPLIT) ra[buf][i][1] = *(const bf16x8*)(sLo + hb[i] + off);
+      ra[buf][i][0] = *(const th8*)(sH + hb[i] + off);
+      if constexpr (SPLIT) ra[buf][i][1] = *(const th8*)(sLo + hb[i] + off);
     }
   };
 
@@ -146,11 +157,17 @@
           if constexpr (sizeof(TX) == 4) {
             const float4 u = __builtin_bit_cast(float4, v0[i]), v = __builtin_bit_cast(float4, v1[i]);
             const float f[8] = {u.x, u.y, u.z, u.w, v.x, v.y, v.z, v.w};
-            bf16x8 hh, ll;
+            th8 hh, ll;
 #pragma unroll
             for (int e = 0; e < 8; ++e) {
-              hh[e] = (bf16)f[e];
-              if constexpr (SPLIT) ll[e] = (bf16)(f[e] - (float)hh[e]);
+              if constexpr (X3) {
+                const float w = opaque(f[e] * a.ascale);
+                hh[e] = (TH)w;
+                ll[e] = (TH)(w - (float)hh[e]);
+              } else {
+                hh[e] = (TH)f[e];
+                if constexpr (SPLIT) ll[e] = (TH)(f[e] - (float)hh[e]);
+              }
             }
             qh = __builtin_bit_cast(uint4, hh);
             if constexpr (SPLIT) ql = __builtin_bit_cast(uint4, ll);
@@ -161,7 +178,7 @@
           if (!okv[i]) qh = ql = make_uint4(0, 0, 0, 0);
           *(uint4*)(sH + pix * PS + c8 * 8) = qh;
           if constexpr (SPLIT) *(uint4*)(sLo + pix * PS + c8 * 8) = ql;
-          if (a.acopy) {
+          if (!X3 && a.acopy) {
             const int hr = fdiv(pix, a.fhwd), hc = pix - hr * HWD;
             if (hr >= 1 && hr <= RPT && hc >= 1 && hc <= XW) {
               uint4 qc = qh;
@@ -189,10 +206,10 @@
       for (int i = 0; i < RM; ++i)
 #pragma unroll
         for (int rn = 0; rn < RN; ++rn) {
-          acc[i][rn] = __builtin_amdgcn_mfma_f32_16x16x32_bf16(rb[ws][rn][0], ra[ab][i][0], acc[i][rn], 0, 0, 0);
+          acc[i][rn] = wr_mfma(rb[ws][rn][0], ra[ab][i][0], acc[i][rn]);
           if constexpr (SPLIT) {
-            acc[i][rn] = __builtin_amdgcn_mfma_f32_16x16x32_bf16(rb[ws][rn][1], ra[ab][i][0], acc[i][rn], 0, 0, 0);
-            acc[i][rn] = __builtin_amdgcn_mfma_f32_16x16x32_bf16(rb[ws][rn][0], ra[ab][i][1], acc[i][rn], 0, 0, 0);
+            acc[i][rn] = wr_mfma(rb[ws][rn][1], ra[ab][i][0], acc[i][rn]);
+            acc[i][rn] = wr_mfma(rb[ws][rn][0], ra[ab][i][1], acc[i][rn]);
           }
         }
       issue_w(ws, wstep(s + PD < KSP ? s + PD : KSP - 1));
@@ -212,6 +229,7 @@
         const int n = 16 * RN * wave + 16 * rn + 4 * fq;
         if (n >= a.N) continue;
         const float4 bb = bias4[rn];
+        if constexpr (X3) acc[i][rn] *= a.oscale;
         float v[4] = {acc[i][rn][0] + bb.x, acc[i][rn][1] + bb.y, acc[i][rn][2] + bb.z, acc[i][rn][3] + bb.w};
         if constexpr (RESID) {
           v[0] += ex[i][rn].x; v[1] += ex[i][rn].y; v[2] += ex[i][rn].z; v[3] += ex[i][rn].w;
@@ -237,7 +255,7 @@
           const int yl = yy / r, xl = xx / r;
           o = (((long)bi * a.psH + yl) * a.psW + xl) * a.ldo + ((yy - yl * r) * r + (xx - xl * r)) * a.N + n;
         }
-        if (a.odt == KAIR_BF16) {
+        if (!X3 && a.odt == KAIR_BF16) {
           const bf16x4 hv = {(bf16)v[0], (bf16)v[1], (bf16)v[2], (bf16)v[3]};
           *(bf16x4*)((bf16*)a.out + o) = hv;
           if (a.out_lo)
@@ -340,6 +358,7 @@
   a.out_lo = (bf16*)out_lo; a.ps_r = pr;
   a.gate = (const bf16*)gate; a.ldg = ldg;
   a.psH = pr ? H / pr : 0; a.psW = pr ? W / pr : 0;
+  a.ascale = a.oscale = 1.f;
   KAIR_CHECK_ARG(act == KAIR_ACT_NONE || (act == KAIR_ACT_LEAKY && !resid && !gate),
                  "conv3x3_wr: act none, or LeakyReLU without residual / gate");
   a.act = act; a.slope = slope;
@@ -391,3 +410,48 @@
   return kair_conv3x3_wr_ex(x, x_dtype, ldx, split, flip, w, n_blocks, bias, resid, ldr, out, out_dtype, ldo, nullptr, 0,
                             KAIR_ACT_NONE, 0.f, nullptr, 0, acopy, ldac, acones, B, H, W, C, N, stream);
 }
+
+extern "C" int kair_conv3x3_wr_x3_tile(int B, int H, int W, int C, int N) {
+  if (N <= 64 || N > 192) return 0;
+  return kair_conv3x3_wr_tile(1, B, H, W, C, N);
+}
+
+extern "C" int kair_conv3x3_wr_x3(const float* x, long ldx, int ea, int flip, const void* w, int n_blocks,
+                                  const float* bias, const float* resid, long ldr, float* out, long ldo, int B, int H,
+                                  int W, int C, int N, void* stream) {
+  KAIR_CHECK_ARG(x && w && out && B > 0, "conv3x3_wr_x3: null operand");
+  KAIR_CHECK_ARG(ea > -100 && ea < 100, "conv3x3_wr_x3: image exponent out of range");
+  const int BM = kair_conv3x3_wr_x3_tile(B, H, W, C, N);
+  KAIR_CHECK_ARG(BM == 48 || BM == 96, "conv3x3_wr_x3: unsupported geometry (B %d, H %d, W %d, C %d, N %d)", B, H, W, C, N);
+  KAIR_CHECK_ARG(n_blocks == 12, "conv3x3_wr_x3: the packed weight needs 192 output rows (12 blocks of 16), got %d blocks",
+                 n_blocks);
+  KAIR_CHECK_ARG(ldx >= C && ldx % 4 == 0 && ((uintptr_t)x & 15) == 0 && ((uintptr_t)w & 15) == 0,
+                 "conv3x3_wr_x3: image rows 16-byte aligned, ldx >= C");
+  KAIR_CHECK_ARG(ldo >= N && ldo % 4 == 0 && ((uintptr_t)out & 15) == 0, "conv3x3_wr_x3: output rows");
+  KAIR_CHECK_ARG(!resid || (ldr >= N && ldr % 4 == 0 && ((uintptr_t)resid & 15) == 0), "conv3x3_wr_x3: residual rows");
+  KAIR_CHECK_ARG(!bias || ((uintptr_t)bias & 15) == 0, "conv3x3_wr_x3: bias alignment");
+  const long M = (long)B * H * W;
+  KAIR_CHECK_ARG(M * (ldx > ldo ? ldx : ldo) < (1L << 31), "conv3x3_wr_x3: operands past 2^31 elements");
+  ConvWrArgs a;
+  a.x = x; a.ldx = ldx; a.w = (const bf16*)w; a.bias = bias; a.resid = resid; a.ldr = ldr;
+  a.out = out; a.odt = KAIR_F32; a.ldo = ldo; a.acopy = nullptr; a.ldac = 0; a.acones = -1;
+  a.out_lo = nullptr; a.ps_r = 0; a.act = KAIR_ACT_NONE; a.slope = 0.f; a.gate = nullptr; a.ldg = 0;
+  a.psH = a.psW = 0;
+  a.ascale = ldexpf(1.f, ea); a.oscale = ldexpf(1.f, -(ea + KAIR_X3_WEXP));
+  a.B = B; a.H = H; a.W = W; a.C = C; a.N = N; a.flip = flip;
+  a.tilesM = M / BM;
+  a.fc8 = make_fdiv(C / 8);
+  a.fhwd = make_fdiv((W < BM ? W : BM) + 2);
+  const int ncu = wr_num_cus();
+  const int grid = (int)(a.tilesM < ncu ? a.tilesM : ncu);
+  hipStream_t s = (hipStream_t)stream;
+#define KAIR_WRX(BMV, RV) KAIR_LAUNCH((conv3x3_wr_kernel<float, true, BMV, RV, 3, 0, f16>), dim3(grid), dim3(WR_NT), 0, s, a)
+  if (BM == 48) {
+    if (resid) KAIR_WRX(48, true); else KAIR_WRX(48, false);
+  } else {
+    if (resid) KAIR_WRX(96, true); else KAIR_WRX(96, false);
+  }
+#undef KAIR_WRX
+  KAIR_CHECK_LAUNCH();
+  return 0;
+}
diff --git a/kair_amd/csrc/elementwise.hip b/kair_amd/csrc/elementwise.hip
--- a/kair_amd/csrc/elementwise.hip
+++ b/kair_amd/csrc/elementwise.hip
@@ -228,6 +228,8 @@
 __host__ __device__ inline bool pack_pair_vec(const kair_wmap& mp, int dt) {
   if (dt != KAIR_F16 && dt != KAIR_BF16) return false;
   const int Np = mp.nG * mp.nGp, Kp = mp.kG * mp.kGp;
+  if (mp.kind == 22) return dt == KAIR_F16 && Np % 16 == 0 && Kp % 8 == 0 && (9 * Kp) % 32 == 0;
+  if (mp.kind == 23) return dt == KAIR_F16 && Kp % 16 == 0 && Np % 8 == 0 && (9 * Np) % 32 == 0;
   if (mp.kind == 9 || mp.kind == 17 || mp.kind == 20) return Kp % 8 == 0;
   if (mp.kind == 18 || mp.kind == 19 || mp.kind == 21) return Np % 8 == 0;
   return false;
@@ -235,17 +237,25 @@
 
 KAIR_DEV void pack_pair_chunk(const float* __restrict__ src, void* __restrict__ dst, int dt, const kair_wmap& mp, int u) {
   const int Np = mp.nG * mp.nGp, Kp = mp.kG * mp.kGp;
-  const bool rows_n = mp.kind == 9 || mp.kind == 17 || mp.kind == 20;
-  const int rowlen = mp.kind == 9 ? 9 * Kp : mp.kind == 17 ? Kp : mp.kind == 18 ? 9 * Np : mp.kind == 20 ? 4 * Kp : Np;
+  const bool frag = mp.kind == 22 || mp.kind == 23;
+  const bool rows_n = mp.kind == 9 || mp.kind == 17 || mp.kind == 20 || mp.kind == 22;
+  const int rowlen = (mp.kind == 9 || mp.kind == 22) ? 9 * Kp : mp.kind == 17 ? Kp : (mp.kind == 18 || mp.kind == 23) ? 9 * Np
+                     : mp.kind == 20 ? 4 * Kp : Np;
   const int rl64 = (rowlen + 63) / 64 * 64, cpr = rl64 / 8;
-  const int row = u / cpr, k0 = (u - row * cpr) * 8;
+  int row = u / cpr, k0 = (u - row * cpr) * 8;
+  if (frag) {
+    const int ln = u & 63, blk = u >> 6, KB = rowlen / 32;
+    row = (blk / KB) * 16 + (ln & 15);
+    k0 = (blk - (blk / KB) * KB) * 32 + 8 * (ln >> 4);
+  }
   float v[8];
 #pragma unroll
   for (int j = 0; j < 8; ++j) v[j] = 0.f;
   if (k0 < rowlen) {
     const int rr = rows_n ? nperm_fwd(mp, unpad(row, mp.nG, mp.nGr, mp.nGp))
                           : unpad(mp.kind == 21 ? row >> 2 : row, mp.kG, mp.kGr, mp.kGp);
-    const int seg = (mp.kind == 9 || mp.kind == 20) ? Kp : (mp.kind == 18) ? Np : rowlen;
+    const int seg = (mp.kind == 9 || mp.kind == 20 || mp.kind == 22) ? Kp : (mp.kind == 18 || mp.kind == 23) ? Np
+                    : rowlen;
     const int tap = mp.kind == 21 ? (row & 3) : k0 / seg, c0 = mp.kind == 21 ? k0 : k0 - (k0 / seg) * seg;
 #pragma unroll
     for (int j = 0; j < 8; ++j) {
@@ -254,13 +264,14 @@
       if (rows_n) { n = rr; k = unpad(c, mp.kG, mp.kGr, mp.kGp); }
       else { n = nperm_fwd(mp, unpad(c, mp.nG, mp.nGr, mp.nGp)); k = rr; }
       if (n < 0 || k < 0) continue;
-      if (mp.kind == 9) v[j] = src[((long)n * mp.K + k % mp.K) * 9 + tap];
-      else if (mp.kind == 18) v[j] = src[((long)n * mp.K + k) * 9 + tap];
+      if (mp.kind == 9 || mp.kind == 22) v[j] = src[((long)n * mp.K + k % mp.K) * 9 + tap];
+      else if (mp.kind == 18 || mp.kind == 23) v[j] = src[((long)n * mp.K + k) * 9 + tap];
       else if (mp.kind == 20 || mp.kind == 21) v[j] = src[((long)n * mp.K + k) * 4 + tap];
       else v[j] = src[(long)n * mp.K + k];
     }
   }
-  const long o = (long)row * 2 * rl64 + ((k0 >> 6) << 7) + (k0 & 63);
+  const long o = frag ? (long)(u >> 6) * 1024 + (u & 63) * 8 : (long)row * 2 * rl64 + ((k0 >> 6) << 7) + (k0 & 63);
+  const int lo_off = frag ? 512 : 64;
   if (dt == KAIR_F16) {
     f16x8 hi, lo;
 #pragma unroll
@@ -270,7 +281,7 @@
       lo[j] = (f16)(w - (float)hi[j]);
     }
     *(f16x8*)((f16*)dst + o) = hi;
-    *(f16x8*)((f16*)dst + o + 64) = lo;
+    *(f16x8*)((f16*)dst + o + lo_off) = lo;
   } else {
     bf16x8 hi, lo;
 #pragma unroll
@@ -279,7 +290,7 @@
       lo[j] = (bf16)(v[j] - (float)hi[j]);
     }
     *(bf16x8*)((bf16*)dst + o) = hi;
-    *(bf16x8*)((bf16*)dst + o + 64) = lo;
+    *(bf16x8*)((bf16*)dst + o + lo_off) = lo;
   }
 }
 
@@ -799,14 +810,14 @@
                  "pack_weight: the hi/lo split forms 12 / 15 are bf16 only");
   KAIR_CHECK_ARG(mp.kind != 9 || dst_dtype == KAIR_BF16 || dst_dtype == KAIR_F16,
                  "pack_weight: kind 9 is a bf16 or (x3) fp16 pair form");
-  KAIR_CHECK_ARG(dst_dtype == KAIR_F32 || dst_dtype == KAIR_BF16 || ((mp.kind == 9 || (mp.kind >= 17 && mp.kind <= 21)) &&
+  KAIR_CHECK_ARG(dst_dtype == KAIR_F32 || dst_dtype == KAIR_BF16 || ((mp.kind == 9 || (mp.kind >= 17 && mp.kind <= 23)) &&
                                                                      dst_dtype == KAIR_F16),
-                 "pack_weight: fp16 destinations are the x3 pair forms (kinds 9, 17, 18, 19, 20, 21)");
+                 "pack_weight: fp16 destinations are the x3 pair forms (kinds 9, 17 .. 23)");
   KAIR_CHECK_ARG(mp.nG > 0 && mp.nGr > 0 && mp.nGp >= mp.nGr && mp.nG * mp.nGr == mp.N, "pack_weight: bad N map");
   KAIR_CHECK_ARG(mp.kind == 4 ||
                      (mp.kG > 0 && mp.kGr > 0 && mp.kGp >= mp.kGr &&
                       (mp.kG * mp.kGr == mp.K ||
-                       ((mp.kind == 1 || mp.kind == 9 || mp.kind == 15) && mp.K > 0 && (mp.kG * mp.kGr) % mp.K == 0))),
+                       ((mp.kind == 1 || mp.kind == 9 || mp.kind == 15 || mp.kind == 22) && mp.K > 0 && (mp.kG * mp.kGr) % mp.K == 0))),
                  "pack_weight: bad K map");
   KAIR_CHECK_ARG(mp.n_perm <= 1 || (mp.nG == 1 && mp.N % mp.n_perm == 0), "pack_weight: n_perm needs nG == 1, N %% n_perm == 0");
   const long Np = (long)mp.nG * mp.nGp, Kp = (long)mp.kG * mp.kGp;
@@ -832,6 +843,14 @@
     *total = rows * 2 * ((rowlen + 63) / 64) * 64;
     return 0;
   }
+  if (mp.kind == 22 || mp.kind == 23) {
+    KAIR_CHECK_ARG(dst_dtype == KAIR_F16, "pack_weight: kinds 22 / 23 are fp16 pairs");
+    KAIR_CHECK_ARG(pack_pair_vec(mp, dst_dtype), "pack_weight: kind 22 needs Np %% 16 == 0, Kp %% 8 == 0, 9 Kp %% 32 == 0; "
+                                                 "kind 23 Kp %% 16 == 0, Np %% 8 == 0, 9 Np %% 32 == 0");
+    KAIR_CHECK_ARG(2 * Np * 9 * Kp / 16 < (1L << 31), "pack_weight: kind %d pack too large", mp.kind);
+    *total = 2 * Np * 9 * Kp;
+    return 0;
+  }
   if (mp.kind == 0 || mp.kind == 3 || mp.kind == 10 || mp.kind == 13 || mp.kind == 14) *total = Np * Kp;
   else if (mp.kind == 12) *total = 2 * Np * Kp;
   else if (mp.kind == 1 || mp.kind == 2 || mp.kind == 16) *total = Np * 9 * Kp;
@@ -847,7 +866,7 @@
   KAIR_CHECK_ARG(src && dst && map, "pack_weight: null pointer");
   long total;
   if (int rc = pack_total(*map, dst_dtype, &total)) return rc;
-  if (map->kind == 20 || map->kind == 21) {
+  if (map->kind >= 20 && map->kind <= 23) {
     KAIR_LAUNCH(pack_pair_kernel, dim3(nblk(total / 16, 256)), dim3(256), 0, (hipStream_t)stream, src, dst, dst_dtype,
                        *map, total / 16);
     KAIR_CHECK_LAUNCH();
diff --git a/kair_amd/engine/swinir_engine.py b/kair_amd/engine/swinir_engine.py
--- a/kair_amd/engine/swinir_engine.py
+++ b/kair_amd/engine/swinir_engine.py
@@ -138,13 +138,19 @@
             self.Wp15 = torch.empty(Cop * 2 * 9 * Cip, device=dev, dtype=torch.bfloat16)
             self.mapp16 = H.wmap(16, Co, Ci, (1, Co, Cop), (1, Ci, Cip), n_perm=n_perm)
             self.Wp16 = torch.empty(Cip * 9 * Cop, device=dev, dtype=torch.bfloat16)
-        self.wr_n64 = bool(wr) and not self.wr and not self.wr_pair and Cop == 64 and Cip == 192 and self.split and not tied_in
+        self.wr_n64 = (bool(wr) and not self.wr and not self.wr_pair and Cop == 64 and Cip == 192 and self.split and
+                       not tied_in and not self.x3)
         if self.wr_n64:
             self.mapc = H.wmap(15, Co, Ci, (1, Co, Cop), (1, Ci, Cip))
             self.Wc15 = torch.empty(Cop * 2 * 9 * Cip, device=dev, dtype=torch.bfloat16)
             self.mapc16 = H.wmap(16, Co, Ci, (1, Co, Cop), (1, Ci, Cip))
             self.Wc16 = torch.empty(Cip * 9 * Cop, device=dev, dtype=torch.bfloat16)
-        if self.wr:
+        if self.wr and self.x3:
+            self.map15 = H.wmap(22, Co, Ci, (1, Co, Cop), (1, Ci, Cip))
+            self.Wf15 = torch.empty(Cop * 2 * 9 * Cip, device=dev, dtype=torch.float16)
+            self.map16 = H.wmap(23, Co, Ci, (1, Co, Cop), (1, Ci, Cip))
+            self.Wd16 = torch.empty(Cip * 2 * 9 * Cop, device=dev, dtype=torch.float16)
+        elif self.wr:
             self.map15 = H.wmap(15, Co, Ci, (1, Co, Cop), (1, Ci, Cip))
             self.Wf15 = torch.empty(Cop * 2 * 9 * Cip, device=dev, dtype=torch.bfloat16)
             self.map16 = H.wmap(16, Co, Ci, (1, Co, Cop), (1, Ci, Cip))
@@ -268,7 +274,7 @@
         self.img_range = float(net.img_range)
         self.Cin_p = 8
         self.xin_hilo = self.split_act and 2 * self.in_ch <= self.Cin_p
-        self.conv_wr = bool(conv_wr) and self.split_act and self.Cp == 192 and self.C % 4 == 0
+        self.conv_wr = bool(conv_wr) and (self.split_act or self.x3) and self.Cp == 192 and self.C % 4 == 0
         self.device = net.conv_first.weight.device
         dev = self.device
         self.mean = net.mean.view(-1).to(dev, torch.float32).contiguous()
@@ -505,6 +511,9 @@
                 if not isinstance(r, _Resi3):
                     P["conv_bf"][id(r)] = (torch.zeros(M, Cp, device=dev, dtype=T), torch.zeros(M, Cp, device=dev, dtype=T))
                     P["conv_bf"][id(r)][1][:, self.C] = 1.0
+        if self.x3:
+            P["conv_wr"] = bool(self.conv_wr and H.conv3x3_wr_x3_tile(B, Hh, Ww, Cp, Cp) > 0 and
+                                M // 96 >= self.conv_wr_min_tiles)
         P["wg_ws"] = e(self._max_wgrad_ws(M, P))
         P["wg_ws2"] = (e(P["wg_ws"].numel() * max(1, -self.side_ctas)) if self.grouped_wgrad or self.side_stream
                        else None)
@@ -590,6 +599,9 @@
         cd, Cp, M, Hh, Ww = self.cd, self.Cp, P["M"], P["H"], P["W"]
         if not isinstance(r, _Resi3):
             ac = (P["conv_bf"][id(r)][1], self.C) if P.get("conv_halo") else None
+            if self.x3 and P.get("conv_wr") and r.wr:
+                H.conv3x3_wr_x3(src, Cp, self._ax, 0, r.Wf15, r.bp, resid, out, P["B"], Hh, Ww, Cp, Cp)
+                return
             if P.get("conv_wr") and r.wr:
                 assert src.dtype == torch.float32 and resid.dtype == torch.float32
                 H.conv3x3_wr(src, Cp, 0, r.Wf15, r.bp, resid, out, P["B"], Hh, Ww, Cp, Cp, acopy=ac[0], acones=ac[1],
@@ -609,7 +621,9 @@
         g = lambda p: grads[p]
         if not isinstance(r, _Resi3):
             ac = (P["conv_bf"][id(r)][0], -1) if P.get("conv_halo") else None
-            if P.get("conv_wr") and r.wr:
+            if self.x3 and P.get("conv_wr") and r.wr:
+                H.conv3x3_wr_x3(G, Cp, self._ax, 1, r.Wd16, None, None, D, P["B"], Hh, Ww, Cp, Cp)
+            elif P.get("conv_wr") and r.wr:
                 H.conv3x3_wr(G, Cp, 1, r.Wd16, None, None, D, P["B"], Hh, Ww, Cp, Cp, acopy=ac[0], split=False)
             else:
                 self._nt(H.im2col(G, Hh, Ww, Cp, flip=True), H.rows(r.Wd), H.epilogue(D, acopy=ac), M, Cp, 9 * Cp, cd)
```

Result: faster. 673.0, median of 6 (+2.9%).
